# hiroharu-kato/neural_renderer

Measured on AMD Instinct MI355X. Metric: rasterize fwd+bwd Mpixels/sec @256x256 batch=64, higher is better.
Workload: dtype f32

## Files before the change

neural_renderer_amd/_build.py:

```python
import os
import subprocess

HERE = os.path.dirname(os.path.abspath(__file__))
SOURCES = [os.path.join(HERE, 'csrc', n) for n in ('nr_forward.hip', 'nr_backward.hip', 'nr_backward_pixel_map.hip',
                                                      'nr_backward_gather.hip', 'nr_geometry.hip',
                                                      'nr_image.hip', 'nr_frontend.hip', 'nr_texture_io.hip', 'nr_optim.hip',
                                                      'nr_uv_pixel.hip', 'nr_vertex_colors.hip')]
HEADERS = [os.path.join(os.path.dirname(HERE), 'include', 'nr_hip.h'), os.path.join(os.path.dirname(HERE), 'include', 'nr_hip_profile.h'),
           os.path.join(HERE, 'csrc', 'nr_device.h'),
           os.path.join(HERE, 'csrc', 'nr_k6_tune.h'), os.path.join(HERE, 'csrc', 'nr_band_lines.h'),
           os.path.join(HERE, 'csrc', 'nr_shade.h')]
LIB_PATH = os.path.join(HERE, 'libnr_hip.so')
PROFILE_LIB_PATH = os.path.join(HERE, 'libnr_hip_prof.so')

HIPCC_FLAGS = [
    '--offload-arch=gfx950', '-O3', '-std=c++17', '-ffp-contract=off',
    '-fhip-fp32-correctly-rounded-divide-sqrt', '-munsafe-fp-atomics', '-fno-fast-math',
    '-fno-slp-vectorize',
    '-fPIC', '-shared', '-fvisibility=hidden',
]


def hipcc():
    for c in (os.environ.get('HIPCC'), '/opt/rocm/bin/hipcc', 'hipcc'):
        if c and (os.path.isabs(c) and os.path.exists(c) or not os.path.isabs(c)):
            return c
    return 'hipcc'


def needs_build():
    if not os.path.exists(LIB_PATH):
        return True
    t = os.path.getmtime(LIB_PATH)
    return any(os.path.getmtime(p) > t for p in SOURCES + HEADERS + [os.path.abspath(__file__)])


def build(force=False, verbose=False):
    if force or needs_build():
        cmd = [hipcc()] + HIPCC_FLAGS + SOURCES + ['-o', LIB_PATH]
        if verbose:
            print(' '.join(cmd))
        subprocess.check_call(cmd)
    return LIB_PATH


def build_profile(force=False, verbose=False):
    if force or not os.path.exists(PROFILE_LIB_PATH) or \
            any(os.path.getmtime(p) > os.path.getmtime(PROFILE_LIB_PATH) for p in SOURCES + HEADERS + [os.path.abspath(__file__)]):
        cmd = [hipcc()] + HIPCC_FLAGS + ['-DNR_PROFILE_HOOK=1'] + SOURCES + ['-o', PROFILE_LIB_PATH]
        if verbose:
            print(' '.join(cmd))
        subprocess.check_call(cmd)
    return PROFILE_LIB_PATH


def build_variant(tag, defines, verbose=False, sources=None, flags=None):
    out = os.path.join(HERE, 'libnr_hip_%s.so' % tag)
    cmd = [hipcc()] + (flags or HIPCC_FLAGS) + ['-D%s' % d for d in defines] + (sources or SOURCES) + ['-o', out]
    if verbose:
        print(' '.join(cmd))
    subprocess.check_call(cmd)
    return out


if __name__ == '__main__':
    import sys
    if len(sys.argv) > 2:
        print(build_variant(sys.argv[1], sys.argv[2:], verbose=True))
    else:
        print(build(force=True, verbose=True))
        print(build_profile(force=True, verbose=True))
```

neural_renderer_amd/csrc/nr_backward.hip:

```cpp
#include "nr_device.h"
#include "nr_band_lines.h"
#include "nr_k6_tune.h"

using namespace nr;

int nr::plan_backward(const BackwardCall &c, BackwardPlan &p)
{
    p = {};
    const bool fused = c.stages == STAGE_ALL;
    const bool k6 = (c.stages & STAGE_K6) && (c.rgb || c.alpha);
    const bool k7 = (c.stages & STAGE_K7) && (!fused || (c.grad_rgb_map && c.grad_textures));
    const bool k8 = (c.stages & STAGE_K8) && (!fused || c.grad_depth_map);
    const bool sampled = c.sampling_weight_map != nullptr;
    if (!c.faces || !c.face_index_map) return NR_E_NULL;
    if ((c.stages & (STAGE_K6 | STAGE_K8)) && !c.grad_faces) return NR_E_NULL;
    if (c.stages == STAGE_K6 && !k6) return NR_E_MODE;
    if (k6 && c.rgb && (!c.rgb_map || !c.grad_rgb_map)) return NR_E_NULL;
    if (k6 && c.alpha && (!c.alpha_map || !c.grad_alpha_map)) return NR_E_NULL;
    if (k7) {
        if (!c.grad_rgb_map || !c.grad_textures) return NR_E_NULL;
        if ((c.sampling_index_map != nullptr) != sampled) return NR_E_MODE;
        if (!sampled && (!c.weight_map || !c.depth_map)) return NR_E_NULL;
    }
    if (k8 && (!c.depth_map || !c.weight_map || !c.grad_depth_map)) return NR_E_NULL;
    if (int e = check_sizes(c.B, c.F, c.S)) return e;
    if (k6 && (size_t)c.B * c.S * c.S > 0x7fffffffull / 3) return NR_E_SIZE;
    if (k7 && (c.ts < 2 || c.ts > 1024)) return NR_E_SIZE;
    if (k7 && c.lit.light && sampled) return NR_E_MODE;

    const int B = c.B, F = c.F, ts = c.ts;
    p.k6 = k6;
    if (k6) {
        p.k6p = plan_k6(B, F, c.S, c.rgb, c.eps, c.flags);
        p.bands = p.k6p.kernel != K6_KERNEL_GLOBAL;
        if (p.bands && (!c.workspace || c.workspace_bytes < nr_backward_workspace_bytes(B, F, c.S, 1, 0))) return NR_E_WORKSPACE;
    }
    const bool fold = p.bands && k7 && ts <= 13;
    p.gather_first = fold && (size_t)B * F <= k6::SHARED_LAUNCH_MAX_FACES && !(c.flags & NR_FLAG_SERIAL_BACKWARD);
    p.face_zeros = p.gather_first ? FACE_ZEROS_ALL : (fold ? FACE_ZEROS_UNLISTED : FACE_ZEROS_NONE);
    p.finish = !p.bands ? FINISH_NONE : p.gather_first ? (ts <= 8 ? FINISH_BIG : FINISH_ADD) : (fold ? FINISH_GATHER : FINISH_KERNEL);

    if (k7) {
        const size_t n_tex = (size_t)ts * ts * ts * 3;
        const bool ts2_static = ts == 2 && (float)(1.0 - c.eps) < 1.0f;
        p.static_taps = ts2_static && !sampled;
        p.gather = ts <= 13 ? GATHER_FACE : GATHER_ATOMIC;
        p.listed = p.bands && ts <= 13;
        p.lanes = p.static_taps ? 16 : (ts <= 5 ? 16 : (ts <= 8 ? 64 : 256));
        p.gather_lds = p.static_taps ? 0 : (size_t)(256 / p.lanes) * n_tex * sizeof(double);
        p.big = ts <= 8;
        p.depth_in_gather = k8 && ts <= 8 && !sampled && !(ts == 2 && !ts2_static);
        p.tex_bytes = (size_t)B * (c.lit.light ? c.lit.tex_faces : F) * n_tex * sizeof(float);
        if (p.gather_first) {
            p.setup_in_gather = p.k6p.use_records && k6_line_setup_args(c, p.k6p).lds_bytes <= 32768 && p.gather_lds <= 40960;
            if (p.setup_in_gather && !c.lit.light && ((size_t)c.grad_textures & 15) == 0) p.tex_zeros = TEX_ZEROS_SETUP;
        } else if (fold && p.tex_bytes % 16 == 0 && ((size_t)c.grad_textures & 15) == 0 && p.tex_bytes <= p.k6p.fill_max) {
            p.tex_zeros = TEX_ZEROS_BAND;
        }
        if (p.tex_zeros == TEX_ZEROS_NONE && (c.lit.light || p.listed || ts > 13)) p.tex_zeros = TEX_ZEROS_FILL;
        p.light_fill = c.lit.light && c.lit.grad_light;
    }
    p.setup_alone = p.bands && p.k6p.use_records && !p.setup_in_gather;
    p.depth = k8 && !p.depth_in_gather;
    p.fill_faces = fused && !k6;
    p.depth_lists = p.fill_faces && k8 && c.visible_faces && c.workspace && k6_lists_fit(B, F, c.workspace_bytes);
    return 0;
}

static int fill_texture_zeros(const BackwardCall &c, const BackwardPlan &p)
{
    int e = p.tex_zeros == TEX_ZEROS_FILL ? fill_bytes(c.grad_textures, 0, p.tex_bytes, c.st) : 0;
    if (e == 0 && p.light_fill) e = fill_bytes(c.lit.grad_light, 0, (size_t)c.B * c.F * 3 * sizeof(float), c.st);
    return e;
}

int nr::run_backward(const BackwardCall &c)
{
    BackwardPlan p;
    if (int e = plan_backward(c, p)) return e;
    K6Lists l = {};
    if (p.fill_faces)
        if (int e = fill_bytes(c.grad_faces, 0, (size_t)c.B * c.F * 9 * sizeof(float), c.st)) return e;
    if (p.depth_lists) l = k6_list_visible(c);
    if (p.k6) {
        LineSetupArgs ls = {};
        if (p.bands) {
            if (int rc = k6_compact(c, p.k6p, p.face_zeros, l)) return rc;
            ls = k6_line_setup_args(c, p.k6p);
        }
        if (p.gather_first) {
            if (int rc = fill_texture_zeros(c, p)) return rc;
            if (int rc = gather_faces(c, p, l, p.setup_in_gather ? &ls : nullptr)) return rc;
        }
        if (p.setup_alone)
            if (int rc = run_line_setup(ls, c.st)) return rc;
        const bool band_fill = p.tex_zeros == TEX_ZEROS_BAND;
        if (int rc = k6_band(c, p.k6p, l, ls, band_fill ? c.grad_textures : nullptr, band_fill ? p.tex_bytes : 0)) return rc;
        if (p.finish == FINISH_KERNEL) k6_finalize(c, l, false);
    }
    if (p.gather != GATHER_NONE && !p.gather_first) {
        if (int rc = fill_texture_zeros(c, p)) return rc;
        if (p.gather == GATHER_FACE)
            if (int rc = gather_faces(c, p, l, nullptr)) return rc;
    }
    if (p.big) gather_big(c, p, l);
    if (p.gather == GATHER_ATOMIC) gather_atomic(c);
    if (p.depth) gather_depth(c, l);
    if (p.finish == FINISH_ADD) k6_finalize(c, l, true);
    return launch_status();
}

NR_API int nr_backward_pixel_map(const float *faces, const int32_t *face_index_map, const float *rgb_map,
                                 const float *alpha_map, const float *grad_rgb_map, const float *grad_alpha_map,
                                 float *grad_faces, int32_t B, int32_t F, int32_t S, double eps, int32_t return_rgb,
                                 int32_t return_alpha, int32_t flags, const uint8_t *visible_faces, void *workspace,
                                 size_t workspace_bytes, void *stream)
{
    BackwardCall c = {};
    c.stages = STAGE_K6, c.rgb = return_rgb != 0, c.alpha = return_alpha != 0;
    c.faces = faces, c.face_index_map = face_index_map, c.rgb_map = rgb_map, c.alpha_map = alpha_map;
    c.grad_rgb_map = grad_rgb_map, c.grad_alpha_map = grad_alpha_map, c.grad_faces = grad_faces;
    c.B = B, c.F = F, c.S = S, c.eps = eps, c.flags = flags, c.visible_faces = visible_faces;
    c.workspace = workspace, c.workspace_bytes = workspace_bytes, c.st = (hipStream_t)stream;
    return run_backward(c);
}

NR_API int nr_backward_textures(const int32_t *face_index_map, const float *sampling_weight_map,
                                const int32_t *sampling_index_map, const float *faces, const float *faces_z_ref,
                                const float *weight_map, const float *depth_map, const float *grad_rgb_map,
                                float *grad_textures, int32_t B, int32_t F, int32_t S, int32_t ts, double eps, int32_t flags,
                                void *stream)
{
    BackwardCall c = {};
    c.stages = STAGE_K7;
    c.faces = faces, c.faces_z_ref = faces_z_ref, c.face_index_map = face_index_map;
    c.sampling_weight_map = sampling_weight_map, c.sampling_index_map = sampling_index_map;
    c.weight_map = weight_map, c.depth_map = depth_map, c.grad_rgb_map = grad_rgb_map, c.grad_textures = grad_textures;
    c.B = B, c.F = F, c.S = S, c.ts = ts, c.eps = eps, c.flags = flags, c.st = (hipStream_t)stream;
    return run_backward(c);
}

NR_API int nr_backward_depth_map(const float *faces, const float *depth_map, const int32_t *face_index_map,
                                 const float *face_inv_map, const float *weight_map, const float *grad_depth_map,
                                 float *grad_faces, int32_t B, int32_t F, int32_t S, void *stream)
{
    BackwardCall c = {};
    c.stages = STAGE_K8;
    c.faces = faces, c.face_index_map = face_index_map, c.face_inv_map = face_inv_map, c.weight_map = weight_map;
    c.depth_map = depth_map, c.grad_depth_map = grad_depth_map, c.grad_faces = grad_faces;
    c.B = B, c.F = F, c.S = S, c.st = (hipStream_t)stream;
    return run_backward(c);
}

NR_API int nr_backward_rasterize(const float *faces, const float *faces_z_ref, const int32_t *face_index_map,
                                 const float *weight_map, const float *depth_map, const float *rgb_map,
                                 const float *alpha_map, const float *grad_rgb_map, const float *grad_alpha_map,
                                 const float *grad_depth_map, float *grad_faces, float *grad_textures, int32_t B,
                                 int32_t F, int32_t S, int32_t ts, double eps, int32_t flags,
                                 const uint8_t *visible_faces, void *workspace, size_t workspace_bytes, void *stream)
{
    return nr_backward_rasterize_lit(nullptr, faces, faces_z_ref, face_index_map, weight_map, depth_map, rgb_map, alpha_map,
                                     grad_rgb_map, grad_alpha_map, grad_depth_map, grad_faces, grad_textures, B, F, S, ts,
                                     eps, flags, visible_faces, workspace, workspace_bytes, stream);
}

NR_API int nr_backward_rasterize_lit(const nr_face_light *lit, const float *faces, const float *faces_z_ref,
                                     const int32_t *face_index_map, const float *weight_map, const float *depth_map,
                                     const float *rgb_map, const float *alpha_map, const float *grad_rgb_map,
                                     const float *grad_alpha_map, const float *grad_depth_map, float *grad_faces,
                                     float *grad_textures, int32_t B, int32_t F, int32_t S, int32_t ts, double eps,
                                     int32_t flags, const uint8_t *visible_faces, void *workspace, size_t workspace_bytes,
                                     void *stream)
{
    BackwardCall c = {};
    if (int e = face_light_args(grad_rgb_map && grad_textures ? lit : nullptr, F, true, c.lit)) return e;
    c.stages = STAGE_ALL, c.rgb = grad_rgb_map != nullptr, c.alpha = grad_alpha_map != nullptr;
    c.faces = faces, c.faces_z_ref = faces_z_ref, c.face_index_map = face_index_map, c.weight_map = weight_map;
    c.depth_map = depth_map, c.rgb_map = c.rgb ? rgb_map : nullptr, c.alpha_map = c.alpha ? alpha_map : nullptr;
    c.grad_rgb_map = grad_rgb_map, c.grad_alpha_map = grad_alpha_map, c.grad_depth_map = grad_depth_map;
    c.grad_faces = grad_faces, c.grad_textures = grad_textures;
    c.B = B, c.F = F, c.S = S, c.ts = ts, c.eps = eps, c.flags = flags, c.visible_faces = visible_faces;
    c.workspace = workspace, c.workspace_bytes = workspace_bytes, c.st = (hipStream_t)stream;
    return run_backward(c);
}
```

neural_renderer_amd/csrc/nr_backward_gather.hip:

```cpp
#include "nr_device.h"
#include "nr_band_lines.h"
#include <type_traits>

using namespace nr;

namespace {

constexpr int BIG_PX = 2048;

__device__ __forceinline__ float group_sum(float v, int width)
{
    for (int o = width >> 1; o > 0; o >>= 1) v += __shfl_xor(v, o, WAVE);
    return v;
}

__device__ __forceinline__ float row16_sum_last(float v)
{
    v += __int_as_float(__builtin_amdgcn_update_dpp(0, __float_as_int(v), 0x111, 0xf, 0xf, true));
    v += __int_as_float(__builtin_amdgcn_update_dpp(0, __float_as_int(v), 0x112, 0xf, 0xf, true));
    v += __int_as_float(__builtin_amdgcn_update_dpp(0, __float_as_int(v), 0x114, 0xf, 0xf, true));
    v += __int_as_float(__builtin_amdgcn_update_dpp(0, __float_as_int(v), 0x118, 0xf, 0xf, true));
    return v;
}

struct DepthConst {
    float tmp[3], zz[3];
};
__device__ __forceinline__ DepthConst depth_constants(const float f[9], int S)
{
    const float fs = (float)S;
    const float px[3] = {to_pixel(f[0], fs), to_pixel(f[3], fs), to_pixel(f[6], fs)};
    const float py[3] = {to_pixel(f[1], fs), to_pixel(f[4], fs), to_pixel(f[7], fs)};
    float inv[9];
    compute_face_inv(px, py, inv);
    DepthConst d;
#pragma unroll
    for (int k = 0; k < 3; k++) {
        d.tmp[k] = 0.0f;
#pragma unroll
        for (int l = 0; l < 3; l++) d.tmp[k] += -inv[3 * l + k] / f[3 * l + 2];
        d.zz[k] = f[3 * k + 2] * f[3 * k + 2];
    }
    return d;
}

template <int STEPS, class Eval>
__device__ __forceinline__ void walk_owned_pixels(const Cand &cd, int n_mine, int fn, const int32_t *__restrict__ fi_img,
                                                  int S, int sub, int L, int *__restrict__ queue_base, Eval eval)
{
    const int tid = threadIdx.x;
    const int QL = L < 64 ? L : 64;
    int *queue = queue_base + (tid / QL) * (2 * QL);
    const int qsub = tid & (QL - 1);
    const int qshift = (tid & 63) & ~(QL - 1);
    const unsigned long long qmask = QL == 64 ? ~0ull : ((1ull << QL) - 1ull);
    int waiting = 0;
    for (int i = sub;; i += STEPS * L) {
        bool more2[STEPS], owned2[STEPS];
        int off2[STEPS];
#pragma unroll
        for (int h = 0; h < STEPS; ++h) {
            const int ii = i + h * L;
            more2[h] = ii < n_mine;
            int x = 0, y = 0, f = 0;
            off2[h] = 0;
            bool in = false;
            if (more2[h] && cand_pixel(cd, ii, S, x, y)) {
                off2[h] = y * S + x;
                f = fi_img[off2[h]];
                in = true;
            }
            owned2[h] = in && f == fn;
        }
        bool done = false;
#pragma unroll
        for (int h = 0; h < STEPS; ++h) {
            if (done) break;
            const bool more = more2[h], owned = owned2[h];
            const int off = off2[h];
            const bool any_more = __ballot(more) != 0ull;
            const unsigned long long m = (__ballot(owned) >> qshift) & qmask;
            if (owned) queue[waiting + __popcll(m & ((1ull << qsub) - 1ull))] = off;
            waiting += __popcll(m);
            const bool ready = waiting >= QL || (!any_more && waiting > 0);
            if (__ballot(ready) != 0ull) {
                __builtin_amdgcn_fence(__ATOMIC_RELEASE, "wavefront");
                __builtin_amdgcn_wave_barrier();
                __builtin_amdgcn_fence(__ATOMIC_ACQUIRE, "wavefront");
                const int take = ready ? (waiting < QL ? waiting : QL) : 0;
                const int e = qsub < take ? queue[qsub] : 0;
                const int rest = (ready && qsub + QL < waiting) ? queue[qsub + QL] : 0;
                __builtin_amdgcn_fence(__ATOMIC_RELEASE, "wavefront");
                __builtin_amdgcn_wave_barrier();
                __builtin_amdgcn_fence(__ATOMIC_ACQUIRE, "wavefront");
                waiting -= take;
                if (ready && qsub < waiting) queue[qsub] = rest;
                if (qsub < take) eval(e);
            }
            if (!any_more) done = true;
        }
        if (done) break;
    }
}

struct FaceGatherArgs {
    const int32_t *face_index_map;
    const float *sampling_weight_map;
    const int32_t *sampling_index_map;
    const float *faces, *zbase, *weight_map, *depth_map, *g_rgb;
    float *grad_textures;
    int n_faces_total, F, S, ts;
    double eps;
    int fix_batch_z, L;
    const int *vis_list, *vis_count;
    const float *g_depth;
    float *grad_faces;
    const double *k6_scratch;
    const int *slot_of;
    FaceLight lit;
};

template <bool TS2, bool DEPTH, bool LIT>
__device__ __forceinline__ void face_gather_body(const FaceGatherArgs &a, const int bx, const int by)
{
    const int32_t *__restrict__ face_index_map = a.face_index_map;
    const float *__restrict__ sampling_weight_map = a.sampling_weight_map;
    const int32_t *__restrict__ sampling_index_map = a.sampling_index_map;
    const float *__restrict__ faces = a.faces, *__restrict__ zbase = a.zbase, *__restrict__ weight_map = a.weight_map,
                *__restrict__ depth_map = a.depth_map, *__restrict__ g_rgb = a.g_rgb;
    float *__restrict__ grad_textures = a.grad_textures;
    const int n_faces_total = a.n_faces_total, F = a.F, S = a.S, ts = a.ts;
    const double eps = a.eps;
    const int fix_batch_z = a.fix_batch_z, L = a.L;
    const int *__restrict__ vis_list = a.vis_list, *__restrict__ vis_count = a.vis_count;
    const float *__restrict__ g_depth = a.g_depth;
    float *__restrict__ grad_faces = a.grad_faces;
    const double *__restrict__ k6_scratch = a.k6_scratch;
    const FaceLight &lit = a.lit;
    extern __shared__ __attribute__((aligned(16))) double s_acc[];
    __shared__ int s_queue[512];
    __shared__ int s_own;
    __shared__ float s_gl[3];

    const int tid = threadIdx.x;
    const int grp = tid / L, sub = tid - grp * L;
    const int n_tex = ts * ts * ts * 3;
    int gi = bx * (256 / L) + grp;
    bool face_ok = gi < n_faces_total;
    int slot = 0;
    if (vis_list) {
        slot = gi;
        const int n_vis = vis_count[by];
        if (bx * (256 / L) >= n_vis) return;
        face_ok = slot < n_vis;
        gi = face_ok ? by * F + vis_list[(size_t)by * F + slot] : 0;
    }
    double *acc_l = s_acc + (size_t)grp * n_tex;

    float acc[24];
#pragma unroll
    for (int k = 0; k < 24; k++) acc[k] = 0.0f;
    float dacc[9];
#pragma unroll
    for (int k = 0; k < 9; k++) dacc[k] = 0.0f;
    bool any_box = false;
    bool own = false;
    if (!TS2) {
        for (int k = sub; k < n_tex; k += L) acc_l[k] = 0.0;
        if (LIT) {
            if (tid < 3) s_gl[tid] = 0.0f;
            if (tid == 0) s_own = 0;
        }
        __syncthreads();
    }

    Cand cd;
    cd.n = 0;
    int fn = 0;
    size_t img = 0;
    DepthConst dc;
#pragma unroll
    for (int k = 0; k < 3; k++) dc.tmp[k] = dc.zz[k] = 0.0f;
    float face_z[3] = {1.0f, 1.0f, 1.0f};
    bool flip = false;
    size_t cube = 0;
    if (LIT) {
        const int b = vis_list ? by : gi / F, f = gi - b * F;
        flip = f >= lit.tex_faces;
        cube = (size_t)b * lit.tex_faces + (flip ? f - lit.tex_faces : f);
    }
    if (face_ok) {
        const int b = gi / F;
        fn = gi - b * F;
        const float *f = faces + (size_t)gi * 9;
        cd = face_candidates(f[0], f[1], f[3], f[4], f[6], f[7], S);
        if (cd.n > 0 && (L == 256 || (cd.n <= BIG_PX))) {
            any_box = true;
            if (DEPTH) {
                float fv[9];
#pragma unroll
                for (int k = 0; k < 9; k++) fv[k] = f[k];
                dc = depth_constants(fv, S);
            }
            const float *fz = (fix_batch_z ? faces + (size_t)b * F * 9 : zbase) + (size_t)fn * 9;
            face_z[0] = fz[2]; face_z[1] = fz[5]; face_z[2] = fz[8];
            img = (size_t)b * S * S;
        }
    }
    walk_owned_pixels<(TS2 && DEPTH) ? 1 : 2>(cd, any_box ? cd.n : 0, fn, face_index_map + img, S, sub, L, s_queue, [&](int off) {
        const size_t p = img + (size_t)off;
        float wk[3] = {0.0f, 0.0f, 0.0f}, depth = 0.0f, gd = 0.0f;
        if (weight_map) { wk[0] = weight_map[3 * p]; wk[1] = weight_map[3 * p + 1]; wk[2] = weight_map[3 * p + 2]; }
        if (depth_map) depth = depth_map[p];
        if (DEPTH) gd = g_depth[p];
        const float g[3] = {g_rgb[3 * p], g_rgb[3 * p + 1], g_rgb[3 * p + 2]};
        if (LIT) own = true;
        Taps t;
        if (sampling_weight_map) {
#pragma unroll
            for (int pn = 0; pn < 8; pn++) {
                t.w[pn] = sampling_weight_map[8 * p + pn];
                t.isc[pn] = sampling_index_map[8 * p + pn];
            }
        } else {
            compute_taps(face_z, wk, depth, ts, eps, t, LIT && flip);
        }
        if (DEPTH) {
            const float depth2 = depth * depth;
#pragma unroll
            for (int k = 0; k < 3; k++) dacc[3 * k + 2] += gd * wk[k] * depth2 / dc.zz[k];
#pragma unroll
            for (int k = 0; k < 3; k++)
#pragma unroll
                for (int l = 0; l < 2; l++) dacc[3 * k + l] += -gd * dc.tmp[l] * wk[k] * depth2 * (float)S / 2.0f;
        }
#pragma unroll
        for (int pn = 0; pn < 8; pn++) {
            if (TS2) {
                acc[3 * pn + 0] += t.w[pn] * g[0];
                acc[3 * pn + 1] += t.w[pn] * g[1];
                acc[3 * pn + 2] += t.w[pn] * g[2];
            } else {
                if (t.isc[pn] * 3 >= n_tex) continue;
                double *q = acc_l + t.isc[pn] * 3;
                atomicAdd(q + 0, (double)(t.w[pn] * g[0]));
                atomicAdd(q + 1, (double)(t.w[pn] * g[1]));
                atomicAdd(q + 2, (double)(t.w[pn] * g[2]));
            }
        }
    });

    bool owned = false;
    if (LIT) {
        if (L <= 64) {
            const unsigned long long bm = __ballot(own);
            owned = L == 64 ? bm != 0ull : ((bm >> (tid & 48)) & 0xffffull) != 0ull;
        } else {
            if (own) s_own = 1;
            __syncthreads();
            owned = s_own != 0;
        }
    }
    if (TS2) {
#pragma unroll
        for (int k = 0; k < 24; k++) acc[k] = row16_sum_last(acc[k]);
        if (LIT) {
            if (face_ok && sub == 15 && owned) {
                const float *lc = lit.light + (size_t)gi * 3;
                const float l3[3] = {lc[0], lc[1], lc[2]};
                float tx[24];
                if (lit.textures) {
                    const float4 *src = reinterpret_cast<const float4 *>(lit.textures + cube * 24);
#pragma unroll
                    for (int k = 0; k < 6; k++) {
                        const float4 v = src[k];
                        tx[4 * k] = v.x; tx[4 * k + 1] = v.y; tx[4 * k + 2] = v.z; tx[4 * k + 3] = v.w;
                    }
                } else {
#pragma unroll
                    for (int k = 0; k < 24; k++) tx[k] = 0.0f;
                }
                float o[24], gl[3] = {0.0f, 0.0f, 0.0f};
#pragma unroll
                for (int u = 0; u < 8; u++) {
                    const int r = (u & 1) * 4 + (u & 2) + (u >> 2);
#pragma unroll
                    for (int c = 0; c < 3; c++) {
                        const float a = flip ? acc[3 * u + c] : acc[3 * r + c];
                        o[3 * u + c] = a * l3[c];
                        gl[c] += a * tx[3 * u + c];
                    }
                }
                float4 *dst = reinterpret_cast<float4 *>(grad_textures + cube * 24);
#pragma unroll
                for (int k = 0; k < 6; k++) dst[k] = make_float4(o[4 * k], o[4 * k + 1], o[4 * k + 2], o[4 * k + 3]);
                if (lit.grad_light) {
                    float *gd = lit.grad_light + (size_t)gi * 3;
                    gd[0] = gl[0]; gd[1] = gl[1]; gd[2] = gl[2];
                }
            }
        } else if (face_ok && sub == 15) {
            float o[24];
#pragma unroll
            for (int pn = 0; pn < 8; pn++) {
                const int isc = (pn & 1) * 4 + ((pn >> 1) & 1) * 2 + ((pn >> 2) & 1);
                o[3 * isc + 0] = acc[3 * pn + 0];
                o[3 * isc + 1] = acc[3 * pn + 1];
                o[3 * isc + 2] = acc[3 * pn + 2];
            }
            float4 *dst = reinterpret_cast<float4 *>(grad_textures + (size_t)gi * 24);
#pragma unroll
            for (int k = 0; k < 6; k++) dst[k] = make_float4(o[4 * k], o[4 * k + 1], o[4 * k + 2], o[4 * k + 3]);
        }
    } else if (LIT) {
        __syncthreads();
        float gl0 = 0.0f, gl1 = 0.0f, gl2 = 0.0f;
        if (face_ok && owned) {
            const float *lc = lit.light + (size_t)gi * 3;
            const float l3[3] = {lc[0], lc[1], lc[2]};
            const float *tex = lit.textures ? lit.textures + cube * n_tex : nullptr;
            float *dst = grad_textures + cube * n_tex;
            if (tex) {
                for (int k = sub; k < n_tex; k += L) {
                    const int c = k % 3;
                    const float v = (float)acc_l[k] * tex[k];
                    gl0 += c == 0 ? v : 0.0f;
                    gl1 += c == 1 ? v : 0.0f;
                    gl2 += c == 2 ? v : 0.0f;
                }
            }
            for (int k = sub; k < n_tex; k += L) {
                const int c = k % 3;
                dst[k] = (float)acc_l[k] * (c == 0 ? l3[0] : (c == 1 ? l3[1] : l3[2]));
            }
        }
        if (lit.grad_light) {
            if (L <= 64) {
                gl0 = group_sum(gl0, L); gl1 = group_sum(gl1, L); gl2 = group_sum(gl2, L);
            } else {
                if (gl0 != 0.0f) atomicAdd(&s_gl[0], gl0);
                if (gl1 != 0.0f) atomicAdd(&s_gl[1], gl1);
                if (gl2 != 0.0f) atomicAdd(&s_gl[2], gl2);
                __syncthreads();
                gl0 = s_gl[0]; gl1 = s_gl[1]; gl2 = s_gl[2];
            }
            if (face_ok && owned && sub == 0) {
                float *gd = lit.grad_light + (size_t)gi * 3;
                gd[0] = gl0; gd[1] = gl1; gd[2] = gl2;
            }
        }
    } else {
        __syncthreads();
        if (face_ok) {
            float *dst = grad_textures + (size_t)gi * n_tex;
            for (int k = sub; k < n_tex; k += L) dst[k] = (float)acc_l[k];
        }
    }
    if (DEPTH || k6_scratch) {
        if (DEPTH && __ballot(any_box) != 0ull) {
#pragma unroll
            for (int k = 0; k < 9; k++) dacc[k] = (L == 16) ? row16_sum_last(dacc[k]) : group_sum(dacc[k], L);
        }
        if (face_ok && sub == ((L == 16) ? 15 : 0)) {
            float *gf = grad_faces + (size_t)gi * 9;
            if (k6_scratch) {
                const double *sc = k6_scratch + ((size_t)by * F + slot) * 6;
#pragma unroll
                for (int v = 0; v < 3; v++) {
                    gf[3 * v + 0] = (float)sc[2 * v + 0] + dacc[3 * v + 0];
                    gf[3 * v + 1] = (float)sc[2 * v + 1] + dacc[3 * v + 1];
                    gf[3 * v + 2] = 0.0f + dacc[3 * v + 2];
                }
            } else if (any_box) {
#pragma unroll
                for (int k = 0; k < 9; k++) gf[k] += dacc[k];
            }
        }
    }
}

template <bool TS2, bool DEPTH, bool LIT>
__global__ __launch_bounds__(256) void k_backward_textures_face(FaceGatherArgs a)
{
    face_gather_body<TS2, DEPTH, LIT>(a, (int)blockIdx.x, (int)blockIdx.y);
}

struct ZeroArgs {
    float *grad_textures;
    const int *slot_of;
    int F;
    int epf;
    int vec;
    unsigned wgs;
};

__device__ __forceinline__ void zero_unlisted_body(const ZeroArgs &z, const int bx, const int by)
{
    const size_t per_image = (size_t)z.F * z.epf;
    const size_t e0 = (size_t)bx * 2048, e1 = e0 + 2048 < per_image ? e0 + 2048 : per_image;
    const int *__restrict__ slot = z.slot_of + (size_t)by * z.F;
    for (size_t e = e0 + threadIdx.x; e < e1; e += 256) {
        const int face = (int)(e / (unsigned)z.epf);
        if (slot[face] >= 0) continue;
        const size_t at = (size_t)by * per_image + e;
        if (z.vec) reinterpret_cast<float4 *>(z.grad_textures)[at] = make_float4(0.0f, 0.0f, 0.0f, 0.0f);
        else z.grad_textures[at] = 0.0f;
    }
}

template <bool TS2, bool DEPTH, bool LIT>
__global__ __launch_bounds__(256) void k_setup_gather(LineSetupArgs ls, FaceGatherArgs g, ZeroArgs z, unsigned gather_x)
{
    const unsigned bx = blockIdx.x;
    if (bx < ls.grid_x) line_setup_body(ls, (int)bx, (int)blockIdx.y);
    else if (bx < ls.grid_x + gather_x) face_gather_body<TS2, DEPTH, LIT>(g, (int)(bx - ls.grid_x), (int)blockIdx.y);
    else zero_unlisted_body(z, (int)(bx - ls.grid_x - gather_x), (int)blockIdx.y);
}

template <int TEX, bool DEPTH, bool LIT>
__global__ __launch_bounds__(256) void k_backward_big(
    const int32_t *__restrict__ face_index_map, const float *__restrict__ sampling_weight_map,
    const int32_t *__restrict__ sampling_index_map, const float *__restrict__ face_inv_map, const float *__restrict__ faces,
    const float *__restrict__ zbase, const float *__restrict__ weight_map, const float *__restrict__ depth_map, const float *__restrict__ g_rgb,
    float *__restrict__ grad_textures, int n_faces_total, int F, int S, int ts, double eps, int fix_batch_z,
    const int *__restrict__ vis_list, const int *__restrict__ vis_count, const float *__restrict__ g_depth,
    float *__restrict__ grad_faces, const unsigned char *__restrict__ visible, FaceLight lit,
    const double *__restrict__ k6_scratch)
{
    extern __shared__ __attribute__((aligned(16))) double s_tex[];
    __shared__ int s_list[256];
    __shared__ int s_wave_n[4];
    __shared__ float s_red[36];
    __shared__ int s_own;
    const int tid = threadIdx.x;
    if (vis_list && (int)blockIdx.x * 256 >= vis_count[blockIdx.y]) return;
    int n_big;
    {
        int gi = blockIdx.x * 256 + tid;
        bool ok = gi < n_faces_total;
        if (vis_list) {
            ok = gi < vis_count[blockIdx.y];
            gi = ok ? (int)blockIdx.y * F + vis_list[(size_t)blockIdx.y * F + gi] : 0;
        }
        if (k6_scratch && ok && blockIdx.z == 0) {
            const double *sc = k6_scratch + ((size_t)blockIdx.y * F + blockIdx.x * 256 + tid) * 6;
            float *gf = grad_faces + (size_t)gi * 9;
#pragma unroll
            for (int v = 0; v < 3; v++) {
                atomicAdd(gf + 3 * v + 0, (float)sc[2 * v + 0]);
                atomicAdd(gf + 3 * v + 1, (float)sc[2 * v + 1]);
            }
        }
        bool big = false;
        if (ok && !vis_list && visible && !visible[gi]) ok = false;
        if (ok) {
            const float *f = faces + (size_t)gi * 9;
            const Cand cd = face_candidates(f[0], f[1], f[3], f[4], f[6], f[7], S);
            big = cd.n > BIG_PX;
        }
        const unsigned long long m = __ballot(big);
        const int lane = tid & 63, wave = tid >> 6;
        if (lane == 0) s_wave_n[wave] = __popcll(m);
        __syncthreads();
        int before = 0;
        for (int w = 0; w < wave; w++) before += s_wave_n[w];
        if (big) s_list[before + __popcll(m & ((1ull << lane) - 1ull))] = gi;
        n_big = s_wave_n[0] + s_wave_n[1] + s_wave_n[2] + s_wave_n[3];
        __syncthreads();
    }
    const int n_tex = TEX ? ts * ts * ts * 3 : 0;
    const int n_lds = TEX == 1 ? n_tex : 0;
    for (int q = blockIdx.z; q < n_big; q += gridDim.z) {
        const int gi = s_list[q];
        const int b = gi / F, fn = gi - b * F;
        const float *fp = faces + (size_t)gi * 9;
        float f[9];
#pragma unroll
        for (int k = 0; k < 9; k++) f[k] = fp[k];
        const Cand cd = face_candidates(f[0], f[1], f[3], f[4], f[6], f[7], S);
        DepthConst dc;
        if (DEPTH) dc = depth_constants(f, S);
        const float *fz = (fix_batch_z ? faces + (size_t)b * F * 9 : zbase) + (size_t)fn * 9;
        const float face_z[3] = {fz[2], fz[5], fz[8]};
        const bool flip = TEX && LIT && fn >= lit.tex_faces;
        for (int k = tid; k < n_lds; k += 256) s_tex[k] = 0.0;
        if (tid < 36) s_red[tid] = 0.0f;
        if (LIT && tid == 0) s_own = 0;
        __syncthreads();
        bool own = false;
        float dacc[9], tacc[24];
#pragma unroll
        for (int k = 0; k < 9; k++) dacc[k] = 0.0f;
#pragma unroll
        for (int k = 0; k < 24; k++) tacc[k] = 0.0f;
        const size_t img = (size_t)b * S * S;
        for (int i = tid; i < cd.n; i += 256) {
            int x, y;
            if (!cand_pixel(cd, i, S, x, y)) continue;
            const size_t p = img + (size_t)y * S + x;
            if (face_index_map[p] != fn) continue;
            if (LIT) own = true;
            float wk[3] = {0.0f, 0.0f, 0.0f}, depth = 0.0f;
            if (weight_map) { wk[0] = weight_map[3 * p]; wk[1] = weight_map[3 * p + 1]; wk[2] = weight_map[3 * p + 2]; }
            if (depth_map) depth = depth_map[p];
            if (TEX) {
                Taps t;
                if (sampling_weight_map) {
#pragma unroll
                    for (int pn = 0; pn < 8; pn++) {
                        t.w[pn] = sampling_weight_map[8 * p + pn];
                        t.isc[pn] = sampling_index_map[8 * p + pn];
                    }
                } else {
                    compute_taps(face_z, wk, depth, ts, eps, t, flip);
                }
                const float g[3] = {g_rgb[3 * p], g_rgb[3 * p + 1], g_rgb[3 * p + 2]};
#pragma unroll
                for (int pn = 0; pn < 8; pn++) {
                    if (TEX == 2) {
                        tacc[3 * pn + 0] += t.w[pn] * g[0];
                        tacc[3 * pn + 1] += t.w[pn] * g[1];
                        tacc[3 * pn + 2] += t.w[pn] * g[2];
                    } else {
                        if (t.isc[pn] * 3 >= n_tex) continue;
                        double *a = s_tex + t.isc[pn] * 3;
                        atomicAdd(a + 0, (double)(t.w[pn] * g[0]));
                        atomicAdd(a + 1, (double)(t.w[pn] * g[1]));
                        atomicAdd(a + 2, (double)(t.w[pn] * g[2]));
                    }
                }
            }
            if (DEPTH) {
                const float gd = g_depth[p];
                const float depth2 = depth * depth;
                float tmp[3] = {dc.tmp[0], dc.tmp[1], dc.tmp[2]};
                if (face_inv_map) {
                    tmp[0] = tmp[1] = tmp[2] = 0.0f;
#pragma unroll
                    for (int k = 0; k < 3; k++)
#pragma unroll
                        for (int l = 0; l < 3; l++) tmp[k] += -face_inv_map[9 * p + 3 * l + k] / f[3 * l + 2];
                }
#pragma unroll
                for (int k = 0; k < 3; k++) dacc[3 * k + 2] += gd * wk[k] * depth2 / dc.zz[k];
#pragma unroll
                for (int k = 0; k < 3; k++)
#pragma unroll
                    for (int l = 0; l < 2; l++) dacc[3 * k + l] += -gd * tmp[l] * wk[k] * depth2 * (float)S / 2.0f;
            }
        }
        if (DEPTH) {
#pragma unroll
            for (int k = 0; k < 9; k++) {
                const float v = group_sum(dacc[k], 64);
                if ((tid & 63) == 0 && v != 0.0f) atomicAdd(&s_red[k], v);
            }
        }
        if (TEX == 2) {
#pragma unroll
            for (int k = 0; k < 24; k++) {
                const float v = group_sum(tacc[k], 64);
                if ((tid & 63) == 0 && v != 0.0f) atomicAdd(&s_red[9 + k], v);
            }
        }
        if (TEX && LIT && own) s_own = 1;
        __syncthreads();
        if (TEX && LIT) {
            if (s_own) {
                const size_t cube = (size_t)b * lit.tex_faces + (flip ? fn - lit.tex_faces : fn);
                const float *lc = lit.light + (size_t)gi * 3;
                const float *tex = lit.textures ? lit.textures + cube * n_tex : nullptr;
                float *dst = grad_textures + cube * n_tex;
                for (int k = tid; k < n_tex; k += 256) {
                    const int q = k / 3, c = k - 3 * q;
                    int u = k;
                    float a;
                    if (TEX == 2) {
                        u = 3 * (flip ? q : (q & 1) * 4 + (q & 2) + (q >> 2)) + c;
                        a = s_red[9 + k];
                    } else {
                        a = (float)s_tex[k];
                    }
                    dst[u] = a * lc[c];
                    if (tex && a != 0.0f) atomicAdd(&s_red[33 + c], a * tex[u]);
                }
                if (lit.grad_light) {
                    __syncthreads();
                    if (tid < 3) lit.grad_light[(size_t)gi * 3 + tid] = s_red[33 + tid];
                }
            }
        } else {
        if (TEX == 1) {
            float *dst = grad_textures + (size_t)gi * n_tex;
            for (int k = tid; k < n_tex; k += 256) dst[k] = (float)s_tex[k];
        }
        if (TEX == 2 && tid < 24) {
            const int pn = tid / 3, c = tid - 3 * pn;
            const int isc = (pn & 1) * 4 + ((pn >> 1) & 1) * 2 + ((pn >> 2) & 1);
            grad_textures[(size_t)gi * 24 + 3 * isc + c] = s_red[9 + tid];
        }
        }
        if (DEPTH && tid < 9) {
            if (k6_scratch) atomicAdd(grad_faces + (size_t)gi * 9 + tid, s_red[tid]);
            else grad_faces[(size_t)gi * 9 + tid] += s_red[tid];
        }
        __syncthreads();
    }
}

__global__ __launch_bounds__(256) void k_backward_textures_atomic(
    const int32_t *__restrict__ face_index_map, const float *__restrict__ sampling_weight_map,
    const int32_t *__restrict__ sampling_index_map, const float *__restrict__ faces,
    const float *__restrict__ zbase, const float *__restrict__ weight_map, const float *__restrict__ depth_map,
    const float *__restrict__ g_rgb, float *__restrict__ grad_textures, int F, int S, int ts, double eps,
    int fix_batch_z, size_t n_pixels)
{
    const size_t i = (size_t)blockIdx.x * blockDim.x + threadIdx.x;
    if (i >= n_pixels) return;
    const int fi = face_index_map[i];
    if (fi < 0) return;
    const int b = (int)(i / ((size_t)S * S));
    Taps t;
    if (sampling_weight_map) {
#pragma unroll
        for (int pn = 0; pn < 8; pn++) {
            t.w[pn] = sampling_weight_map[8 * i + pn];
            t.isc[pn] = sampling_index_map[8 * i + pn];
        }
    } else {
        const float *face = (fix_batch_z ? faces + (size_t)b * F * 9 : zbase) + (size_t)fi * 9;
        const float w[3] = {weight_map[3 * i], weight_map[3 * i + 1], weight_map[3 * i + 2]};
        const float fz[3] = {face[2], face[5], face[8]};
        compute_taps(fz, w, depth_map[i], ts, eps, t);
    }
    const float g[3] = {g_rgb[3 * i], g_rgb[3 * i + 1], g_rgb[3 * i + 2]};
    float *gt = grad_textures + ((size_t)b * F + fi) * ts * ts * ts * 3;
#pragma unroll
    for (int pn = 0; pn < 8; pn++) {
        if (t.isc[pn] >= ts * ts * ts) continue;
        float *p = gt + t.isc[pn] * 3;
        atomicAdd(p + 0, t.w[pn] * g[0]);
        atomicAdd(p + 1, t.w[pn] * g[1]);
        atomicAdd(p + 2, t.w[pn] * g[2]);
    }
}


__global__ __launch_bounds__(256) void k_backward_textures_atomic_lit(
    const int32_t *__restrict__ face_index_map, const float *__restrict__ faces, const float *__restrict__ zbase,
    const float *__restrict__ weight_map, const float *__restrict__ depth_map, const float *__restrict__ g_rgb,
    float *__restrict__ grad_textures, int F, int S, int ts, double eps, int fix_batch_z, size_t n_pixels, FaceLight lit)
{
    const size_t i = (size_t)blockIdx.x * blockDim.x + threadIdx.x;
    if (i >= n_pixels) return;
    const int fi = face_index_map[i];
    if (fi < 0) return;
    const int b = (int)(i / ((size_t)S * S));
    const bool flip = fi >= lit.tex_faces;
    const size_t cube = ((size_t)b * lit.tex_faces + (flip ? fi - lit.tex_faces : fi)) * ts * ts * ts * 3;
    Taps t;
    const float *face = (fix_batch_z ? faces + (size_t)b * F * 9 : zbase) + (size_t)fi * 9;
    const float w[3] = {weight_map[3 * i], weight_map[3 * i + 1], weight_map[3 * i + 2]};
    const float fz[3] = {face[2], face[5], face[8]};
    compute_taps(fz, w, depth_map[i], ts, eps, t, flip);
    const float g[3] = {g_rgb[3 * i], g_rgb[3 * i + 1], g_rgb[3 * i + 2]};
    const float *lc = lit.light + ((size_t)b * F + fi) * 3;
    const float l3[3] = {lc[0], lc[1], lc[2]};
    float *gt = grad_textures + cube;
    const float *tex = lit.textures ? lit.textures + cube : nullptr;
    float sample[3] = {0.0f, 0.0f, 0.0f};
#pragma unroll
    for (int pn = 0; pn < 8; pn++) {
        if (t.isc[pn] >= ts * ts * ts) continue;
        float *p = gt + t.isc[pn] * 3;
#pragma unroll
        for (int c = 0; c < 3; c++) {
            atomicAdd(p + c, (t.w[pn] * g[c]) * l3[c]);
            if (tex) sample[c] += t.w[pn] * tex[t.isc[pn] * 3 + c];
        }
    }
    if (lit.grad_light) {
        float *gl = lit.grad_light + ((size_t)b * F + fi) * 3;
#pragma unroll
        for (int c = 0; c < 3; c++) atomicAdd(gl + c, g[c] * sample[c]);
    }
}

__global__ __launch_bounds__(256) void k_backward_depth_face(
    const float *__restrict__ faces, const float *__restrict__ depth_map, const int32_t *__restrict__ face_index_map,
    const float *__restrict__ face_inv_map, const float *__restrict__ weight_map, const float *__restrict__ g_depth,
    float *__restrict__ grad_faces, int n_faces_total, int F, int S, const int *__restrict__ vis_list,
    const int *__restrict__ vis_count, const unsigned char *__restrict__ visible)
{
    constexpr int L = 16;
    const int tid = threadIdx.x;
    const int grp = tid / L, sub = tid - grp * L;
    if (vis_list && (int)blockIdx.x * (256 / L) >= vis_count[blockIdx.y]) return;
    int gi = blockIdx.x * (256 / L) + grp;
    bool face_ok = gi < n_faces_total;
    if (vis_list) {
        const int slot = gi;
        face_ok = slot < vis_count[blockIdx.y];
        gi = face_ok ? (int)blockIdx.y * F + vis_list[(size_t)blockIdx.y * F + slot] : 0;
    } else if (visible && face_ok && !visible[gi]) {
        face_ok = false;
    }
    float acc[9];
#pragma unroll
    for (int k = 0; k < 9; k++) acc[k] = 0.0f;
    bool any_box = false;
    __shared__ int s_queue[512];
    Cand cd;
    cd.n = 0;
    int fn = 0;
    size_t img = 0;
    float f[9];
#pragma unroll
    for (int k = 0; k < 9; k++) f[k] = 1.0f;
    DepthConst dc;
#pragma unroll
    for (int k = 0; k < 3; k++) dc.tmp[k] = dc.zz[k] = 0.0f;
    if (face_ok) {
        const int b = gi / F;
        fn = gi - b * F;
        const float *fp = faces + (size_t)gi * 9;
#pragma unroll
        for (int k = 0; k < 9; k++) f[k] = fp[k];
        cd = face_candidates(f[0], f[1], f[3], f[4], f[6], f[7], S);
        if (cd.n > 0 && cd.n <= BIG_PX) {
            any_box = true;
            dc = depth_constants(f, S);
            img = (size_t)b * S * S;
        }
    }
    walk_owned_pixels<2>(cd, any_box ? cd.n : 0, fn, face_index_map + img, S, sub, L, s_queue, [&](int off) {
        const size_t p = img + (size_t)off;
        const float depth = depth_map[p];
        const float w[3] = {weight_map[3 * p], weight_map[3 * p + 1], weight_map[3 * p + 2]};
        const float gd = g_depth[p];
        const float depth2 = depth * depth;
#pragma unroll
        for (int k = 0; k < 3; k++) acc[3 * k + 2] += gd * w[k] * depth2 / dc.zz[k];
        float tmp[3] = {dc.tmp[0], dc.tmp[1], dc.tmp[2]};
        if (face_inv_map) {
            tmp[0] = tmp[1] = tmp[2] = 0.0f;
#pragma unroll
            for (int k = 0; k < 3; k++)
#pragma unroll
                for (int l = 0; l < 3; l++) tmp[k] += -face_inv_map[9 * p + 3 * l + k] / f[3 * l + 2];
        }
#pragma unroll
        for (int k = 0; k < 3; k++)
#pragma unroll
            for (int l = 0; l < 2; l++) acc[3 * k + l] += -gd * tmp[l] * w[k] * depth2 * (float)S / 2.0f;
    });
    if (__ballot(any_box) == 0ull) return;
#pragma unroll
    for (int k = 0; k < 9; k++) acc[k] = row16_sum_last(acc[k]);
    if (face_ok && any_box && sub == 15) {
        float *gf = grad_faces + (size_t)gi * 9;
#pragma unroll
        for (int k = 0; k < 9; k++) gf[k] += acc[k];
    }
}

inline dim3 big_grid(bool listed, int B, int F)
{
    const size_t n = (size_t)B * F;
    const dim3 g = listed ? dim3((unsigned)((F + 255) / 256), (unsigned)B) : dim3((unsigned)((n + 255) / 256));
    const size_t ranges = (size_t)g.x * g.y;
    const size_t target = n / 64 < 1024 ? 1024 : (n / 64 > 4096 ? 4096 : n / 64);
    const size_t z = target / ranges;
    return dim3(g.x, g.y, (unsigned)(z < 1 ? 1 : (z > 64 ? 64 : z)));
}

}


int nr::gather_faces(const BackwardCall &c, const BackwardPlan &p, const K6Lists &l, const LineSetupArgs *ls)
{
    const int B = c.B, F = c.F, n = B * F, ts = c.ts;
    const size_t n_tex = (size_t)ts * ts * ts * 3;
    const int per = 256 / p.lanes;
    const int *vis_list = p.listed ? l.vis_list : nullptr;
    const dim3 grid = vis_list ? dim3((unsigned)((F + per - 1) / per), (unsigned)B) : dim3((unsigned)((n + per - 1) / per));
    const bool fold = p.finish == FINISH_GATHER;
    const FaceGatherArgs ga = {c.face_index_map, c.sampling_weight_map, c.sampling_index_map, c.faces,
                               c.faces_z_ref ? c.faces_z_ref : c.faces,
                               c.weight_map, c.depth_map, c.grad_rgb_map, c.grad_textures, n, F, c.S, ts, c.eps,
                               (c.flags & NR_FLAG_FIX_TEXTURE_BATCH_Z) ? 1 : 0, p.lanes, vis_list, l.vis_count,
                               p.depth_in_gather ? c.grad_depth_map : nullptr,
                               (p.depth_in_gather || fold) ? c.grad_faces : nullptr, fold ? l.scratch : nullptr,
                               fold ? l.slot_of : nullptr, c.lit};
    auto go = [&](auto ts2, auto dep, auto lit) {
        constexpr bool T = decltype(ts2)::value, D = decltype(dep)::value, LIT = decltype(lit)::value;
        if (ls) {
            ZeroArgs z = {c.grad_textures, l.slot_of, F, (int)n_tex, 0, 0u};
            if (p.tex_zeros == TEX_ZEROS_SETUP) {
                z.vec = n_tex % 4 == 0;
                z.epf = z.vec ? (int)(n_tex / 4) : (int)n_tex;
                z.wgs = (unsigned)(((size_t)F * z.epf + 2047) / 2048);
            }
            const size_t both = p.gather_lds > ls->lds_bytes ? p.gather_lds : ls->lds_bytes;
            hipLaunchKernelGGL((k_setup_gather<T, D, LIT>), dim3(ls->grid_x + grid.x + z.wgs, (unsigned)B), dim3(256), both, c.st,
                               *ls, ga, z, grid.x);
        } else {
            hipLaunchKernelGGL((k_backward_textures_face<T, D, LIT>), grid, dim3(256), p.gather_lds, c.st, ga);
        }
    };
    auto with_lit = [&](auto ts2, auto dep) {
        if (c.lit.light) go(ts2, dep, std::true_type()); else go(ts2, dep, std::false_type());
    };
    using T = std::true_type;
    using N = std::false_type;
    if (p.static_taps) { if (p.depth_in_gather) with_lit(T(), T()); else with_lit(T(), N()); }
    else { if (p.depth_in_gather) with_lit(N(), T()); else with_lit(N(), N()); }
    return launch_status();
}

void nr::gather_big(const BackwardCall &c, const BackwardPlan &p, const K6Lists &l)
{
    const int n = c.B * c.F, ts = c.ts;
    const int *vis_list = p.listed ? l.vis_list : nullptr;
    const dim3 grid = big_grid(vis_list != nullptr, c.B, c.F);
    const size_t lds = p.static_taps ? 0 : (size_t)ts * ts * ts * 3 * sizeof(double);
    const float *zbase = c.faces_z_ref ? c.faces_z_ref : c.faces;
    const int fix = (c.flags & NR_FLAG_FIX_TEXTURE_BATCH_Z) ? 1 : 0;
    const double *finish_k6 = p.finish == FINISH_BIG ? l.scratch : nullptr;
    const float *g_depth = p.depth_in_gather ? c.grad_depth_map : nullptr;
    float *grad_faces = (p.depth_in_gather || finish_k6) ? c.grad_faces : nullptr;
    auto go = [&](auto lit) {
        constexpr bool LIT = decltype(lit)::value;
#define NR_BIG(T, D)                                                                                                            \
    hipLaunchKernelGGL((k_backward_big<T, D, LIT>), grid, dim3(256), lds, c.st, c.face_index_map, c.sampling_weight_map,        \
                       c.sampling_index_map, (const float *)nullptr, c.faces, zbase, c.weight_map, c.depth_map, c.grad_rgb_map, \
                       c.grad_textures, n, c.F, c.S, ts, c.eps, fix, vis_list, l.vis_count, g_depth, grad_faces,               \
                       (const unsigned char *)nullptr, c.lit, finish_k6)
        if (p.static_taps) { if (g_depth) NR_BIG(2, true); else NR_BIG(2, false); }
        else { if (g_depth) NR_BIG(1, true); else NR_BIG(1, false); }
#undef NR_BIG
    };
    if (c.lit.light) go(std::true_type()); else go(std::false_type());
}

void nr::gather_atomic(const BackwardCall &c)
{
    const size_t np = (size_t)c.B * c.S * c.S;
    const float *zbase = c.faces_z_ref ? c.faces_z_ref : c.faces;
    const int fix = (c.flags & NR_FLAG_FIX_TEXTURE_BATCH_Z) ? 1 : 0;
    if (c.lit.light)
        hipLaunchKernelGGL(k_backward_textures_atomic_lit, dim3((unsigned)((np + 255) / 256)), dim3(256), 0, c.st,
                           c.face_index_map, c.faces, zbase, c.weight_map, c.depth_map, c.grad_rgb_map, c.grad_textures, c.F,
                           c.S, c.ts, c.eps, fix, np, c.lit);
    else
        hipLaunchKernelGGL(k_backward_textures_atomic, dim3((unsigned)((np + 255) / 256)), dim3(256), 0, c.st, c.face_index_map,
                           c.sampling_weight_map, c.sampling_index_map, c.faces, zbase, c.weight_map, c.depth_map,
                           c.grad_rgb_map, c.grad_textures, c.F, c.S, c.ts, c.eps, fix, np);
}

void nr::gather_depth(const BackwardCall &c, const K6Lists &l)
{
    const int B = c.B, F = c.F, n = B * F;
    const dim3 grid = l.vis_list ? dim3((unsigned)((F + 15) / 16), (unsigned)B) : dim3((unsigned)((n + 15) / 16));
    hipLaunchKernelGGL(k_backward_depth_face, grid, dim3(256), 0, c.st, c.faces, c.depth_map, c.face_index_map, c.face_inv_map,
                       c.weight_map, c.grad_depth_map, c.grad_faces, n, F, c.S, l.vis_list, l.vis_count, c.visible_faces);
    const dim3 grid_big = big_grid(l.vis_list != nullptr, B, F);
    hipLaunchKernelGGL((k_backward_big<0, true, false>), grid_big, dim3(256), 0, c.st, c.face_index_map, (const float *)nullptr,
                       (const int32_t *)nullptr, c.face_inv_map, c.faces, c.faces, c.weight_map, c.depth_map, (const float *)nullptr,
                       (float *)nullptr, n, F, c.S, 2, 0.0, 0, l.vis_list, l.vis_count, c.grad_depth_map, c.grad_faces,
                       c.visible_faces, FaceLight(), (const double *)nullptr);
}
```

neural_renderer_amd/csrc/nr_backward_pixel_map.hip:

```cpp
#include "nr_device.h"
#include "nr_band_lines.h"
#include "nr_k6_tune.h"

#include <atomic>
#include <mutex>
#include <type_traits>

using namespace nr;

namespace {

constexpr int GRP = 10;
constexpr int NGRP = 6;

struct __attribute__((aligned(16))) LineRec {
    int in_rng;
    int out_rng;
    int base;
    int flags;
    float cross, c0, c1, pad;
    float in_c[4];
    float out_c[4];
};

template <bool RGB, bool ALPHA>
__global__ __launch_bounds__(WAVE) void k_bpm_global(
    const float *__restrict__ faces, const int32_t *__restrict__ fi_map, const float *__restrict__ rgb_map,
    const float *__restrict__ alpha_map, const float *__restrict__ g_rgb, const float *__restrict__ g_alpha,
    float *__restrict__ grad_faces, int F, int S, double eps)
{
    __shared__ LineRec recs[NGRP][GRP];

    const int lane = threadIdx.x;
    const int gi = blockIdx.x;
    const int b = gi / F, fn = gi - b * F;
    const float *f = faces + (size_t)gi * 9;
    const float fx[3] = {f[0], f[3], f[6]}, fy[3] = {f[1], f[4], f[7]};
    float *out = grad_faces + (size_t)gi * 9;
    if (is_backside(fx[0], fy[0], fx[1], fy[1], fx[2], fy[2])) {
        if (lane < 9) out[lane] = 0.0f;
        return;
    }
    const int g = lane / GRP, sub = lane - g * GRP;
    const bool lane_on = g < NGRP;
    const int edge = (g >> 1) % 3, axis = g & 1;
    const double s_d = (double)S, two_over_s = 2.0 / (double)S;
    const bool s_pow2 = (S & (S - 1)) == 0;

    const float fs = (float)S;
    const int i0 = edge, i1 = (edge + 1) % 3, i2 = (edge + 2) % 3;
    const float ppx[3] = {to_pixel(fx[i0], fs), to_pixel(fx[i1], fs), to_pixel(fx[i2], fs)};
    const float ppy[3] = {to_pixel(fy[i0], fs), to_pixel(fy[i1], fs), to_pixel(fy[i2], fs)};
    const float p0x = axis ? ppy[0] : ppx[0], p0y = axis ? ppx[0] : ppy[0];
    const float p1x = axis ? ppy[1] : ppx[1], p1y = axis ? ppx[1] : ppy[1];
    const float p2x = axis ? ppy[2] : ppx[2], p2y = axis ? ppx[2] : ppy[2];
    int direction;
    if (axis == 0) direction = (p0x < p1x) ? -1 : 1; else direction = (p0x < p1x) ? 1 : -1;
    const int d0_from = (int)fmax((double)ceilf(fminf(p0x, p1x)), 0.0);
    const int d0_to = (int)fmin((double)fmaxf(p0x, p1x), S - 1.0);
    int n_lines = 0;
    if (lane_on && p0x != p1x && d0_to >= d0_from) n_lines = d0_to - d0_from + 1;
    const float slope = (p1y - p0y) / (p1x - p0x);
    const int sd0 = axis ? S : 1, sd1 = axis ? 1 : S;
    const int img_base = b * S * S;

    int max_lines = n_lines;
#pragma unroll
    for (int o = 32; o > 0; o >>= 1) max_lines = max(max_lines, __shfl_xor(max_lines, o, WAVE));

    double G0 = 0.0, G1 = 0.0;

    for (int batch0 = 0; batch0 < max_lines; batch0 += GRP) {
        if (lane_on) {
            LineRec r;
            r.in_rng = 1; r.out_rng = 1; r.base = 0; r.flags = 0;
            r.cross = r.c0 = r.c1 = r.pad = 0.0f;
#pragma unroll
            for (int k = 0; k < 4; k++) { r.in_c[k] = 0.0f; r.out_c[k] = 0.0f; }
            const int it = batch0 + sub;
            if (it < n_lines) {
                const int d0 = d0_from + it;
                const float d0f = (float)d0;
                const float d1_cross = slope * (d0f - p0x) + p0y;
                const int d1_in = (0 < direction) ? (int)floorf(d1_cross) : (int)ceilf(d1_cross);
                const int d1_out = d1_in + direction;
                if (!(d1_in < 0 || S <= d1_in) && !(d1_out < 0 || S <= d1_out)) {
                    const int line_base = img_base + d0 * sd0;
                    const int idx_in = line_base + d1_in * sd1, idx_out = line_base + d1_out * sd1;
                    if (ALPHA) { r.in_c[0] = alpha_map[idx_in]; r.out_c[0] = alpha_map[idx_out]; }
                    if (RGB) {
#pragma unroll
                        for (int k = 0; k < 3; k++) {
                            r.in_c[1 + k] = rgb_map[3 * (size_t)idx_in + k];
                            r.out_c[1 + k] = rgb_map[3 * (size_t)idx_out + k];
                        }
                    }
                    const bool is_in_fn = (fi_map[idx_in] == fn);
                    int flags = 0;
                    if (p1x != d0f) flags |= 4;
                    if (p0x != d0f) flags |= 8;
                    r.c0 = (p1x - p0x) / (p1x - d0f);
                    r.c1 = (p1x - p0x) / (d0f - p0x);
                    if (is_in_fn) {
                        const int lim = (0 < direction) ? S - 1 : 0;
                        const int o_from = max(min(d1_out, lim), 0), o_to = min(max(d1_out, lim), S - 1);
                        r.out_rng = o_from | (o_to << 16);
                        flags |= 2;
                    }
                    float d0_cross2;
                    if ((d0f - p0x) * (d0f - p2x) < 0)
                        d0_cross2 = (p2y - p0y) / (p2x - p0x) * (d0f - p0x) + p0y;
                    else
                        d0_cross2 = (p1y - p2y) / (p1x - p2x) * (d0f - p2x) + p2y;
                    const int lim2 = (0 < direction) ? (int)ceilf(d0_cross2) : (int)floorf(d0_cross2);
                    const int i_from = max(min(d1_in, lim2), 0), i_to = min(max(d1_in, lim2), S - 1);
                    r.in_rng = i_from | (i_to << 16);
                    r.base = line_base;
                    r.flags = flags;
                    r.cross = d1_cross;
                }
            }
            recs[g][sub] = r;
        }
        __syncthreads();

        const int nl = lane_on ? min(max(n_lines - batch0, 0), GRP) : 0;
        int l = -1, ph = 0, d1 = 0, d1_end = -1, base = 0, cur_flags = 0;
        float cross = 0, c0 = 0, c1 = 0, ref_a = 0, ref_r = 0, ref_g = 0, ref_b = 0;
        while (__ballot(l < nl) != 0ull) {
            if (d1 > d1_end && l < nl) {
                if (ph == 0 && (cur_flags & 2)) ph = 1; else { ph = 0; ++l; }
                if (l < nl) {
                    const LineRec *r = &recs[g][l];
                    const int4 h = *reinterpret_cast<const int4 *>(r);
                    const float4 q = *reinterpret_cast<const float4 *>(&r->cross);
                    const float4 col = *reinterpret_cast<const float4 *>(ph == 0 ? r->out_c : r->in_c);
                    const int rng = ph == 0 ? h.x : h.y;
                    d1 = (rng & 0xffff) + sub;
                    d1_end = rng >> 16;
                    base = h.z;
                    cur_flags = h.w;
                    cross = q.x; c0 = q.y; c1 = q.z;
                    ref_a = col.x; ref_r = col.y; ref_g = col.z; ref_b = col.w;
                }
            }
            if (l < nl && d1 <= d1_end) {
                const int idx = base + d1 * sd1;
                bool skip = (ph == 0) && (fi_map[idx] != fn);
                float diff = 0.0f;
                if (!skip) {
                    if (ALPHA) diff += (alpha_map[idx] - ref_a) * g_alpha[idx];
                    if (RGB) {
                        const float *pp = rgb_map + 3 * (size_t)idx;
                        const float *gg = g_rgb + 3 * (size_t)idx;
                        diff += (pp[0] - ref_r) * gg[0];
                        diff += (pp[1] - ref_g) * gg[1];
                        diff += (pp[2] - ref_b) * gg[2];
                    }
                }
                if (!skip && !(diff <= 0.0f)) {
                    const float t = (float)d1 - cross;
                    if (cur_flags & 4) {
                        const float ct = c0 * t;
                        float dist = (float)(s_pow2 ? (double)ct * two_over_s : (double)ct * 2.0 / s_d);
                        dist = (0.0f < dist) ? (float)((double)dist + eps) : (float)((double)dist - eps);
                        G0 -= (double)(diff / dist);
                    }
                    if (cur_flags & 8) {
                        const float ct = c1 * t;
                        float dist = (float)(s_pow2 ? (double)ct * two_over_s : (double)ct * 2.0 / s_d);
                        dist = (0.0f < dist) ? (float)((double)dist + eps) : (float)((double)dist - eps);
                        G1 -= (double)(diff / dist);
                    }
                }
                d1 += GRP;
            }
        }
        __syncthreads();
    }

#pragma unroll
    for (int o = 8; o > 0; o >>= 1) {
        const double t0 = __shfl_down(G0, o, WAVE), t1 = __shfl_down(G1, o, WAVE);
        if (sub + o < GRP) { G0 += t0; G1 += t1; }
    }
    const int partner = (2 * ((edge + 2) % 3) + axis) * GRP;
    const double G1p = __shfl(G1, partner, WAVE);
    if (lane_on && sub == 0) {
        out[3 * edge + (1 - axis)] = (float)(G0 + G1p);
        if (axis == 0) out[3 * edge + 2] = 0.0f;
    }
}


constexpr int BAND_WIN = 256;
constexpr int FSEG = 15;
enum { K6_FAST = 0, K6_EXACT_POW2 = 1, K6_EXACT = 2 };

__global__ __launch_bounds__(256) void k_mark_visible(const int32_t *__restrict__ fi_map,
                                                      unsigned char *__restrict__ flags, int F, int SS, size_t P)
{
    const size_t i = (size_t)blockIdx.x * blockDim.x + threadIdx.x;
    if (i >= P) return;
    const int fi = fi_map[i];
    if (fi >= 0) flags[(i / SS) * F + fi] = 1;
}

__device__ __forceinline__ void emit_visible(int b, int fn, int pos, int F, int S, const float *__restrict__ faces,
                                             int *__restrict__ vis_list, unsigned *__restrict__ rng,
                                             double *__restrict__ scratch, int *band_count, int n_bands, int W,
                                             int *line_diff = nullptr)
{
    vis_list[(size_t)b * F + pos] = fn;
    const float *f = faces + ((size_t)b * F + fn) * 9;
    const float fs = (float)S;
    float px[3], py[3];
#pragma unroll
    for (int k = 0; k < 3; k++) { px[k] = to_pixel(f[3 * k], fs); py[k] = to_pixel(f[3 * k + 1], fs); }
    unsigned *r0 = rng + (((size_t)b * 2 + 0) * F + pos) * 3, *r1 = rng + (((size_t)b * 2 + 1) * F + pos) * 3;
#pragma unroll
    for (int e = 0; e < 3; e++) {
        const unsigned ra = edge_range(px[e], px[(e + 1) % 3], S), rb = edge_range(py[e], py[(e + 1) % 3], S);
        r0[e] = ra;
        r1[e] = rb;
#pragma unroll
        for (int axis = 0; axis < 2; axis++) {
            const unsigned r = axis ? rb : ra;
            const int lo = (int)(r & 0xffffu), hi = (int)(r >> 16);
            if (line_diff) {
                if (lo <= hi) {
                    atomicAdd(line_diff + axis * (S + 1) + lo, 1);
                    atomicAdd(line_diff + axis * (S + 1) + hi + 1, -1);
                }
                continue;
            }
            for (int band = lo / W; band * W <= hi; ++band)
                atomicAdd(band_count + axis * n_bands + band, min(hi, band * W + W - 1) - max(lo, band * W) + 1);
        }
    }
    double2 *z = reinterpret_cast<double2 *>(scratch + ((size_t)b * F + pos) * 6);
    z[0] = z[1] = z[2] = make_double2(0.0, 0.0);
}

__device__ __forceinline__ void zero_face(float *__restrict__ o)
{
#pragma unroll
    for (int k = 0; k < 9; k++) o[k] = 0.0f;
}

constexpr int VIS_CHUNK = 1024;
constexpr int SMALL_CHUNKS = 16;

__global__ __launch_bounds__(VIS_CHUNK) void k_compact_par(const unsigned char *__restrict__ flags,
                                                           int *__restrict__ vis_list, int *__restrict__ vis_count,
                                                           int *__restrict__ slot_of, int F, int n_chunks,
                                                           const float *__restrict__ faces, unsigned *__restrict__ rng,
                                                           double *__restrict__ scratch, int S,
                                                           int *__restrict__ chunk_band, int n_bands, int W,
                                                           int *__restrict__ band_cursor, float *__restrict__ zero_faces,
                                                           int zero_listed, int use_diff)
{
    extern __shared__ int s_band[];
    __shared__ int s_wcnt[VIS_CHUNK / 64];
    __shared__ int s_part[VIS_CHUNK / 64];
    const int b = blockIdx.y, chunk = blockIdx.x, tid = threadIdx.x, lane = tid & 63, wave = tid >> 6;
    for (int i = tid; i < 2 * n_bands; i += VIS_CHUNK) s_band[i] = 0;
    int *s_diff = use_diff ? s_band + 2 * n_bands : nullptr;
    if (use_diff)
        for (int i = tid; i < 2 * (S + 1); i += VIS_CHUNK) s_diff[i] = 0;
    int part = 0;
    for (int c = 0; c < chunk; ++c) part += __popcll(__ballot(flags[(size_t)b * F + c * VIS_CHUNK + tid] != 0));
    const int fn = chunk * VIS_CHUNK + tid;
    const bool v = fn < F && flags[(size_t)b * F + fn] != 0;
    const unsigned long long m = __ballot(v);
    if (lane == 0) { s_part[wave] = part; s_wcnt[wave] = __popcll(m); }
    __syncthreads();
    int off = 0, own = 0;
    for (int w = 0; w < VIS_CHUNK / 64; ++w) {
        off += s_part[w];
        if (w < wave) off += s_wcnt[w];
        own += s_wcnt[w];
    }
    if (fn < F) {
        const int before = off + __popcll(m & ((1ull << lane) - 1ull));
        slot_of[(size_t)b * F + fn] = v ? before : -1;
        if (v) emit_visible(b, fn, before, F, S, faces, vis_list, rng, scratch, s_band, n_bands, W, s_diff);
        if (zero_faces && (!v || zero_listed)) zero_face(zero_faces + ((size_t)b * F + fn) * 9);
    }
    __syncthreads();
    if (use_diff) {
        const int n2 = 2 * (S + 1), per = (n2 + VIS_CHUNK - 1) / VIS_CHUNK, i0 = tid * per, i1 = min(n2, i0 + per);
        int local = 0;
        for (int i = i0; i < i1; ++i) local += s_diff[i];
        int inc = local;
#pragma unroll
        for (int o = 1; o < 64; o <<= 1) {
            const int t = __shfl_up(inc, o, WAVE);
            if (lane >= o) inc += t;
        }
        __syncthreads();
        if (lane == 63) s_wcnt[wave] = inc;
        __syncthreads();
        int run = inc - local;
        for (int w = 0; w < wave; ++w) run += s_wcnt[w];
// ... 553 lines not shown
                        f0 = __builtin_fmaf(-dm, __builtin_amdgcn_rcpf(y0), f0);
                        f1 = __builtin_fmaf(-dm, __builtin_amdgcn_rcpf(y1), f1);
                    }
                };
                if (cls == 0) {
                    for (int u = 0; u < u_cnt; ++u) {
                    const auto p0 = f0, p1 = f1;
                    f0 = 0;
                    f1 = 0;
                    float4 gc[FB], gn[FB];
                    float ac[FB], an[FB];
#pragma unroll
                    for (int j = 0; j < FB; ++j) {
                        gc[j] = gn[j] = make_float4(0.0f, 0.0f, 0.0f, 0.0f);
                        ac[j] = an[j] = 0.0f;
                        if (RGB) gc[j] = lds_px4(gp + 4 * j);
                        else ac[j] = gp[j];
                    }
#pragma unroll
                    for (int kb = 0; kb < FSEG; kb += FB) {
                        asm volatile("" : "+v"(d1fb));
                        if (kb + FB < FSEG) {
#pragma unroll
                            for (int j = 0; j < FB; ++j) {
                                if (RGB) gn[j] = lds_px4(gp + 4 * (kb + FB + j));
                                else an[j] = gp[kb + FB + j];
                            }
                        }
#pragma unroll
                        for (int j = 0; j < FB; ++j) visit(bg_diff(gc[j], ac[j]), kb + j);
#pragma unroll
                        for (int j = 0; j < FB; ++j) { gc[j] = gn[j]; ac[j] = an[j]; }
                        __builtin_amdgcn_sched_barrier(0);
                    }
                    f0 += p0;
                    f1 += p1;
                    gp += (RGB ? 4 : 1) * FSEG;
                    d1fb += (float)FSEG;
                    }
                } else {
#pragma unroll
                    for (int kb = 0; kb < FSEG; kb += FB) {
                        asm volatile("" : "+v"(d1fb));
                        float4 g4[FB], c4[FB];
                        float ga[FB], ca[FB];
#pragma unroll
                        for (int j = 0; j < FB; ++j) {
                            g4[j] = c4[j] = make_float4(0.0f, 0.0f, 0.0f, 0.0f);
                            ga[j] = ca[j] = 0.0f;
                            if (RGB) {
                                g4[j] = lds_px4(gp + 4 * (kb + j));
                                c4[j] = lds_px4(cp + 4 * (kb + j));
                            } else {
                                ga[j] = gp[kb + j];
                                ca[j] = cp[kb + j];
                            }
                        }
#pragma unroll
                        for (int j = 0; j < FB; ++j) visit(own_diff(c4[j], ca[j], g4[j], ga[j]), kb + j);
                        __builtin_amdgcn_sched_barrier(0);
                    }
                }
            } else {
                const int own_mask = mode_in ? -1 : 0;
                float d1f = (float)s_from;
                float b0 = 0.0f, b1 = 0.0f;
                for (int l = base + s_from; l <= base + s_to; ++l, d1f += 1.0f) {
                    const int fi = px.fi[l];
                    float4 g4 = make_float4(0.0f, 0.0f, 0.0f, 0.0f), c4 = g4;
                    float ga = 0.0f, ca = 0.0f;
                    if (RGB) { g4 = lds_px4(px.g + 4 * (size_t)l); c4 = lds_px4(px.c + 4 * (size_t)l); }
                    else { ga = px.g[l]; ca = px.c[l]; }
                    const float diff = own_diff(c4, ca, g4, ga);
                    if ((((fi ^ fnr) & own_mask) != 0) | (diff <= 0.0f)) continue;
                    const float t = d1f - cross;
                    if constexpr (EXACT) {
                        f0 -= (double)exact_term(diff, c0k, t);
                        f1 -= (double)exact_term(diff, c1k, t);
                    } else {
                        const float x0 = c0k * t, x1 = c1k * t;
                        const float y0 = x0 + ((0.0f < x0) ? eps_f : -eps_f);
                        const float y1 = x1 + ((0.0f < x1) ? eps_f : -eps_f);
                        b0 = __builtin_fmaf(-diff, __builtin_amdgcn_rcpf(y0), b0);
                        b1 = __builtin_fmaf(-diff, __builtin_amdgcn_rcpf(y1), b1);
                    }
                }
                if constexpr (!EXACT) { f0 += b0; f1 += b1; }
            }
            using RunT = typename std::conditional<EXACT, double, float>::type;
            RunT p0 = (valid && (flags & 2)) ? (RunT)f0 : RunT(0), p1 = (valid && (flags & 4)) ? (RunT)f1 : RunT(0);
            const int key = valid ? line : -1 - (tid & 63);
            run_sums(key, p0, p1);
            const double a0 = (double)p0, a1 = (double)p1;
            if (a0 != 0.0) atomicAdd(&acc[2 * line], a0);
            if (a1 != 0.0) atomicAdd(&acc[2 * line + 1], a1);
        }
    }
}

template <bool RGB, bool ALPHA, int MODE, int NT, bool OVF = false>
__global__ __launch_bounds__(NT, MODE == K6_EXACT ? 4 : (NT == 256 ? k6::MINWAVES_256 : 6)) void k_bpm_fast(
    const float *__restrict__ faces, const int32_t *__restrict__ fi_map, const float *__restrict__ rgb_map,
    const float *__restrict__ alpha_map, const float *__restrict__ g_rgb, const float *__restrict__ g_alpha,
    const int *__restrict__ vis_list, const int *__restrict__ vis_count, const unsigned *__restrict__ rng,
    double *__restrict__ scratch, const int *__restrict__ band_lines, const int *__restrict__ band_start,
    const int *__restrict__ lines_ok, const BandLine *__restrict__ line_buf, size_t cap, int F, int S, int W, int SP,
    double eps, float k2s, int B, int win_lines, int qcap, uint4 *__restrict__ zero16, size_t n_zero16)
{
    extern __shared__ __attribute__((aligned(16))) unsigned char smem[];
    const int tid = threadIdx.x;
    const unsigned n_bands = (unsigned)(S + W - 1) / (unsigned)W;
    const unsigned total_wg = n_bands * 2u * (unsigned)B;
    constexpr bool overflow_only = OVF;
    auto band_body = [&](const unsigned logical) {
    if (n_zero16) {
        const size_t per = (n_zero16 + total_wg - 1) / total_wg, z_lo = (size_t)logical * per, z_hi = min(n_zero16, z_lo + per);
        for (size_t k = z_lo + tid; k < z_hi; k += NT) zero16[k] = make_uint4(0u, 0u, 0u, 0u);
    }
    const int band = (int)(logical % n_bands), axis = (int)((logical / n_bands) & 1u), b = (int)(logical / (2u * n_bands));
    const int band_lo = band * W, band_hi = min(band_lo + W, S) - 1;
    const int nld = band_hi - band_lo + 1;
    const size_t bidx = ((size_t)b * 2 + axis) * n_bands + band;
    if (overflow_only && lines_ok[b] != 0) return;
    const int n_band_lines = overflow_only ? 1 : band_lines[bidx];
    if (n_band_lines == 0) return;

    size_t off = 0;
    auto carve = [&](size_t bytes) { unsigned char *p = smem + off; off += (bytes + 15) & ~(size_t)15; return p; };
    constexpr int NC = RGB ? 4 : 1;
    FastPx px;
    px.fi = (int *)carve((size_t)W * SP * 4);
    px.g = (float *)carve((size_t)W * SP * NC * 4);
    px.c = (float *)carve((size_t)W * SP * NC * 4);
    px.bg = (float *)carve(16);
    px.CW = (((SP + 31) >> 5) + 3) & ~3;
    px.cov = (unsigned *)carve((size_t)W * px.CW * 4);
    px.span = (int *)carve(4 * 2 * 4);
    const bool wide = S > 63 * FSEG;
    BandLine *s_line = (BandLine *)carve(sizeof(BandLine) * win_lines);
    double *s_lacc = (double *)carve(16 * (size_t)win_lines);
    void *s_queue = carve((size_t)qcap * (wide ? 4 : 2));
    int *s_tmp = (int *)carve(4 * 16);

    const size_t img = (size_t)b * S * S;
    for (int i = tid; i < W * px.CW; i += NT) px.cov[i] = 0u;
    __syncthreads();
    fast_stage<RGB, ALPHA, NT>(px, fi_map, rgb_map, alpha_map, g_rgb, g_alpha, img, axis, band_lo, nld, S, SP);
    __syncthreads();
    if (tid < nld) {
        int first = 0x7fffffff, last = -1;
        for (int w = 0; w < px.CW; ++w) {
            const unsigned m = px.cov[tid * px.CW + w];
            if (m) { first = min(first, 32 * w + __ffs((int)m) - 1); last = 32 * w + 31 - __clz((int)m); }
        }
        px.span[2 * tid] = first;
        px.span[2 * tid + 1] = last;
    }

    const bool use_rec = !overflow_only && lines_ok[b] != 0;
    const BandLine *recs = line_buf + (size_t)b * cap + (use_rec ? band_start[bidx] : 0);
    const int n_vis = use_rec ? 0 : vis_count[b];
    const unsigned *rng_ba = rng + ((size_t)b * 2 + axis) * F * 3;
    int chunk = 0, win = 0;
    auto each_sum = [&](int n2, auto fn) {
        if (tid < n2) fn(tid);
        if (NT < 2 * BAND_WIN && tid + NT < n2) fn(tid + NT);
    };
    for (;;) {
        int n_win;
        if (use_rec) {
            if (win >= n_band_lines) break;
            n_win = min(n_band_lines - win, win_lines);
            if (tid < n_win) s_line[tid] = recs[win + tid];
            each_sum(2 * n_win, [&](int i) { s_lacc[i] = 0.0; });
            win += win_lines;
        } else {
            if (chunk >= n_vis) break;
            int nl = 0;
            int e_lo[3] = {0, 0, 0}, e_n[3] = {0, 0, 0};
            if (chunk + tid < n_vis) {
                const unsigned *r = rng_ba + (size_t)(chunk + tid) * 3;
#pragma unroll
                for (int e = 0; e < 3; e++) {
                    const unsigned pr = r[e];
                    const int lo = max((int)(pr & 0xffffu), band_lo), hi = min((int)(pr >> 16), band_hi);
                    if (hi >= lo) { e_lo[e] = lo; e_n[e] = hi - lo + 1; nl += e_n[e]; }
                }
            }
            int total_lines = 0;
            const int line_off = block_excl_scan<NT>(nl, s_tmp, &total_lines);
            if (win >= total_lines) {
                chunk += NT;
                win = 0;
                continue;
            }
            n_win = min(total_lines - win, win_lines);
            int2 *s_rec = reinterpret_cast<int2 *>(s_lacc);
            if (nl > 0 && line_off < win + win_lines && line_off + nl > win) {
                int k = line_off;
#pragma unroll
                for (int e = 0; e < 3; e++)
                    for (int j = 0; j < e_n[e]; j++, k++)
                        if (k >= win && k < win + win_lines) s_rec[k - win] = make_int2((chunk + tid) | (e << 28), e_lo[e] + j - band_lo);
            }
            __syncthreads();
            int2 rec = make_int2(0, 0);
            if (tid < n_win) rec = s_rec[tid];
            __syncthreads();
            if (tid < n_win) {
                const int pos = rec.x & 0x0fffffff, e = (rec.x >> 28) & 3, ld = rec.y;
                const int rfn = vis_list[(size_t)b * F + pos];
                s_line[tid] = make_fast_line(faces + ((size_t)b * F + rfn) * 9, e, axis, band_lo + ld, ld, S, rfn,
                                             pos | (e << 28) | (((e + 1) % 3) << 30),
                                             [&](int d1) { return px.fi[ld * SP + d1]; }, k2s);
            }
            each_sum(2 * n_win, [&](int i) { s_lacc[i] = 0.0; });
            win += win_lines;
        }
        __syncthreads();
        fast_sweeps<RGB, ALPHA, MODE, NT>(px, s_line, n_win, SP, eps, S, s_lacc, s_queue, qcap, wide,
                                      reinterpret_cast<unsigned long long *>(s_tmp));
        __syncthreads();
        each_sum(2 * n_win, [&](int i) {
            const double a = s_lacc[i];
            if (a != 0.0) {
                const int tgt = s_line[i >> 1].tgt;
                const int pos = tgt & 0x0fffffff, v = (i & 1) ? (tgt >> 30) & 3 : (tgt >> 28) & 3;
                atomicAdd(scratch + ((size_t)b * F + pos) * 6 + 2 * v + (1 - axis), a);
            }
        });
        __syncthreads();
    }
    };
    if constexpr (!OVF) {
        const unsigned logical = xcd_block(total_wg);
        if (logical < total_wg) band_body(logical);
    } else {
        int any = 0;
        for (int i = tid; i < B; i += NT) any |= lines_ok[i] == 0;
        if (!__syncthreads_or(any)) return;
        for (unsigned logical = blockIdx.x; logical < total_wg; logical += gridDim.x) {
            band_body(logical);
            __syncthreads();
        }
    }
}

__device__ __forceinline__ int window_team(int n_rec, int n_parts, int nsl)
{
    const int n_win = (n_rec + 63) >> 6;
    if (nsl < 32) return 1;
    int team = n_parts;
    while (team > 1 && n_parts / team < n_win) team >>= 1;
    return team;
}

__device__ __forceinline__ void wave_lds_handover()
{
    __builtin_amdgcn_fence(__ATOMIC_RELEASE, "wavefront");
    __builtin_amdgcn_wave_barrier();
    __builtin_amdgcn_fence(__ATOMIC_ACQUIRE, "wavefront");
}

namespace rowk {
constexpr int NT = 256, NW = NT / 64;
constexpr int WIN = 64;
constexpr int SEG = 16;
constexpr int MAX_SEGS = 64;
constexpr int IN_SEG = 16;
constexpr int IN_BATCH = 4;
constexpr int MAX_PX = 1024;
constexpr int K_BYTES = 4 * 16, WAVE_BYTES = WIN * 16;
template <bool RGB> __host__ __device__ constexpr size_t g_bytes(size_t npx) { return npx * (RGB ? 16 : 4); }
template <bool RGB, bool EXACT> __host__ __device__ constexpr size_t c_bytes(size_t npx) { return EXACT ? g_bytes<RGB>(npx) : npx * 4; }
template <bool RGB, bool EXACT> __host__ __device__ constexpr size_t lds_bytes(size_t npx)
{
    return g_bytes<RGB>(npx) + c_bytes<RGB, EXACT>(npx) + npx * 4 + (EXACT ? 0 : K_BYTES) + NW * WAVE_BYTES;
}
}

#ifdef NR_ROW_STATS
__device__ unsigned long long g_row_stats[8];
NR_API int nr_dev_row_stats(unsigned long long *out8)
{
    if (hipMemcpyFromSymbol(out8, HIP_SYMBOL(g_row_stats), sizeof(unsigned long long) * 8) != hipSuccess) return 1;
    unsigned long long z[8] = {0, 0, 0, 0, 0, 0, 0, 0};
    return hipMemcpyToSymbol(HIP_SYMBOL(g_row_stats), z, sizeof(z)) == hipSuccess ? 0 : 1;
}
#define NR_ROW_STAT(i, v) do { if (lane == 0) atomicAdd(&g_row_stats[i], (unsigned long long)(v)); } while (0)
constexpr unsigned NR_ROW_DUMP_WINDOWS = 1u << 16;
__device__ unsigned g_row_dump_n;
__device__ unsigned g_row_dump[NR_ROW_DUMP_WINDOWS * 64];
NR_API int nr_dev_row_dump(unsigned *out, unsigned *n_windows)
{
    if (hipMemcpyFromSymbol(n_windows, HIP_SYMBOL(g_row_dump_n), sizeof(unsigned)) != hipSuccess) return 1;
    const unsigned n = *n_windows < NR_ROW_DUMP_WINDOWS ? *n_windows : NR_ROW_DUMP_WINDOWS, zero = 0;
    if (n && hipMemcpyFromSymbol(out, HIP_SYMBOL(g_row_dump), (size_t)n * 64 * sizeof(unsigned)) != hipSuccess) return 1;
    return hipMemcpyToSymbol(HIP_SYMBOL(g_row_dump_n), &zero, sizeof(unsigned)) == hipSuccess ? 0 : 1;
}
#else
#define NR_ROW_STAT(i, v) ((void)0)
#endif

template <bool RGB, bool ALPHA, int MODE, bool CHUNKED>
__global__ __launch_bounds__(rowk::NT, MODE == K6_FAST ? 5 : 4) void k_bpm_row(
    const int32_t *__restrict__ fi_map, const float *__restrict__ rgb_map, const float *__restrict__ alpha_map,
    const float *__restrict__ g_rgb, const float *__restrict__ g_alpha, double *__restrict__ scratch,
    const int *__restrict__ band_lines, const int *__restrict__ band_start, const int *__restrict__ lines_ok,
    const BandLine *__restrict__ line_buf, size_t cap, int F, int S, int W, int CH, float eps_f, double eps_d, int B,
    uint4 *__restrict__ zero16, size_t n_zero16)
{
    using namespace rowk;
    constexpr bool EXACT = MODE != K6_FAST;
    extern __shared__ __attribute__((aligned(16))) unsigned char smem[];
    const int tid = threadIdx.x, lane = tid & 63, wave = rfl(tid >> 6);
    const unsigned n_bands = (unsigned)(S + W - 1) / (unsigned)W, n_ch = CHUNKED ? (unsigned)(S + CH - 1) / (unsigned)CH : 1u;
    const unsigned total_wg = n_bands * 2u * (unsigned)B * n_ch;
    const unsigned logical = xcd_block(total_wg);
    if (logical >= total_wg) return;
    if (n_zero16) {
        const size_t per = (n_zero16 + total_wg - 1) / total_wg, z_lo = (size_t)logical * per, z_hi = min(n_zero16, z_lo + per);
        for (size_t k = z_lo + tid; k < z_hi; k += NT) zero16[k] = make_uint4(0u, 0u, 0u, 0u);
    }
    const unsigned bandidx = logical / n_ch;
    const int c0 = CHUNKED ? (int)(logical - bandidx * n_ch) * CH : 0, SL = CHUNKED ? min(CH, S - c0) : S;
    const int band = (int)(bandidx % n_bands), axis = (int)((bandidx / n_bands) & 1u), b = (int)(bandidx / (2u * n_bands));
    if (lines_ok[b] == 0) return;
    const int band_lo = band * W, nld = min(W, S - band_lo);
    const size_t lt = ((size_t)b * 2 + axis) * S + band_lo;
    int n_tot = 0;
    for (int l = 0; l < nld; ++l) n_tot += band_lines[lt + l];
    if (n_tot == 0) return;

    constexpr int NC = RGB ? 4 : 1;
    const int SP = (SL + 31) & ~31, nsl = SP / SEG;
    const unsigned npx = (unsigned)(W * SP), G_BYTES = (unsigned)g_bytes<RGB>(npx), C_BYTES = (unsigned)c_bytes<RGB, EXACT>(npx), FI_BYTES = npx * 4u;
    float *const s_g = (float *)smem;
    float *const s_p = (float *)(smem + G_BYTES);
    int *const s_fi = (int *)(smem + G_BYTES + C_BYTES);
    float4 *const s_k = (float4 *)(smem + G_BYTES + C_BYTES + FI_BYTES);
    unsigned char *wave_mem = smem + G_BYTES + C_BYTES + FI_BYTES + (EXACT ? 0u : (unsigned)K_BYTES) + (unsigned)wave * WAVE_BYTES;
    double2 *acc = (double2 *)wave_mem;
    int *hist = (int *)wave_mem;
    const int n_parts = max(1, NW / W);
    const BandLine *recs_b = line_buf + (size_t)b * cap;
    const size_t img = (size_t)b * S * S;
    auto map_index = [&](int ld, int d1) { return axis ? img + (size_t)(band_lo + ld) * S + (c0 + d1) : img + (size_t)(c0 + d1) * S + band_lo + ld; };
    auto map_colour = [&](size_t gi) {
        float4 c = make_float4(0.0f, 0.0f, 0.0f, 0.0f);
        if constexpr (!RGB || ALPHA) c.x = alpha_map[gi];
        if constexpr (RGB) { c.y = rgb_map[3 * gi]; c.z = rgb_map[3 * gi + 1]; c.w = rgb_map[3 * gi + 2]; }
        return c;
    };
    auto line_k = [&](int ld) {
        if constexpr (EXACT) return make_float4(0.0f, 0.0f, 0.0f, 0.0f);
        float4 k = map_colour(map_index(ld, 0));
        const bool fin = fabsf(k.x) <= 3.0e38f && fabsf(k.y) <= 3.0e38f && fabsf(k.z) <= 3.0e38f && fabsf(k.w) <= 3.0e38f;
        if (!fin) k = make_float4(0.0f, 0.0f, 0.0f, 0.0f);
        return k;
    };
    int4 hh_first = make_int4(1, 1, 0, 0);
    float4 qq_first = make_float4(0.0f, 0.0f, 0.0f, 0.0f);
    if (wave < nld * n_parts) {
        const int ld = wave / n_parts, part = wave - ld * n_parts;
        const int n_rec = band_lines[lt + ld], r = (part / window_team(n_rec, n_parts, nsl)) * WIN + lane;
        if (r < n_rec) {
            const BandLine *R = recs_b + band_start[lt + ld] + r;
            hh_first = *reinterpret_cast<const int4 *>(R);
            qq_first = *reinterpret_cast<const float4 *>(&R->cross);
        }
    }
    {
        auto put = [&](int ld, int d1, int fi, const float4 &k, float al, float ga, float r, float g, float bl, float gr, float gg, float gb) {
            const int l = ld * SP + d1;
            s_fi[l] = fi;
            if constexpr (RGB) {
                *reinterpret_cast<float4 *>(s_g + 4 * (size_t)l) = make_float4(ga, gr, gg, gb);
                if constexpr (EXACT)
                    *reinterpret_cast<float4 *>(s_p + 4 * (size_t)l) = make_float4(al, r, g, bl);
                else
                    s_p[l] = (float)((ALPHA ? (double)(al - k.x) * (double)ga : 0.0) + (double)(r - k.y) * (double)gr +
                                     (double)(g - k.z) * (double)gg + (double)(bl - k.w) * (double)gb);
            } else {
                s_g[l] = ga;
                s_p[l] = EXACT ? al : (al - k.x) * ga;
            }
            if constexpr (!EXACT) { if (d1 == 0) s_k[ld] = k; }
        };
        auto put_quad = [&](size_t g, int ld0, int d10, int ld_step, int d1_step) {
            const int4 vf = *reinterpret_cast<const int4 *>(fi_map + g);
            float4 va = make_float4(0, 0, 0, 0), vg = va;
            if (ALPHA) {
                va = *reinterpret_cast<const float4 *>(alpha_map + g);
                vg = *reinterpret_cast<const float4 *>(g_alpha + g);
            }
            float rr[12], qq[12];
#pragma unroll
            for (int k = 0; k < 12; k++) rr[k] = qq[k] = 0.0f;
            if (RGB) {
                const float4 *pr = reinterpret_cast<const float4 *>(rgb_map + 3 * g);
                const float4 *pg = reinterpret_cast<const float4 *>(g_rgb + 3 * g);
                const float4 r0 = pr[0], r1 = pr[1], r2 = pr[2], q0 = pg[0], q1 = pg[1], q2 = pg[2];
                rr[0] = r0.x; rr[1] = r0.y; rr[2] = r0.z; rr[3] = r0.w; rr[4] = r1.x; rr[5] = r1.y; rr[6] = r1.z; rr[7] = r1.w;
                rr[8] = r2.x; rr[9] = r2.y; rr[10] = r2.z; rr[11] = r2.w;
                qq[0] = q0.x; qq[1] = q0.y; qq[2] = q0.z; qq[3] = q0.w; qq[4] = q1.x; qq[5] = q1.y; qq[6] = q1.z; qq[7] = q1.w;
                qq[8] = q2.x; qq[9] = q2.y; qq[10] = q2.z; qq[11] = q2.w;
            }
            const int fis[4] = {vf.x, vf.y, vf.z, vf.w};
            const float als[4] = {va.x, va.y, va.z, va.w}, gas[4] = {vg.x, vg.y, vg.z, vg.w};
            float4 k = line_k(ld0);
#pragma unroll
            for (int j = 0; j < 4; ++j) {
                if (j > 0 && ld_step) k = line_k(ld0 + j * ld_step);
                put(ld0 + j * ld_step, d10 + j * d1_step, fis[j], k, als[j], gas[j], rr[3 * j], rr[3 * j + 1], rr[3 * j + 2], qq[3 * j],
                    qq[3 * j + 1], qq[3 * j + 2]);
            }
        };
        auto put_one = [&](int ld, int d1) {
            const size_t g = map_index(ld, d1);
            float al = 0, ga = 0, r = 0, gn = 0, bl = 0, gr = 0, gg = 0, gb = 0;
            if (ALPHA) { al = alpha_map[g]; ga = g_alpha[g]; }
            if (RGB) {
                r = rgb_map[3 * g]; gn = rgb_map[3 * g + 1]; bl = rgb_map[3 * g + 2];
                gr = g_rgb[3 * g]; gg = g_rgb[3 * g + 1]; gb = g_rgb[3 * g + 2];
            }
            put(ld, d1, fi_map[g], line_k(ld), al, ga, r, gn, bl, gr, gg, gb);
        };
        if (SP != SL) {
            const int pad = SP - SL;
            for (int i = tid; i < nld * pad; i += NT) {
                const int ld = i / pad, l = ld * SP + SL + (i - ld * pad);
                s_fi[l] = -1;
                if constexpr (EXACT && RGB) *reinterpret_cast<float4 *>(s_p + 4 * (size_t)l) = make_float4(0.0f, 0.0f, 0.0f, 0.0f);
                else s_p[l] = 0.0f;
                if constexpr (RGB) *reinterpret_cast<float4 *>(s_g + 4 * (size_t)l) = make_float4(0.0f, 0.0f, 0.0f, 0.0f);
                else s_g[l] = 0.0f;
            }
        }
        if (axis && (S & 3) == 0) {
            const int quads = SL >> 2;
            for (int i = tid; i < nld * quads; i += NT) {
                const int ld = i / quads, x = (i - ld * quads) << 2;
                put_quad(img + (size_t)(band_lo + ld) * S + c0 + x, ld, x, 0, 1);
            }
        } else if (axis) {
            for (int i = tid; i < nld * SL; i += NT) put_one(i / SL, i % SL);
        } else if (nld == 4 && (S & 3) == 0 && (band_lo & 3) == 0) {
            for (int y = tid; y < SL; y += NT) put_quad(img + (size_t)(c0 + y) * S + band_lo, 0, y, 1, 0);
        } else {
            for (int i = tid; i < nld * SL; i += NT) put_one(i % nld, i / nld);
        }
    }
    __syncthreads();

    float eps_v = eps_f;
    asm volatile("" : "+v"(eps_v));
    const unsigned eps_hi = (unsigned)__double2hiint(eps_d), eps_lo = (unsigned)__double2loint(eps_d);
    const double s_d = (double)S, two_over_s_d = 2.0 / (double)S;
    const float two_over_s_f = (float)(2.0 / (double)S);
    auto exact_scale = [&](float ct) {
        if constexpr (MODE == K6_EXACT_POW2) return ct * two_over_s_f;
        float q = (float)((double)ct * two_over_s_d);
        if (__builtin_expect(!(fabsf(q) >= 1.17549435e-38f) && ct != 0.0f, 0)) q = (float)((double)ct * 2.0 / s_d);
        return q;
    };
    auto exact_dist = [&](float ct) {
        const float dist = exact_scale(ct);
        return (float)((double)dist + signed_eps(dist, eps_hi, eps_lo));
    };
    auto recip_n = [](float y) {
        const float r = __builtin_amdgcn_rcpf(y);
        return __builtin_fmaf(__builtin_fmaf(-y, r, 1.0f), r, r);
    };
    auto exact_diff = [&](const float4 &c4, const float4 &cr, const float4 &g4) {
        if constexpr (!RGB) return (c4.x - cr.x) * g4.x;
        float d = ALPHA ? (c4.x - cr.x) * g4.x + (c4.y - cr.y) * g4.y : (c4.y - cr.y) * g4.y;
        d += (c4.z - cr.z) * g4.z;
        d += (c4.w - cr.w) * g4.w;
        return d;
    };
    const int row = (lane >> 2) & 3, l16 = ((((lane >> 4) + ((lane >> 2) & 2)) & 3) << 2) | (lane & 3);
    for (int vt = wave; vt < nld * n_parts; vt += NW) {
        const int ld = vt / n_parts, part = vt - ld * n_parts;
        const int n_rec = band_lines[lt + ld];
        if (n_rec == 0) continue;
        const BandLine *recs = recs_b + band_start[lt + ld];
        const int base = ld * SP;
        float4 kc = make_float4(0.0f, 0.0f, 0.0f, 0.0f);
        if constexpr (!EXACT) kc = s_k[ld];
        const int team = window_team(n_rec, n_parts, nsl), member = part & (team - 1), n_teams = n_parts / team;
        const bool sweeps_mine = member == 0;
        const int w_first = (part / team) * WIN;
        for (int w0 = w_first; w0 < n_rec; w0 += WIN * n_teams) {
            const int nw = min(WIN, n_rec - w0);
            int4 hh = hh_first;
            float4 qq = qq_first;
            if (!(vt == wave && w0 == w_first)) {
                hh = make_int4(1, 1, 0, 0);
                qq = make_float4(0.0f, 0.0f, 0.0f, 0.0f);
                if (lane < nw) {
                    const BandLine *R = recs + w0 + lane;
                    hh = *reinterpret_cast<const int4 *>(R);
                    qq = *reinterpret_cast<const float4 *>(&R->cross);
                }
            }
            const int flags = (hh.z >> 24) & 0xff, d1_in = (hh.z & 0xffff) - c0;
            const int og_from = hh.y & 0xffff, og_to = hh.y >> 16;
            const int ig_from = hh.x & 0xffff, ig_to = hh.x >> 16;
            const bool has_out = og_from <= og_to;
            const bool has_in = ig_from <= ig_to;
            const bool dpos = (flags & 8) != 0;
            const int d1_out = d1_in + (dpos ? 1 : -1);
            const int in_from = max(ig_from, c0) - c0, in_to = min(ig_to, c0 + SL - 1) - c0;
            const bool out_px_here = has_out && d1_out >= 0 && d1_out < SL;
            const int bg_from = og_from + ((dpos && !EXACT) ? 1 : 0), bg_to = og_to - ((!dpos && !EXACT) ? 1 : 0);
            const int b_from = max(bg_from, c0) - c0, b_to = min(bg_to, c0 + SL - 1) - c0;
            const bool has_b = has_out && b_from <= b_to;
            const bool in_here = has_in && in_from <= in_to;
            float4 c_in = make_float4(0.0f, 0.0f, 0.0f, 0.0f), c_out = c_in;
            if (has_in && (has_b || in_here || out_px_here)) {
                c_in = map_colour(map_index(ld, d1_in));
                c_out = map_colour(map_index(ld, d1_out));
            }
            const float4 oref = make_float4(c_in.x - kc.x, c_in.y - kc.y, c_in.z - kc.z, c_in.w - kc.w);
            const float4 iref = make_float4(c_out.x - kc.x, c_out.y - kc.y, c_out.z - kc.z, c_out.w - kc.w);
            auto direct_diff = [&](const float4 &ci, const float4 &cr, int l) {
                float4 g4;
                if constexpr (RGB) g4 = lds_px4(s_g + 4 * (size_t)l);
                else g4 = make_float4(s_g[l], 0.0f, 0.0f, 0.0f);
                float d;
                if constexpr (EXACT) {
                    d = exact_diff(ci, cr, g4);
                } else if constexpr (RGB) {
                    d = ALPHA ? __builtin_fmaf(ci.y - cr.y, g4.y, (ci.x - cr.x) * g4.x) : (ci.y - cr.y) * g4.y;
                    d = __builtin_fmaf(ci.z - cr.z, g4.z, d);
                    d = __builtin_fmaf(ci.w - cr.w, g4.w, d);
                } else {
                    d = (ci.x - cr.x) * g4.x;
                }
                return d;
            };
            float f0 = 0.0f, f1 = 0.0f;
            if (out_px_here && !EXACT && sweeps_mine) {
                const float d = direct_diff(c_out, c_in, base + d1_out);
                const float dm = !(d <= 0.0f) ? d : 0.0f;
                const float t = fabsf((float)(c0 + d1_out) - qq.x);
                f0 = dm * recip_n(__builtin_fmaf(fabsf(qq.y), t, eps_v));
                f1 = dm * recip_n(__builtin_fmaf(fabsf(qq.z), t, eps_v));
            }
            if constexpr (!EXACT) {
                const int d1_2 = d1_out + (dpos ? 1 : -1);
                const float t2 = fabsf((float)(c0 + d1_2) - qq.x);
                if (has_out && og_from < og_to && d1_2 >= 0 && d1_2 < SL && t2 <= 1.0f && sweeps_mine) {
                    const int l = base + d1_2;
                    float4 g4;
                    if constexpr (RGB) g4 = lds_px4(s_g + 4 * (size_t)l);
                    else g4 = make_float4(s_g[l], 0.0f, 0.0f, 0.0f);
                    float d = s_p[l];
                    if constexpr (!RGB || ALPHA) d = __builtin_fmaf(-oref.x, g4.x, d);
                    if constexpr (RGB) {
                        d = __builtin_fmaf(-oref.y, g4.y, d);
                        d = __builtin_fmaf(-oref.z, g4.z, d);
                        d = __builtin_fmaf(-oref.w, g4.w, d);
                    }
                    const float dm = !(d <= 0.0f) ? d : 0.0f;
                    f0 = __builtin_fmaf(dm, recip_n(__builtin_fmaf(fabsf(qq.y), t2, eps_v)), f0);
                    f1 = __builtin_fmaf(dm, recip_n(__builtin_fmaf(fabsf(qq.z), t2, eps_v)), f1);
                }
            }
            const int nseg = has_b ? (dpos ? nsl - (b_from >> 4) : (b_to >> 4) + 1) : 0;
            hist[lane] = 0;
            double in0 = 0.0, in1 = 0.0;
            if (in_here && sweeps_mine) {
                const float cross = qq.x, c0k = qq.y, c1k = qq.z;
                const int fnr = __float_as_int(qq.w);
                const float d_first = (EXACT || d1_in < 0 || d1_in >= SL) ? 0.0f : direct_diff(c_in, c_out, base + d1_in);
                for (int s0 = in_from; s0 <= in_to; s0 += IN_SEG) {
                    const int s1 = min(s0 + IN_SEG - 1, in_to);
                    float b0 = 0.0f, b1 = 0.0f;
                    for (int q0 = s0; q0 <= s1; q0 += IN_BATCH) {
                        int fi[IN_BATCH];
                        float4 g4[IN_BATCH], c4[IN_BATCH];
                        float p4[IN_BATCH];
#pragma unroll
                        for (int k = 0; k < IN_BATCH; ++k) {
                            const int l = base + min(q0 + k, s1);
                            fi[k] = s_fi[l];
                            c4[k] = make_float4(0.0f, 0.0f, 0.0f, 0.0f);
                            p4[k] = 0.0f;
                            if constexpr (EXACT) {
                                if constexpr (RGB) c4[k] = lds_px4(s_p + 4 * (size_t)l);
                                else c4[k].x = s_p[l];
                            } else {
                                p4[k] = s_p[l];
                            }
                            if constexpr (RGB) g4[k] = lds_px4(s_g + 4 * (size_t)l);
                            else g4[k] = make_float4(s_g[l], 0.0f, 0.0f, 0.0f);
                        }
#pragma unroll
                        for (int k = 0; k < IN_BATCH; ++k) {
                            float diff;
                            if constexpr (EXACT) {
                                diff = exact_diff(c4[k], c_out, g4[k]);
                            } else {
                                diff = p4[k];
                                if constexpr (!RGB || ALPHA) diff = __builtin_fmaf(-iref.x, g4[k].x, diff);
                                if constexpr (RGB) {
                                    diff = __builtin_fmaf(-iref.y, g4[k].y, diff);
                                    diff = __builtin_fmaf(-iref.z, g4[k].z, diff);
                                    diff = __builtin_fmaf(-iref.w, g4[k].w, diff);
                                }
                                if (q0 + k == d1_in) diff = d_first;
                            }
                            const bool take = (q0 + k <= s1) & (fi[k] == fnr) & !(diff <= 0.0f);
                            const float t = (float)(c0 + q0 + k) - cross;
                            if constexpr (EXACT) {
                                const float dm = take ? diff : 0.0f;
                                const float y0 = take ? exact_dist(c0k * t) : 1.0f, y1 = take ? exact_dist(c1k * t) : 1.0f;
                                in0 -= (double)(dm / y0);
                                in1 -= (double)(dm / y1);
                            } else {
                                const float x0 = c0k * t, x1 = c1k * t;
                                const float y0 = x0 + ((0.0f < x0) ? eps_v : -eps_v);
                                const float y1 = x1 + ((0.0f < x1) ? eps_v : -eps_v);
                                const float dm = take ? diff : 0.0f;
                                b0 = __builtin_fmaf(-dm, recip_n(y0), b0);
                                b1 = __builtin_fmaf(-dm, recip_n(y1), b1);
                            }
                        }
                    }
                    in0 += (double)b0;
                    in1 += (double)b1;
                }
            }
            wave_lds_handover();
            const int key = MAX_SEGS - nseg;
            int rank = 0;
            if (has_b) rank = atomicAdd(&hist[key], 1);
            wave_lds_handover();
            const int cnt = hist[lane], incl = wave_incl_sum_dpp(cnt);
            const int n_out = __builtin_amdgcn_readlane(incl, 63);
            wave_lds_handover();
            hist[lane] = incl - cnt;
            wave_lds_handover();
            const unsigned long long no_out = __ballot(!has_b);
            int pos = n_out + (int)__builtin_amdgcn_mbcnt_hi((unsigned)(no_out >> 32), __builtin_amdgcn_mbcnt_lo((unsigned)no_out, 0u));
            if (has_b) pos = hist[key] + rank;
            const int inv = __builtin_amdgcn_ds_permute(pos << 2, lane);
            wave_lds_handover();
            NR_ROW_STAT(0, 1);
            NR_ROW_STAT(1, nw);
            NR_ROW_STAT(2, n_out);
#ifdef NR_ROW_STATS
            {
                unsigned wid = 0;
                if (lane == 0) wid = atomicAdd(&g_row_dump_n, 1u);
                wid = (unsigned)__builtin_amdgcn_readfirstlane((int)wid);
                if (wid < NR_ROW_DUMP_WINDOWS)
                    g_row_dump[(size_t)wid * 64 + lane] = lane < nw ? ((unsigned)nseg | (dpos ? 256u : 0u) | (has_b ? 512u : 0u) | 1024u) : 0u;
            }
            {
                int sn = nseg, si = has_b ? (b_to - b_from + 1) : 0;
                for (int o = 32; o > 0; o >>= 1) { sn += __shfl_xor(sn, o, WAVE); si += __shfl_xor(si, o, WAVE); }
                NR_ROW_STAT(3, sn);
                NR_ROW_STAT(4, si);
            }
#endif
            const float v_ncd = dpos ? -qq.x : qq.x;
            const float v_ac0 = EXACT ? (dpos ? qq.y : -qq.y)
                                      : __uint_as_float((__float_as_uint(qq.y) & 0x7fffffffu) | (dpos ? 0u : 0x80000000u));
            const float v_ac1 = EXACT ? (dpos ? qq.z : -qq.z) : fabsf(qq.z);
            const int v_nseg = EXACT ? (dpos ? nseg : -nseg) : nseg;
            float4 oref_b = oref;
            if constexpr (EXACT) oref_b = c_in;
            const int g_first = 4 * member, g_step = 4 * team;
            int src_next = __builtin_amdgcn_ds_bpermute(((g_first + row) & 63) << 2, inv);
            for (int g0 = g_first; g0 < n_out; g0 += g_step) {
                const bool act = g0 + row < n_out;
                const int src = src_next;
                src_next = __builtin_amdgcn_ds_bpermute(((g0 + g_step + row) & 63) << 2, inv);
                const int sa = src << 2;
                const int r_nseg_s = __builtin_amdgcn_ds_bpermute(sa, v_nseg);
                const int r_nseg = EXACT ? abs(r_nseg_s) : r_nseg_s;
                float ncd = __int_as_float(__builtin_amdgcn_ds_bpermute(sa, __float_as_int(v_ncd)));
                const float ac0s = __int_as_float(__builtin_amdgcn_ds_bpermute(sa, __float_as_int(v_ac0)));
                const float ac1 = __int_as_float(__builtin_amdgcn_ds_bpermute(sa, __float_as_int(v_ac1)));
                float ra = 0.0f, rr = 0.0f, rg = 0.0f, rb = 0.0f;
                if constexpr (!RGB || ALPHA) ra = __int_as_float(__builtin_amdgcn_ds_bpermute(sa, __float_as_int(oref_b.x)));
                if constexpr (RGB) {
                    rr = __int_as_float(__builtin_amdgcn_ds_bpermute(sa, __float_as_int(oref_b.y)));
                    rg = __int_as_float(__builtin_amdgcn_ds_bpermute(sa, __float_as_int(oref_b.z)));
                    rb = __int_as_float(__builtin_amdgcn_ds_bpermute(sa, __float_as_int(oref_b.w)));
                }
                if (!act) ncd = -__builtin_inff();
                const float sdir = EXACT ? (r_nseg_s < 0 ? -1.0f : 1.0f)
                                         : __uint_as_float(0x3f800000u | (__float_as_uint(ac0s) & 0x80000000u));
                const int steps = __builtin_amdgcn_readfirstlane(r_nseg), steps2 = EXACT ? (steps + 1) & ~1 : steps;
                NR_ROW_STAT(5, 1);
                NR_ROW_STAT(6, steps2);
                const bool rpos = EXACT ? r_nseg_s >= 0 : !(__float_as_uint(ac0s) >> 31);
                const int seg0 = rpos ? nsl - steps2 : 0;
                const int p0 = seg0 * SEG + l16;
                float pf = (float)(c0 + p0);
                double A0 = 0.0, A1 = 0.0;
                if constexpr (EXACT) {
                    const unsigned char *gp = (const unsigned char *)s_g + (size_t)(base + p0) * (NC * 4);
                    const unsigned char *cp = (const unsigned char *)s_p + (size_t)(base + p0) * (NC * 4);
                    const float4 cref = make_float4(ra, rr, rg, rb);
                    auto load_x = [&](int k, float4 &g4, float4 &c4) {
                        if constexpr (RGB) {
                            g4 = *reinterpret_cast<const float4 *>(gp + k * (SEG * NC * 4));
                            c4 = *reinterpret_cast<const float4 *>(cp + k * (SEG * NC * 4));
                        } else {
                            g4 = make_float4(*reinterpret_cast<const float *>(gp + k * (SEG * NC * 4)), 0.0f, 0.0f, 0.0f);
                            c4 = make_float4(*reinterpret_cast<const float *>(cp + k * (SEG * NC * 4)), 0.0f, 0.0f, 0.0f);
                        }
                    };
                    auto visit_x = [&](const float4 &g4, const float4 &c4, const float pfv) {
                        if constexpr (RGB && !ALPHA) asm volatile("" : : "v"(g4.x), "v"(c4.x));
                        const float d = exact_diff(c4, cref, g4);
                        const float td = __builtin_fmaf(sdir, pfv, ncd);
                        const bool keep = !(td <= 0.0f) && !(d <= 0.0f);
                        const float e0 = exact_dist(ac0s * td), e1 = exact_dist(ac1 * td);
                        const float dm = keep ? d : 0.0f, y0 = keep ? e0 : 1.0f, y1 = keep ? e1 : 1.0f;
                        A0 -= (double)(dm / y0);
                        A1 -= (double)(dm / y1);
                    };
                    for (int s = 0; s < steps2; s += 2) {
                        float4 gA, cA, gB, cB;
                        load_x(0, gA, cA);
                        load_x(1, gB, cB);
                        visit_x(gA, cA, pf);
                        visit_x(gB, cB, pf + (float)SEG);
                        gp += 2 * SEG * NC * 4;
                        cp += 2 * SEG * NC * 4;
                        pf += (float)(2 * SEG);
                    }
                    A0 = __builtin_amdgcn_mfma_f64_4x4x4f64(A0, 1.0, 0.0, 0, 0, 0);
                    A1 = __builtin_amdgcn_mfma_f64_4x4x4f64(A1, 1.0, 0.0, 0, 0, 0);
                    A0 = __builtin_amdgcn_mfma_f64_4x4x4f64(A0, 1.0, 0.0, 0, 0, 0);
                    A1 = __builtin_amdgcn_mfma_f64_4x4x4f64(A1, 1.0, 0.0, 0, 0, 0);
                } else {
                    const unsigned char *gp = (const unsigned char *)s_g + (size_t)(base + p0) * (NC * 4);
                    const float *pp = s_p + base + p0;
                    auto visit = [&](const float4 &g4, const float pv, const float pfv, float &a0, float &a1) {
                        float d = pv;
                        if constexpr (!RGB || ALPHA) d = __builtin_fmaf(-ra, g4.x, d);
                        if constexpr (RGB) {
                            d = __builtin_fmaf(-rr, g4.y, d);
                            d = __builtin_fmaf(-rg, g4.z, d);
                            d = __builtin_fmaf(-rb, g4.w, d);
                        }
                        const float td = __builtin_fmaf(sdir, pfv, ncd);
                        const bool keep = !(td <= 1.0f) && !(d <= 0.0f);
                        const float dm = keep ? d : 0.0f;
                        const float y0 = __builtin_fmaf(fabsf(ac0s), fabsf(td), eps_v), y1 = __builtin_fmaf(ac1, fabsf(td), eps_v);
                        a0 = __builtin_fmaf(dm, __builtin_amdgcn_rcpf(y0), a0);
                        a1 = __builtin_fmaf(dm, __builtin_amdgcn_rcpf(y1), a1);
                    };
                    auto load = [&](int k, float4 &g4, float &pv) {
                        if constexpr (RGB) g4 = *reinterpret_cast<const float4 *>(gp + k * (SEG * NC * 4));
                        else g4 = make_float4(*reinterpret_cast<const float *>(gp + k * (SEG * NC * 4)), 0.0f, 0.0f, 0.0f);
                        pv = pp[k * SEG];
                    };
                    auto used = [&](const float4 &g4) {
                        if constexpr (RGB && !ALPHA) asm volatile("" : : "v"(g4.x));
                    };
                    float a0 = 0.0f, a1 = 0.0f, b0 = 0.0f, b1 = 0.0f;
                    {
                        float4 gA, gB, gC, gD;
                        float pA, pB, pC, pD;
                        load(0, gA, pA);
                        load(1, gB, pB);
                        int s = 0;
                        for (; s + 4 <= steps2; s += 4) {
                            load(2, gC, pC);
                            load(3, gD, pD);
                            __builtin_amdgcn_sched_barrier(0);
                            visit(gA, pA, pf, a0, a1);
                            used(gA);
                            visit(gB, pB, pf + (float)SEG, b0, b1);
                            used(gB);
                            __builtin_amdgcn_sched_barrier(0);
                            load(4, gA, pA);
                            load(5, gB, pB);
                            __builtin_amdgcn_sched_barrier(0);
                            visit(gC, pC, pf + (float)(2 * SEG), a0, a1);
                            used(gC);
                            visit(gD, pD, pf + (float)(3 * SEG), b0, b1);
                            used(gD);
                            __builtin_amdgcn_sched_barrier(0);
                            gp += 4 * (SEG * NC * 4);
                            pp += 4 * SEG;
                            pf += (float)(4 * SEG);
                        }
                        if (const int rem = steps2 - s) {
                            if (rem == 3) load(2, gC, pC);
                            visit(gA, pA, pf, a0, a1);
                            used(gA);
                            if (rem >= 2) {
                                visit(gB, pB, pf + (float)SEG, b0, b1);
                                used(gB);
                            }
                            if (rem == 3) {
                                visit(gC, pC, pf + (float)(2 * SEG), a0, a1);
                                used(gC);
                            }
                        }
                    }
                    A0 = __builtin_amdgcn_mfma_f64_4x4x4f64((double)a0, 1.0, 0.0, 0, 0, 0);
                    A1 = __builtin_amdgcn_mfma_f64_4x4x4f64((double)a1, 1.0, 0.0, 0, 0, 0);
                    A0 = __builtin_amdgcn_mfma_f64_4x4x4f64((double)b0, 1.0, A0, 0, 0, 0);
                    A1 = __builtin_amdgcn_mfma_f64_4x4x4f64((double)b1, 1.0, A1, 0, 0, 0);
                    A0 = __builtin_amdgcn_mfma_f64_4x4x4f64(A0, 1.0, 0.0, 0, 0, 0);
                    A1 = __builtin_amdgcn_mfma_f64_4x4x4f64(A1, 1.0, 0.0, 0, 0, 0);
                }
                if (act && lane == (row << 2)) acc[src] = make_double2(A0, A1);
            }
            wave_lds_handover();
            if (lane < nw) {
                double2 a = make_double2(0.0, 0.0);
                if (has_b && ((pos >> 2) & (team - 1)) == member) a = acc[lane];
                a.x += (double)f0;
                a.y += (double)f1;
                const bool tneg = !dpos;
                const bool neg0 = EXACT || (((__float_as_uint(qq.y) >> 31) != 0) != tneg);
                const bool neg1 = EXACT || (((__float_as_uint(qq.z) >> 31) != 0) != tneg);
                const double t0 = (flags & 2) ? in0 + (neg0 ? a.x : -a.x) : 0.0;
                const double t1 = (flags & 4) ? in1 + (neg1 ? a.y : -a.y) : 0.0;
                const int tgt = hh.w, lpos = tgt & 0x0fffffff;
                double *dst = scratch + ((size_t)b * F + lpos) * 6 + (1 - axis);
                if (t0 != 0.0) atomicAdd(dst + 2 * ((tgt >> 28) & 3), t0);
                if (t1 != 0.0) atomicAdd(dst + 2 * ((tgt >> 30) & 3), t1);
            }
            wave_lds_handover();
        }
    }
}

__global__ __launch_bounds__(256) void k_bpm_finalize(const double *__restrict__ scratch, const int *__restrict__ slot_of,
                                                      float *__restrict__ grad_faces, int F, int n_faces_total, int add)
{
    const int i = blockIdx.x * blockDim.x + threadIdx.x;
    if (i >= n_faces_total) return;
    const int pos = slot_of[i];
    float *o = grad_faces + (size_t)i * 9;
    if (add) {
        if (pos < 0) return;
        const double *src = scratch + ((size_t)(i / F) * F + pos) * 6;
#pragma unroll
        for (int v = 0; v < 3; v++) {
            o[3 * v + 0] = (float)src[2 * v + 0] + o[3 * v + 0];
            o[3 * v + 1] = (float)src[2 * v + 1] + o[3 * v + 1];
        }
        return;
    }
    double a[6] = {0.0, 0.0, 0.0, 0.0, 0.0, 0.0};
    if (pos >= 0) {
        const double *src = scratch + ((size_t)(i / F) * F + pos) * 6;
#pragma unroll
        for (int k = 0; k < 6; k++) a[k] = src[k];
    }
#pragma unroll
    for (int v = 0; v < 3; v++) {
        o[3 * v + 0] = (float)a[2 * v + 0];
        o[3 * v + 1] = (float)a[2 * v + 1];
        o[3 * v + 2] = 0.0f;
    }
}


struct BpmLayout {
    size_t flags_off, scratch_off, count_off, chunk_off, cband_off, list_off, rng_off, slot_off, band_off, start_off, cursor_off, ok_off,
        lines_off, total, cap;
    int n_chunks;
};

size_t line_capacity(int F, int S)
{
    const size_t want = (size_t)8 * F + (size_t)32 * S + (size_t)(1.2 * (double)S * sqrt((double)F));
    return (want + 2047 - 1088) / 2048 * 2048 + 1088;
}

BpmLayout bpm_layout(int B, int F, int S)
{
    BpmLayout L;
    const size_t n = (size_t)B * F;
    L.flags_off = 0;
    L.scratch_off = align_up(n, 256);
    L.count_off = align_up(L.scratch_off + n * 6 * sizeof(double), 256);
    L.n_chunks = (F + VIS_CHUNK - 1) / VIS_CHUNK;
    L.chunk_off = L.count_off + align_up((size_t)B * sizeof(int), 256);
    L.cband_off = L.chunk_off + align_up((size_t)B * L.n_chunks * sizeof(int), 256);
    L.list_off = L.cband_off + (L.n_chunks <= SMALL_CHUNKS ? align_up((size_t)B * L.n_chunks * 2 * S * sizeof(int), 256) : 0);
    L.rng_off = L.list_off + align_up(n * sizeof(int), 256);
    L.slot_off = L.rng_off + align_up(n * 6 * sizeof(unsigned), 256);
    const size_t per_band = align_up((size_t)B * 2 * S * sizeof(int), 256);
    L.band_off = L.slot_off + align_up(n * sizeof(int), 256);
    L.start_off = L.band_off + per_band;
    L.cursor_off = L.start_off + per_band;
    L.ok_off = L.cursor_off + per_band;
    L.lines_off = L.ok_off + align_up((size_t)B * sizeof(int), 256);
    L.cap = line_capacity(F, S);
    L.total = L.lines_off + (size_t)B * L.cap * sizeof(BandLine);
    return L;
}

struct ListsLayout {
    size_t count_off, list_off, total;
};
ListsLayout lists_layout(int B, int F)
{
    ListsLayout L;
    L.count_off = 0;
    L.list_off = align_up((size_t)B * sizeof(int), 256);
    L.total = L.list_off + (size_t)B * F * sizeof(int);
    return L;
}

BandShape band_shape(int S)
{
    if (S <= k6::SMALL_RASTER_MAX) return {256, 2, (size_t)40 * 1024};
    if (S > k6::WIDE_BUDGET_FROM && S <= k6::WIDE_BUDGET_TO) return {512, k6::WMAX, (size_t)80 * 1024};
    return {512, k6::WMAX, k6::LDS_BUDGET};
}

int fast_band_config(int S, bool rgb, const BandShape &shape, int w_max, size_t *lds_bytes, int *win, int *qcap)
{
    const size_t per_px = rgb ? 36 : 12, SP = (size_t)S + 4, dsz = S > 63 * FSEG ? 4 : 2;
    const size_t segs_per_line = (size_t)S / (S <= 320 ? 32 : 48) + 3;
    const size_t NT = (size_t)shape.threads, LDS_BUDGET = shape.budget;
    const int win_max = BAND_WIN < shape.threads ? BAND_WIN : shape.threads;
    auto lines_bytes = [&](int ww) { return (sizeof(BandLine) + 16) * (size_t)ww; };
    for (int W = w_max; W >= 1; W >>= 1) {
        const size_t px = (size_t)W * SP * per_px + (size_t)W * (((SP + 31) / 32 + 3) / 4 * 4) * 4 + 16  + 32  + 64  +
                          8 * 16 ;
        const size_t lim = (W == 1 && px + lines_bytes(32) + NT * dsz > LDS_BUDGET) ? 160 * 1024 : LDS_BUDGET;
        if (px + lines_bytes(32) + NT * dsz > lim) continue;
        const size_t rest = lim - px;
        int w = (int)(rest / (48 + segs_per_line * dsz));
        w = max(32, min(win_max, w / 32 * 32));
        while (w > 32 && lines_bytes(w) + NT * dsz > rest) w -= 32;
        if (W > 1 && w < 96) continue;
        size_t q = (rest - lines_bytes(w)) / dsz / NT * NT;
        q = q > 16384 ? 16384 : q;
        *win = w;
        *qcap = (int)q;
        *lds_bytes = px + lines_bytes(w) + q * dsz;
        return W;
    }
    return 0;
}

struct LdsLimit {
    std::atomic<size_t> granted[32];
    std::mutex mtx;
    LdsLimit() { for (auto &g : granted) g.store(48 * 1024); }
    int ensure(const void *kern, size_t lds)
    {
        int dev = 0;
        if (hipGetDevice(&dev) != hipSuccess || dev < 0 || dev >= 32) dev = 31;
        if (lds <= granted[dev].load(std::memory_order_acquire) && dev != 31) return 0;
        std::lock_guard<std::mutex> lock(mtx);
        const size_t have = granted[dev].load(std::memory_order_relaxed);
        if (lds <= have && dev != 31) return 0;
        const size_t want = lds > have ? lds : have;
        const hipError_t e = hipFuncSetAttribute(kern, hipFuncAttributeMaxDynamicSharedMemorySize, (int)want);
        if (e != 0) return e;
        granted[dev].store(want, std::memory_order_release);
        return 0;
    }
};

template <class Fn> int with_k6_types(bool rgb, bool alpha, int mode, const Fn &f)
{
    using T = std::true_type;
    using N = std::false_type;
    auto by_mode = [&](auto r, auto a) {
        if (mode == K6_FAST) return f(r, a, std::integral_constant<int, K6_FAST>());
        if (mode == K6_EXACT_POW2) return f(r, a, std::integral_constant<int, K6_EXACT_POW2>());
        return f(r, a, std::integral_constant<int, K6_EXACT>());
    };
    return (rgb && alpha) ? by_mode(T(), T()) : (rgb ? by_mode(T(), N()) : by_mode(N(), T()));
}

template <bool RGB, bool ALPHA, int MODE, bool OVF>
int launch_fast(const K6Plan &p, const BackwardCall &c, const K6Lists &l, const LineSetupArgs &ls, void *zero_ptr, size_t zero_bytes)
{
    const int B = c.B, S = c.S;
    const unsigned total_wg = (unsigned)((S + p.W_fast - 1) / p.W_fast) * 2u * (unsigned)B;
    const unsigned grid = OVF ? (total_wg < k6::OVF_GRID ? total_wg : k6::OVF_GRID) : xcd_grid(total_wg);
    auto go = [&](auto nt) {
        constexpr int NT = decltype(nt)::value;
        static LdsLimit limit;
        auto kern = k_bpm_fast<RGB, ALPHA, MODE, NT, OVF>;
        if (int rc = limit.ensure((const void *)kern, p.fast_lds)) return rc;
        hipLaunchKernelGGL(kern, dim3(grid), dim3(NT), p.fast_lds, c.st, c.faces, c.face_index_map, c.rgb_map, c.alpha_map,
                           c.grad_rgb_map, c.grad_alpha_map, l.vis_list, l.vis_count, ls.rng, l.scratch, ls.band_lines, ls.band_start,
                           ls.lines_ok, ls.line_buf, ls.cap, c.F, S, p.W_fast, S + 4, c.eps, ls.k2s, B, p.win_lines, p.qcap,
                           (uint4 *)zero_ptr, zero_bytes / 16);
        return 0;
    };
    return p.shape.threads == 256 ? go(std::integral_constant<int, 256>()) : go(std::integral_constant<int, 512>());
}

constexpr int ROW_CHUNK_PX = 512;
int row_chunk(int S, int F)
{
    if (F >= (1 << 15)) return (S + 31) & ~31;
    const int n_ch = (S + ROW_CHUNK_PX - 1) / ROW_CHUNK_PX, len = (S + n_ch - 1) / n_ch;
    return (len + 31) & ~31;
}

int row_band_config(int S, int F, bool rgb, bool exact, int B, size_t *lds_bytes)
{
    if ((((size_t)S + 31) & ~(size_t)31) / rowk::SEG > (size_t)rowk::MAX_SEGS) return 0;
    const size_t SP = (size_t)row_chunk(S, F), n_ch = ((size_t)S + SP - 1) / SP;
    for (int W = rowk::NW; W >= 1; W >>= 1) {
        const size_t wgs = (size_t)B * 2 * ((S + W - 1) / W) * n_ch;
        if ((W > 2 && wgs < k6::ROW_MIN_WGS) || (W == 2 && wgs < k6::ROW_MIN_WGS_1)) continue;
        if ((size_t)W * SP > (size_t)rowk::MAX_PX) continue;
        const size_t npx = (size_t)W * SP;
        *lds_bytes = rgb ? (exact ? rowk::lds_bytes<true, true>(npx) : rowk::lds_bytes<true, false>(npx))
                         : (exact ? rowk::lds_bytes<false, true>(npx) : rowk::lds_bytes<false, false>(npx));
        return W;
    }
    return 0;
}

template <bool RGB, bool ALPHA, int MODE>
int launch_row(const K6Plan &p, const BackwardCall &c, const K6Lists &l, const LineSetupArgs &ls, void *zero_ptr, size_t zero_bytes)
{
    const int B = c.B, F = c.F, S = c.S;
    const double eps = c.eps;
    const int CH = row_chunk(S, F), W = p.W_row;
    const unsigned n_ch = (unsigned)((S + CH - 1) / CH), total_wg = (unsigned)((S + W - 1) / W) * 2u * (unsigned)B * n_ch;
    auto go = [&](auto chunked) {
        constexpr bool C = decltype(chunked)::value;
        static LdsLimit limit;
        if (int rc = limit.ensure((const void *)k_bpm_row<RGB, ALPHA, MODE, C>, p.row_lds)) return rc;
        hipLaunchKernelGGL((k_bpm_row<RGB, ALPHA, MODE, C>), dim3(xcd_grid(total_wg)), dim3(rowk::NT), p.row_lds, c.st,
                           c.face_index_map, c.rgb_map, c.alpha_map, c.grad_rgb_map, c.grad_alpha_map, l.scratch, ls.band_lines,
                           ls.band_start, ls.lines_ok, ls.line_buf, ls.cap, F, S, W, CH, (float)eps, eps, B, (uint4 *)zero_ptr,
                           zero_bytes / 16);
        return 0;
    };
    return n_ch > 1 ? go(std::true_type()) : go(std::false_type());
}

int k6_row_band(int B, int F, int S, bool rgb, double eps, int flags, size_t *row_lds)
{
    const bool exact = (flags & NR_FLAG_EXACT_GRADIENT) != 0;
    const bool possible = !(flags & (NR_FLAG_K6_SCAN | NR_FLAG_K6_LEGACY)) && B <= 65535 && (exact || (float)eps >= 1e-30f);
    return possible ? row_band_config(S, F, rgb, exact, B, row_lds) : 0;
}

}

K6Plan nr::plan_k6(int B, int F, int S, bool rgb, double eps, int flags)
{
    K6Plan p = {};
    const bool exact = (flags & NR_FLAG_EXACT_GRADIENT) != 0;
    p.mode = !exact ? K6_FAST : ((S & (S - 1)) == 0 ? K6_EXACT_POW2 : K6_EXACT);
    p.shape = band_shape(S);
    int w_max = p.shape.w_max, win = BAND_WIN;
    while (w_max > 1 && (size_t)B * 2 * ((S + w_max - 1) / w_max) < 3072) w_max >>= 1;
    p.W_fast = fast_band_config(S, rgb, p.shape, w_max, &p.fast_lds, &win, &p.qcap);
    if (p.W_fast == 0 || (flags & NR_FLAG_K6_GLOBAL)) {
        p.kernel = K6_KERNEL_GLOBAL;
        return p;
    }
    p.win_lines = min(win, max(4, min(BAND_WIN, (int)(65535ll * FSEG / (2ll * S))) & ~3));
    p.W_row = k6_row_band(B, F, S, rgb, eps, flags, &p.row_lds);
    const bool row = p.W_row > 0;
    p.kernel = row ? K6_KERNEL_ROW : K6_KERNEL_FAST;
    p.overflow_pass = row;
    p.W = row ? 1 : p.W_fast;
    p.n_bands = (S + p.W - 1) / p.W;
    p.use_records = !(flags & NR_FLAG_K6_SCAN) && B <= 65535 && p.n_bands <= 3072;
    const int W_band = row ? p.W_row : p.W_fast;
    const size_t band_wgs = (size_t)((S + W_band - 1) / W_band) * 2 * (size_t)B;
    p.fill_max = band_wgs * ((size_t)k6::FOLD_KB << 10) * (size_t)(row ? rowk::NT : p.shape.threads) / 512;
    return p;
}

NR_API size_t nr_backward_workspace_bytes(int32_t B, int32_t F, int32_t S, int32_t return_rgb, int32_t return_alpha)
{
    if (check_sizes(B, F, S)) return 0;
    if (!return_rgb && !return_alpha) return lists_layout(B, F).total;
    return bpm_layout(B, F, S).total;
}

#ifdef NR_PROFILE_HOOK
#include "../../include/nr_hip_profile.h"
namespace {
struct BandKernelTimer {
    bool on = false, recorded = false;
    int which = -1;
    hipEvent_t start = nullptr, stop = nullptr;
} g_band_timer;
}

NR_API int nr_profile_band_kernel(int32_t enable)
{
    BandKernelTimer &t = g_band_timer;
    if (enable && !t.start) {
        if (hipEventCreate(&t.start) != hipSuccess || hipEventCreate(&t.stop) != hipSuccess) {
            t.start = t.stop = nullptr;
            return launch_status();
        }
    }
    t.on = enable != 0 && t.start != nullptr;
    t.recorded = false;
    return 0;
}

NR_API float nr_profile_band_kernel_ms(void)
{
    BandKernelTimer &t = g_band_timer;
    float ms = -1.0f;
    if (!t.recorded || hipEventSynchronize(t.stop) != hipSuccess || hipEventElapsedTime(&ms, t.start, t.stop) != hipSuccess) {
        (void)hipGetLastError();
        return -1.0f;
    }
    return ms;
}
NR_API int nr_profile_band_kernel_which(void) { return g_band_timer.recorded ? g_band_timer.which : -1; }
NR_API int nr_profile_k6_choice(int32_t B, int32_t F, int32_t S, int32_t return_rgb, int32_t return_alpha, double eps, int32_t flags)
{
    (void)return_alpha;
    return plan_k6(B, F, S, return_rgb != 0, eps, flags).kernel == K6_KERNEL_ROW ? 1 : 0;
}
#define NR_BAND_TIMER_START(st, kernel) if (g_band_timer.on) { g_band_timer.which = (kernel); g_band_timer.recorded = hipEventRecord(g_band_timer.start, st) == hipSuccess; }
#define NR_BAND_TIMER_STOP(st) if (g_band_timer.on && g_band_timer.recorded) g_band_timer.recorded = hipEventRecord(g_band_timer.stop, st) == hipSuccess
#else
#define NR_BAND_TIMER_START(st, kernel) ((void)0)
#define NR_BAND_TIMER_STOP(st) ((void)0)
#endif


static bool compact_in_one_launch(const BpmLayout &L, int n_bands) { return L.n_chunks <= SMALL_CHUNKS && n_bands <= 4096; }

int nr::k6_compact(const BackwardCall &c, const K6Plan &plan, int face_zeros, K6Lists &out)
{
    const int B = c.B, F = c.F, S = c.S, n = B * F;
    const BpmLayout L = bpm_layout(B, F, S);
    const hipStream_t st = c.st;
    unsigned char *ws = (unsigned char *)c.workspace;
    int *band_lines = (int *)(ws + L.band_off);
    const int W = plan.W, n_bands = plan.n_bands;
    double *scratch = (double *)(ws + L.scratch_off);
    int *vis_count = (int *)(ws + L.count_off);
    int *vis_list = (int *)(ws + L.list_off);
    int *slot_of = (int *)(ws + L.slot_off);
    unsigned *rng = (unsigned *)(ws + L.rng_off);
    out = {vis_list, vis_count, slot_of, scratch};
    const unsigned char *vflags = c.visible_faces;
    if (!vflags) {
        unsigned char *f = ws + L.flags_off;
        const int he = fill_bytes(f, 0, (size_t)n, st);
        if (he != 0) return he;
        const size_t P = (size_t)B * S * S;
        hipLaunchKernelGGL(k_mark_visible, dim3((unsigned)((P + 255) / 256)), dim3(256), 0, st, c.face_index_map, f, F,
                           S * S, P);
        vflags = f;
    }
    int *band_start = (int *)(ws + L.start_off), *band_cursor = (int *)(ws + L.cursor_off), *lines_ok = (int *)(ws + L.ok_off);
    float *zero_faces = face_zeros != FACE_ZEROS_NONE ? c.grad_faces : nullptr;
    const int zero_listed = face_zeros == FACE_ZEROS_ALL ? 1 : 0;
    if (compact_in_one_launch(L, n_bands)) {
        int *chunk_band = (int *)(ws + L.cband_off);
        const int use_diff = (size_t)(2 * n_bands + 2 * (S + 1)) * sizeof(int) <= 40960 ? 1 : 0;
        hipLaunchKernelGGL(k_compact_par, dim3((unsigned)L.n_chunks, (unsigned)B), dim3(VIS_CHUNK),
                           (size_t)(2 * n_bands + (use_diff ? 2 * (S + 1) : 0)) * sizeof(int), st, vflags, vis_list, vis_count,
                           slot_of, F, L.n_chunks, c.faces, rng, scratch, S, chunk_band, n_bands, W, band_cursor, zero_faces,
                           zero_listed, use_diff);
        if (!plan.use_records)
            hipLaunchKernelGGL(k_band_total, dim3((unsigned)B), dim3(256), 0, st, chunk_band, L.n_chunks, band_lines, band_start,
                               lines_ok, n_bands);
    } else {
        int *chunk_count = (int *)(ws + L.chunk_off);
        hipLaunchKernelGGL(k_count_visible, dim3((unsigned)L.n_chunks, (unsigned)B), dim3(VIS_CHUNK), 0, st, vflags,
                           chunk_count, F, L.n_chunks, band_lines, n_bands);
        const int lds_counters = n_bands <= 4096;
        hipLaunchKernelGGL(k_compact_visible, dim3((unsigned)L.n_chunks, (unsigned)B), dim3(VIS_CHUNK),
                           lds_counters ? (size_t)2 * n_bands * sizeof(int) : 0, st, vflags, chunk_count, vis_list, vis_count,
                           slot_of, F, L.n_chunks, c.faces, rng, scratch, S, band_lines, n_bands, W, lds_counters, zero_faces,
                           zero_listed);
        hipLaunchKernelGGL(k_band_scan, dim3((unsigned)B), dim3(256), 0, st, band_lines, band_start, band_cursor, lines_ok,
                           n_bands, plan.use_records ? L.cap : 0, 0);
    }
    return launch_status();
}

LineSetupArgs nr::k6_line_setup_args(const BackwardCall &c, const K6Plan &plan)
{
    const BpmLayout L = bpm_layout(c.B, c.F, c.S);
    unsigned char *ws = (unsigned char *)c.workspace;
    const int n_bands = plan.n_bands;
    const float k2s = (c.flags & NR_FLAG_EXACT_GRADIENT) ? 1.0f : 2.0f / (float)c.S;
    return {c.faces, c.face_index_map, (const int *)(ws + L.list_off), (const int *)(ws + L.count_off),
            (const unsigned *)(ws + L.rng_off), (const int *)(ws + L.cband_off), compact_in_one_launch(L, n_bands) ? L.n_chunks : 0,
            (int *)(ws + L.band_off), (int *)(ws + L.start_off), (int *)(ws + L.cursor_off), (int *)(ws + L.ok_off),
            (BandLine *)(ws + L.lines_off), L.cap, c.F, c.S, plan.W, n_bands, k2s, (unsigned)((c.F + LS_FACES - 1) / LS_FACES),
            (unsigned)c.B, (size_t)6 * n_bands * sizeof(int)};
}

int nr::run_line_setup(const LineSetupArgs &a, hipStream_t st)
{
    static LdsLimit ls_limit;
    if (int rc = ls_limit.ensure((const void *)k_line_setup, a.lds_bytes)) return rc;
    hipLaunchKernelGGL(k_line_setup, dim3(a.grid_x, a.grid_y), dim3(256), a.lds_bytes, st, a);
    return launch_status();
}

int nr::k6_band(const BackwardCall &c, const K6Plan &plan, const K6Lists &l, const LineSetupArgs &ls, void *fill, size_t fill_bytes)
{
    if (plan.kernel == K6_KERNEL_GLOBAL) {
        auto global = [&](auto r, auto a) {
            hipLaunchKernelGGL((k_bpm_global<decltype(r)::value, decltype(a)::value>), dim3((unsigned)(c.B * c.F)), dim3(WAVE), 0,
                               c.st, c.faces, c.face_index_map, c.rgb_map, c.alpha_map, c.grad_rgb_map, c.grad_alpha_map,
                               c.grad_faces, c.F, c.S, c.eps);
            return launch_status();
        };
        using T = std::true_type;
        using N = std::false_type;
        return (c.rgb && c.alpha) ? global(T(), T()) : (c.rgb ? global(T(), N()) : global(N(), T()));
    }
    auto band_fast = [&](auto overflow_only, void *zp, size_t zb) {
        return with_k6_types(c.rgb, c.alpha, plan.mode, [&](auto r, auto a, auto m) {
            return launch_fast<decltype(r)::value, decltype(a)::value, decltype(m)::value, decltype(overflow_only)::value>(
                plan, c, l, ls, zp, zb);
        });
    };
    auto band_row = [&]() {
        return with_k6_types(c.rgb, c.alpha, plan.mode, [&](auto r, auto a, auto m) {
            return launch_row<decltype(r)::value, decltype(a)::value, decltype(m)::value>(plan, c, l, ls, fill, fill_bytes);
        });
    };
    NR_BAND_TIMER_START(c.st, plan.kernel);
    int rc = plan.kernel == K6_KERNEL_ROW ? band_row() : band_fast(std::false_type(), fill, fill_bytes);
    NR_BAND_TIMER_STOP(c.st);
    if (rc == 0 && plan.overflow_pass) rc = band_fast(std::true_type(), nullptr, 0);
    return rc ? rc : launch_status();
}

void nr::k6_finalize(const BackwardCall &c, const K6Lists &l, bool add)
{
    const int n = c.B * c.F;
    hipLaunchKernelGGL(k_bpm_finalize, dim3((unsigned)((n + 255) / 256)), dim3(256), 0, c.st, l.scratch, l.slot_of, c.grad_faces,
                       c.F, n, add ? 1 : 0);
}

bool nr::k6_lists_fit(int B, int F, size_t workspace_bytes)
{
    return workspace_bytes >= lists_layout(B, F).total && (F + VIS_CHUNK - 1) / VIS_CHUNK <= SMALL_CHUNKS;
}

K6Lists nr::k6_list_visible(const BackwardCall &c)
{
    const ListsLayout L = lists_layout(c.B, c.F);
    const int n_chunks = (c.F + VIS_CHUNK - 1) / VIS_CHUNK;
    unsigned char *ws = (unsigned char *)c.workspace;
    int *list = (int *)(ws + L.list_off), *count = (int *)(ws + L.count_off);
    hipLaunchKernelGGL(k_list_visible, dim3((unsigned)n_chunks, (unsigned)c.B), dim3(VIS_CHUNK), 0, c.st, c.visible_faces, list,
                       count, c.F, n_chunks);
    return {list, count, nullptr, nullptr};
}
```

neural_renderer_amd/csrc/nr_device.h:

```cpp
#pragma once
#include <hip/hip_runtime.h>
#include <stdint.h>
#include <stdlib.h>

#include "../../include/nr_hip.h"

#define NR_API extern "C" __attribute__((visibility("default")))

namespace nr {

constexpr int WAVE = 64;


__device__ __forceinline__ bool is_backside(float x0, float y0, float x1, float y1, float x2, float y2)
{
    return (y2 - y0) * (x1 - x0) < (y1 - y0) * (x2 - x0);
}

__device__ __forceinline__ float to_pixel(float v, float fs) { return 0.5f * (v * fs + fs - 1.0f); }

__device__ __forceinline__ void compute_face_inv(const float px[3], const float py[3], float inv[9])
{
    inv[0] = py[1] - py[2];
    inv[1] = px[2] - px[1];
// ... 39 lines not shown
{
    Cand c;
    c.x_lo = c.y_lo = 0; c.bw = 1; c.n = 0; c.strip = 0; c.a = c.b = 0.0f;
    if (is_backside(x0, y0, x1, y1, x2, y2)) return c;
    if ((x0 == x1) && (x1 == x2) && (y0 == y1) && (y1 == y2)) return c;
    const float fs = (float)S;
    const float px[3] = {to_pixel(x0, fs), to_pixel(x1, fs), to_pixel(x2, fs)};
    const float py[3] = {to_pixel(y0, fs), to_pixel(y1, fs), to_pixel(y2, fs)};
    const float den = px[2] * (py[0] - py[1]) + px[0] * (py[1] - py[2]) + px[1] * (py[2] - py[0]);
    const float e0x = x1 - x0, e0y = y1 - y0, e1x = x2 - x1, e1y = y2 - y1, e2x = x0 - x2, e2y = y0 - y2;
    const float area2 = fabsf(e0x * e1y - e0y * e1x);
    const float l0 = e0x * e0x + e0y * e0y, l1 = e1x * e1x + e1y * e1y, l2 = e2x * e2x + e2y * e2y;
    const float len2 = fmaxf(fmaxf(l0, l1), l2);
    const bool thin = !(area2 > 0x1p-18f * len2) || !(fabsf(den) > 0.0f);
    const float big = 1.0e6f;
    const bool wild = !(len2 < __builtin_inff()) || !(fabsf(den) < __builtin_inff()) ||
                      !(fmaxf(fmaxf(fabsf(px[0]), fabsf(px[1])), fabsf(px[2])) < big) ||
                      !(fmaxf(fmaxf(fabsf(py[0]), fabsf(py[1])), fabsf(py[2])) < big);
    const bool strip_ok = len2 * fs * fs * 0.25f * 0x1p-36f <= 0.25f;
    if (thin && !wild && strip_ok) {
        const int k = (l0 >= l1 && l0 >= l2) ? 0 : (l1 >= l2 ? 1 : 2);
        const float ax = px[k], ay = py[k];
        const float dx = k == 0 ? e0x : (k == 1 ? e1x : e2x), dy = k == 0 ? e0y : (k == 1 ? e1y : e2y);
        if (fabsf(dy) >= fabsf(dx) && dy != 0.0f) {
            c.strip = 1; c.a = dx / dy; c.b = ax - c.a * ay;
        } else if (dx != 0.0f) {
            c.strip = 2; c.a = dy / dx; c.b = ay - c.a * ax;
        }
        if (c.strip) { c.n = S * STRIP_W; return c; }
    }
    if (thin || wild) {
        c.bw = S; c.n = S * S;
        return c;
    }
    const float xmin = fminf(fminf(px[0], px[1]), px[2]), xmax = fmaxf(fmaxf(px[0], px[1]), px[2]);
    const float ymin = fminf(fminf(py[0], py[1]), py[2]), ymax = fmaxf(fmaxf(py[0], py[1]), py[2]);
    const float lo_c = -2.0f, hi_c = (float)S + 1.0f;
    const int xl = max((int)ceilf(fminf(fmaxf(xmin - BBOX_GUARD, lo_c), hi_c)), 0);
    const int xh = min((int)floorf(fminf(fmaxf(xmax + BBOX_GUARD, lo_c), hi_c)), S - 1);
    const int yl = max((int)ceilf(fminf(fmaxf(ymin - BBOX_GUARD, lo_c), hi_c)), 0);
    const int yh = min((int)floorf(fminf(fmaxf(ymax + BBOX_GUARD, lo_c), hi_c)), S - 1);
    if (xl <= xh && yl <= yh) {
        c.x_lo = xl; c.y_lo = yl; c.bw = xh - xl + 1; c.n = c.bw * (yh - yl + 1);
    }
    return c;
}

__device__ __forceinline__ bool cand_pixel(const Cand &c, int i, int S, int &x, int &y)
{
    if (c.strip == 0) {
        const int yy = i / c.bw;
        x = c.x_lo + (i - yy * c.bw);
        y = c.y_lo + yy;
        return true;
    }
    const int m = i / STRIP_W, j = i - m * STRIP_W;
    const int o = (int)floorf(c.a * (float)m + c.b) - 1 + j;
    if (c.strip == 1) { y = m; x = o; } else { x = m; y = o; }
    return o >= 0 && o < S;
}

struct FaceLight {
    const float *light = nullptr;
    int tex_faces = 0;
    const float *textures = nullptr;
    float *grad_light = nullptr;
};

__device__ __forceinline__ int transpose_texel(int t, int ts)
{
    const int k = t % ts, j = (t / ts) % ts, i = t / (ts * ts);
    return (k * ts + j) * ts + i;
}

struct Taps {
    int isc[8];
    float w[8];
};

__device__ __forceinline__ void compute_taps(const float *__restrict__ z, const float *__restrict__ weight,
                                             float depth, int ts, double eps, Taps &t, bool flip = false)
{
    float tif[3];
    int ti[3];
    float fr[3];
#pragma unroll
    for (int k = 0; k < 3; k++) {
        float v = weight[k] * (float)(ts - 1) * (depth / z[k]);
        v = fmaxf(v, 0.0f);
        v = (float)fmin((double)v, (double)(ts - 1) - eps);
        tif[k] = v;
        ti[k] = (int)v;
        fr[k] = v - (float)ti[k];
    }
#pragma unroll
    for (int pn = 0; pn < 8; pn++) {
        float w = 1.0f;
        int idx[3];
#pragma unroll
        for (int k = 0; k < 3; k++) {
            if (((pn >> k) & 1) == 0) {
                w *= 1.0f - fr[k];
                idx[k] = ti[k];
            } else {
                w *= fr[k];
                idx[k] = ti[k] + 1;
            }
        }
        t.isc[pn] = (flip ? idx[2] : idx[0]) * ts * ts + idx[1] * ts + (flip ? idx[0] : idx[2]);
        t.w[pn] = w;
    }
}


__device__ __forceinline__ int f2i(float x) { return (int)x; }

__device__ __forceinline__ void texel_reads(const float *face, const float d[3], int H, int W, long long p[4], float w[4])
{
    const float pos_x = (face[0] * d[0] + face[2] * d[1] + face[4] * d[2]) * (float)(W - 1);
    const float pos_y = (face[1] * d[0] + face[3] * d[1] + face[5] * d[2]) * (float)(H - 1);
    const int xi = f2i(pos_x), yi = f2i(pos_y), yi1 = f2i(pos_y + 1.0f);
    const float wx1 = pos_x - (float)xi, wx0 = 1.0f - wx1;
    const float wy1 = pos_y - (float)yi, wy0 = 1.0f - wy1;
    const long long last = (long long)H * W - 1;
    auto clampi = [&](int row, int col) -> long long {
        const long long q = (long long)row * W + col;
        return q < 0 ? 0 : (q > last ? last : q);
    };
    p[0] = clampi(yi, xi);
    p[1] = clampi(yi1, xi);
    p[2] = clampi(yi, xi + 1);
    p[3] = clampi(yi1, xi + 1);
    w[0] = wx0 * wy0;
    w[1] = wx0 * wy1;
    w[2] = wx1 * wy0;
    w[3] = wx1 * wy1;
}

__device__ __forceinline__ int mirror_row(long long p, int H, int W)
{
    const int row = (int)(p / W), col = (int)(p - (long long)row * W);
    return (H - 1 - row) * W + col;
}

struct UVShade {
    const float *images = nullptr;
    const int32_t *table = nullptr;
    const float *faces_uv = nullptr;
    const int32_t *face_image = nullptr;
    const float *base = nullptr;
    int ts = 0, M = 0, P = 0;
    int shared = 0;
};

struct UVSample {
    int m, f0;
    int q[4];
    float w[4];
    Taps t;
};

__device__ __forceinline__ void uv_locate(const UVShade &uv, int fi, int tex_faces, const float *face, float w0, float w1,
                                          float w2, float zp, double eps, UVSample &s)
{
    const bool flip = fi >= tex_faces;
    s.f0 = flip ? fi - tex_faces : fi;
    const int m = uv.face_image[s.f0];
    s.m = (m >= 0 && m < uv.M) ? m : -1;
    const float fz[3] = {face[2], face[5], face[8]};
    const float w[3] = {w0, w1, w2};
    if (s.m < 0) {
        compute_taps(fz, w, zp, uv.ts, eps, s.t, flip);
        return;
    }
    float d[3];
#pragma unroll
    for (int k = 0; k < 3; k++) d[k] = fminf(fmaxf(w[k] * (zp / fz[k]), 0.0f), 1.0f);
    if (flip) {
        const float d0 = d[0];
        d[0] = d[2];
        d[2] = d0;
    }
    const int off = uv.table[3 * s.m], H = uv.table[3 * s.m + 1], W = uv.table[3 * s.m + 2];
    long long p[4];
    texel_reads(uv.faces_uv + (size_t)s.f0 * 6, d, H, W, p, s.w);
#pragma unroll
    for (int r = 0; r < 4; r++) s.q[r] = off + mirror_row(p[r], H, W);
}

__device__ __forceinline__ void uv_color(const UVShade &uv, const UVSample &s, int b, float c[3])
{
    c[0] = c[1] = c[2] = 0.0f;
    if (s.m >= 0) {
        const float *img = uv.images + (uv.shared ? 0 : (size_t)b * uv.P * 3);
#pragma unroll
        for (int r = 0; r < 4; r++) {
            const float *px = img + (size_t)s.q[r] * 3;
            c[0] += px[0] * s.w[r];
            c[1] += px[1] * s.w[r];
            c[2] += px[2] * s.w[r];
        }
        return;
    }
    const int T = uv.ts * uv.ts * uv.ts;
    const float *texture = uv.base + (size_t)s.f0 * T * 3;
#pragma unroll
    for (int pn = 0; pn < 8; pn++) {
        if (s.t.isc[pn] >= T) continue;
        const float *tx = texture + s.t.isc[pn] * 3;
        c[0] += s.t.w[pn] * tx[0];
        c[1] += s.t.w[pn] * tx[1];
        c[2] += s.t.w[pn] * tx[2];
    }
}


constexpr unsigned NUM_XCD = 8;
inline unsigned xcd_grid(size_t n_blocks) { return (unsigned)((n_blocks + NUM_XCD - 1) / NUM_XCD * NUM_XCD); }
#ifdef __HIPCC__
__device__ __forceinline__ unsigned xcd_block(unsigned n_blocks)
{
    const unsigned chunk = (n_blocks + NUM_XCD - 1) / NUM_XCD;
    const unsigned logical = (blockIdx.x % NUM_XCD) * chunk + blockIdx.x / NUM_XCD;
    return logical < n_blocks ? logical : n_blocks;
}
#endif

inline size_t align_up(size_t v, size_t a) { return (v + a - 1) / a * a; }

#ifdef __HIPCC__
static __global__ __launch_bounds__(256) void k_fill_bytes(unsigned char *__restrict__ dst, size_t bytes, unsigned value32)
{
    const size_t i0 = ((size_t)blockIdx.x * blockDim.x + threadIdx.x) * 16;
    if (i0 >= bytes) return;
    if (i0 + 16 <= bytes && ((size_t)(dst + i0) & 15) == 0) {
        *reinterpret_cast<uint4 *>(dst + i0) = make_uint4(value32, value32, value32, value32);
    } else {
        for (size_t i = i0; i < bytes && i < i0 + 16; ++i) dst[i] = (unsigned char)value32;
    }
}
inline int fill_bytes(void *dst, int byte, size_t bytes, hipStream_t st)
{
    if (bytes == 0) return 0;
    const unsigned b = (unsigned)(byte & 0xff), v = b | (b << 8) | (b << 16) | (b << 24);
    hipLaunchKernelGGL(k_fill_bytes, dim3((unsigned)((bytes + 4095) / 4096)), dim3(256), 0, st, (unsigned char *)dst, bytes, v);
    return (int)hipGetLastError();
}
#endif

inline int check_sizes(int B, int F, int S)
{
    if (B < 1 || B > 65535 || F < 1 || S < 1 || S > 16384) return NR_E_SIZE;
    if ((size_t)B * (size_t)F > 0x7fffffffull / 9) return NR_E_SIZE;
    return 0;
}

inline int launch_status()
{
    const hipError_t e = hipGetLastError();
    return e == hipSuccess ? 0 : (int)e;
}


enum { STAGE_K6 = 1, STAGE_K7 = 2, STAGE_K8 = 4, STAGE_ALL = 7 };

struct BackwardCall {
    int stages;
    bool rgb, alpha;
    const float *faces, *faces_z_ref;
    const int32_t *face_index_map;
    const float *weight_map, *depth_map, *rgb_map, *alpha_map, *grad_rgb_map, *grad_alpha_map, *grad_depth_map;
    const float *sampling_weight_map;
    const int32_t *sampling_index_map;
    const float *face_inv_map;
    float *grad_faces, *grad_textures;
    int B, F, S, ts;
    double eps;
    int flags;
    const unsigned char *visible_faces;
    void *workspace;
    size_t workspace_bytes;
    FaceLight lit;
    hipStream_t st;
};

struct BandShape {
    int threads;
    int w_max;
    size_t budget;
};
enum K6Kernel { K6_KERNEL_FAST = 0, K6_KERNEL_ROW = 1, K6_KERNEL_GLOBAL = 2 };
struct K6Plan {
    int kernel;
    int mode;
    BandShape shape;
    int W_fast;
    size_t fast_lds;
    int win_lines, qcap;
    int W_row;
    size_t row_lds;
    int W, n_bands;
    bool use_records;
    bool overflow_pass;
    size_t fill_max;
};
K6Plan plan_k6(int B, int F, int S, bool rgb, double eps, int flags);

enum FaceZeros { FACE_ZEROS_NONE, FACE_ZEROS_UNLISTED, FACE_ZEROS_ALL };
enum TexZeros { TEX_ZEROS_NONE, TEX_ZEROS_BAND, TEX_ZEROS_SETUP, TEX_ZEROS_FILL };
enum K6Finish { FINISH_NONE, FINISH_KERNEL, FINISH_GATHER, FINISH_BIG, FINISH_ADD };
enum Gather { GATHER_NONE, GATHER_FACE, GATHER_ATOMIC };

struct BackwardPlan {
    bool k6;
    K6Plan k6p;
    bool bands;
    int face_zeros;
    bool gather_first;
    bool setup_alone;
    bool setup_in_gather;
    int tex_zeros;
    size_t tex_bytes;
    bool light_fill;
    int gather;
    bool listed;
    bool static_taps;
    int lanes;
    size_t gather_lds;
    bool depth_in_gather;
    bool big;
    int finish;
    bool depth;
    bool fill_faces;
    bool depth_lists;
};
int plan_backward(const BackwardCall &c, BackwardPlan &p);
int run_backward(const BackwardCall &c);

struct K6Lists {
    const int *vis_list, *vis_count, *slot_of;
    double *scratch;
};
struct LineSetupArgs;

int k6_compact(const BackwardCall &c, const K6Plan &p, int face_zeros, K6Lists &out);
LineSetupArgs k6_line_setup_args(const BackwardCall &c, const K6Plan &p);
int run_line_setup(const LineSetupArgs &a, hipStream_t st);
int k6_band(const BackwardCall &c, const K6Plan &p, const K6Lists &l, const LineSetupArgs &ls, void *fill,
            size_t fill_bytes);
void k6_finalize(const BackwardCall &c, const K6Lists &l, bool add);
bool k6_lists_fit(int B, int F, size_t workspace_bytes);
K6Lists k6_list_visible(const BackwardCall &c);
int gather_faces(const BackwardCall &c, const BackwardPlan &p, const K6Lists &l, const LineSetupArgs *ls);
void gather_big(const BackwardCall &c, const BackwardPlan &p, const K6Lists &l);
void gather_atomic(const BackwardCall &c);
void gather_depth(const BackwardCall &c, const K6Lists &l);

int face_light_args(const nr_face_light *lit, int F, bool backward, FaceLight &out);
int uv_images_args(const nr_face_light *lit, const nr_uv_images *uv, int B, int F, FaceLight &fl, UVShade &out);

}
```

neural_renderer_amd/csrc/nr_k6_tune.h:

```cpp
#pragma once

#ifndef NR_K6_FB
#define NR_K6_FB 3
#endif
#ifndef NR_K6_U_GROUP
#define NR_K6_U_GROUP 3
#endif
#ifndef NR_K6_SMALL_RASTER_MAX
#define NR_K6_SMALL_RASTER_MAX 400
#endif
#ifndef NR_K6_MINWAVES_256
#define NR_K6_MINWAVES_256 4
#endif
#ifndef NR_K6_WMAX
#define NR_K6_WMAX 4
#endif
#ifndef NR_K6_FOLD_KB
#define NR_K6_FOLD_KB 128
#endif
#ifndef NR_K6_LDS_BUDGET
#define NR_K6_LDS_BUDGET (53 * 1024)
#endif

#ifndef NR_K6_WIDE_BUDGET_FROM
#define NR_K6_WIDE_BUDGET_FROM 576
#endif
#ifndef NR_K6_WIDE_BUDGET_TO
#define NR_K6_WIDE_BUDGET_TO 832
#endif
#ifndef NR_K6_OVF_GRID
#define NR_K6_OVF_GRID 256
#endif
#ifndef NR_ROW_MIN_WGS
#define NR_ROW_MIN_WGS 4096
#endif
#ifndef NR_ROW_MIN_WGS_1
#define NR_ROW_MIN_WGS_1 1024
#endif

#ifndef NR_SHARED_LAUNCH_MAX_FACES
#define NR_SHARED_LAUNCH_MAX_FACES 98304
#endif

namespace nr {
namespace k6 {
constexpr int FB = NR_K6_FB;
constexpr int U_GROUP = NR_K6_U_GROUP;
static_assert(U_GROUP >= 1 && U_GROUP <= 4, "a super-piece's count travels in two bits");
constexpr int SMALL_RASTER_MAX = NR_K6_SMALL_RASTER_MAX;
constexpr int MINWAVES_256 = NR_K6_MINWAVES_256;
constexpr int WMAX = NR_K6_WMAX;
constexpr int FOLD_KB = NR_K6_FOLD_KB;
constexpr unsigned long LDS_BUDGET = NR_K6_LDS_BUDGET;
constexpr unsigned long ROW_MIN_WGS = NR_ROW_MIN_WGS, ROW_MIN_WGS_1 = NR_ROW_MIN_WGS_1;
constexpr unsigned OVF_GRID = NR_K6_OVF_GRID;
constexpr int WIDE_BUDGET_FROM = NR_K6_WIDE_BUDGET_FROM, WIDE_BUDGET_TO = NR_K6_WIDE_BUDGET_TO;
constexpr unsigned long SHARED_LAUNCH_MAX_FACES = NR_SHARED_LAUNCH_MAX_FACES;
}
}
```

Measured before the change: 14140.

## Fold texture face-gather into the tail of the row band backward kernel

Adds a gather-in-tail path. For ts=2 static-tap, unlit, unsampled row-kernel configurations too large for the shared-launch gather-first path, the per-face texture gather runs inside the band kernel's tail rather than as a separate launch. The gather body moves into a shared header so both kernels can use it, and textures are zeroed only for unlisted faces. This removes a kernel launch and a re-read of the pixel maps, but adds register and LDS pressure to the band kernel and makes its control flow more complex.

```diff
diff --git a/neural_renderer_amd/_build.py b/neural_renderer_amd/_build.py
--- a/neural_renderer_amd/_build.py
+++ b/neural_renderer_amd/_build.py
@@ -8,7 +8,7 @@
                                                       'nr_uv_pixel.hip', 'nr_vertex_colors.hip')]
 HEADERS = [os.path.join(os.path.dirname(HERE), 'include', 'nr_hip.h'), os.path.join(os.path.dirname(HERE), 'include', 'nr_hip_profile.h'),
            os.path.join(HERE, 'csrc', 'nr_device.h'),
-           os.path.join(HERE, 'csrc', 'nr_k6_tune.h'), os.path.join(HERE, 'csrc', 'nr_band_lines.h'),
+           os.path.join(HERE, 'csrc', 'nr_k6_tune.h'), os.path.join(HERE, 'csrc', 'nr_band_lines.h'), os.path.join(HERE, 'csrc', 'nr_face_gather.h'),
            os.path.join(HERE, 'csrc', 'nr_shade.h')]
 LIB_PATH = os.path.join(HERE, 'libnr_hip.so')
 PROFILE_LIB_PATH = os.path.join(HERE, 'libnr_hip_prof.so')
diff --git a/neural_renderer_amd/csrc/nr_backward.hip b/neural_renderer_amd/csrc/nr_backward.hip
--- a/neural_renderer_amd/csrc/nr_backward.hip
+++ b/neural_renderer_amd/csrc/nr_backward.hip
@@ -37,12 +37,16 @@
     }
     const bool fold = p.bands && k7 && ts <= 13;
     p.gather_first = fold && (size_t)B * F <= k6::SHARED_LAUNCH_MAX_FACES && !(c.flags & NR_FLAG_SERIAL_BACKWARD);
-    p.face_zeros = p.gather_first ? FACE_ZEROS_ALL : (fold ? FACE_ZEROS_UNLISTED : FACE_ZEROS_NONE);
-    p.finish = !p.bands ? FINISH_NONE : p.gather_first ? (ts <= 8 ? FINISH_BIG : FINISH_ADD) : (fold ? FINISH_GATHER : FINISH_KERNEL);
+    const bool ts2_static = ts == 2 && (float)(1.0 - c.eps) < 1.0f;
+    p.gather_in_tail = k6::TAIL_GATHER_MAX_FACES > 0 && fold && !p.gather_first && !(c.flags & NR_FLAG_SERIAL_BACKWARD) &&
+                       ts2_static && !sampled && !c.lit.light && p.k6p.kernel == K6_KERNEL_ROW && !(c.flags & NR_FLAG_EXACT_GRADIENT) &&
+                       !p.k6p.row_chunked && c.S <= 512 && (size_t)B * F <= k6::TAIL_GATHER_MAX_FACES;
+    const bool gather_early = p.gather_first || p.gather_in_tail;
+    p.face_zeros = gather_early ? FACE_ZEROS_ALL : (fold ? FACE_ZEROS_UNLISTED : FACE_ZEROS_NONE);
+    p.finish = !p.bands ? FINISH_NONE : gather_early ? (ts <= 8 ? FINISH_BIG : FINISH_ADD) : (fold ? FINISH_GATHER : FINISH_KERNEL);
 
     if (k7) {
         const size_t n_tex = (size_t)ts * ts * ts * 3;
-        const bool ts2_static = ts == 2 && (float)(1.0 - c.eps) < 1.0f;
         p.static_taps = ts2_static && !sampled;
         p.gather = ts <= 13 ? GATHER_FACE : GATHER_ATOMIC;
         p.listed = p.bands && ts <= 13;
@@ -55,7 +59,7 @@
             p.setup_in_gather = p.k6p.use_records && k6_line_setup_args(c, p.k6p).lds_bytes <= 32768 && p.gather_lds <= 40960;
             if (p.setup_in_gather && !c.lit.light && ((size_t)c.grad_textures & 15) == 0) p.tex_zeros = TEX_ZEROS_SETUP;
         } else if (fold && p.tex_bytes % 16 == 0 && ((size_t)c.grad_textures & 15) == 0 && p.tex_bytes <= p.k6p.fill_max) {
-            p.tex_zeros = TEX_ZEROS_BAND;
+            p.tex_zeros = p.gather_in_tail ? TEX_ZEROS_BAND_UNLISTED : TEX_ZEROS_BAND;
         }
         if (p.tex_zeros == TEX_ZEROS_NONE && (c.lit.light || p.listed || ts > 13)) p.tex_zeros = TEX_ZEROS_FILL;
         p.light_fill = c.lit.light && c.lit.grad_light;
@@ -94,11 +98,15 @@
         }
         if (p.setup_alone)
             if (int rc = run_line_setup(ls, c.st)) return rc;
-        const bool band_fill = p.tex_zeros == TEX_ZEROS_BAND;
-        if (int rc = k6_band(c, p.k6p, l, ls, band_fill ? c.grad_textures : nullptr, band_fill ? p.tex_bytes : 0)) return rc;
+        if (p.gather_in_tail)
+            if (int rc = fill_texture_zeros(c, p)) return rc;
+        const bool band_fill = p.tex_zeros == TEX_ZEROS_BAND || p.tex_zeros == TEX_ZEROS_BAND_UNLISTED;
+        if (int rc = k6_band(c, p.k6p, l, ls, band_fill ? c.grad_textures : nullptr, band_fill ? p.tex_bytes : 0,
+                             p.gather_in_tail ? &p : nullptr))
+            return rc;
         if (p.finish == FINISH_KERNEL) k6_finalize(c, l, false);
     }
-    if (p.gather != GATHER_NONE && !p.gather_first) {
+    if (p.gather != GATHER_NONE && !p.gather_first && !p.gather_in_tail) {
         if (int rc = fill_texture_zeros(c, p)) return rc;
         if (p.gather == GATHER_FACE)
             if (int rc = gather_faces(c, p, l, nullptr)) return rc;
diff --git a/neural_renderer_amd/csrc/nr_backward_gather.hip b/neural_renderer_amd/csrc/nr_backward_gather.hip
--- a/neural_renderer_amd/csrc/nr_backward_gather.hip
+++ b/neural_renderer_amd/csrc/nr_backward_gather.hip
@@ -1,411 +1,16 @@
 #include "nr_device.h"
 #include "nr_band_lines.h"
+#include "nr_face_gather.h"
 #include <type_traits>
 
 using namespace nr;
 
 namespace {
-
-constexpr int BIG_PX = 2048;
-
-__device__ __forceinline__ float group_sum(float v, int width)
-{
-    for (int o = width >> 1; o > 0; o >>= 1) v += __shfl_xor(v, o, WAVE);
-    return v;
-}
-
-__device__ __forceinline__ float row16_sum_last(float v)
-{
-    v += __int_as_float(__builtin_amdgcn_update_dpp(0, __float_as_int(v), 0x111, 0xf, 0xf, true));
-    v += __int_as_float(__builtin_amdgcn_update_dpp(0, __float_as_int(v), 0x112, 0xf, 0xf, true));
-    v += __int_as_float(__builtin_amdgcn_update_dpp(0, __float_as_int(v), 0x114, 0xf, 0xf, true));
-    v += __int_as_float(__builtin_amdgcn_update_dpp(0, __float_as_int(v), 0x118, 0xf, 0xf, true));
-    return v;
-}
-
-struct DepthConst {
-    float tmp[3], zz[3];
-};
-__device__ __forceinline__ DepthConst depth_constants(const float f[9], int S)
-{
-    const float fs = (float)S;
-    const float px[3] = {to_pixel(f[0], fs), to_pixel(f[3], fs), to_pixel(f[6], fs)};
-    const float py[3] = {to_pixel(f[1], fs), to_pixel(f[4], fs), to_pixel(f[7], fs)};
-    float inv[9];
-    compute_face_inv(px, py, inv);
-    DepthConst d;
-#pragma unroll
-    for (int k = 0; k < 3; k++) {
-        d.tmp[k] = 0.0f;
-#pragma unroll
-        for (int l = 0; l < 3; l++) d.tmp[k] += -inv[3 * l + k] / f[3 * l + 2];
-        d.zz[k] = f[3 * k + 2] * f[3 * k + 2];
-    }
-    return d;
-}
-
-template <int STEPS, class Eval>
-__device__ __forceinline__ void walk_owned_pixels(const Cand &cd, int n_mine, int fn, const int32_t *__restrict__ fi_img,
-                                                  int S, int sub, int L, int *__restrict__ queue_base, Eval eval)
-{
-    const int tid = threadIdx.x;
-    const int QL = L < 64 ? L : 64;
-    int *queue = queue_base + (tid / QL) * (2 * QL);
-    const int qsub = tid & (QL - 1);
-    const int qshift = (tid & 63) & ~(QL - 1);
-    const unsigned long long qmask = QL == 64 ? ~0ull : ((1ull << QL) - 1ull);
-    int waiting = 0;
-    for (int i = sub;; i += STEPS * L) {
-        bool more2[STEPS], owned2[STEPS];
-        int off2[STEPS];
-#pragma unroll
-        for (int h = 0; h < STEPS; ++h) {
-            const int ii = i + h * L;
-            more2[h] = ii < n_mine;
-            int x = 0, y = 0, f = 0;
-            off2[h] = 0;
-            bool in = false;
-            if (more2[h] && cand_pixel(cd, ii, S, x, y)) {
-                off2[h] = y * S + x;
-                f = fi_img[off2[h]];
-                in = true;
-            }
-            owned2[h] = in && f == fn;
-        }
-        bool done = false;
-#pragma unroll
-        for (int h = 0; h < STEPS; ++h) {
-            if (done) break;
-            const bool more = more2[h], owned = owned2[h];
-            const int off = off2[h];
-            const bool any_more = __ballot(more) != 0ull;
-            const unsigned long long m = (__ballot(owned) >> qshift) & qmask;
-            if (owned) queue[waiting + __popcll(m & ((1ull << qsub) - 1ull))] = off;
-            waiting += __popcll(m);
-            const bool ready = waiting >= QL || (!any_more && waiting > 0);
-            if (__ballot(ready) != 0ull) {
-                __builtin_amdgcn_fence(__ATOMIC_RELEASE, "wavefront");
-                __builtin_amdgcn_wave_barrier();
-                __builtin_amdgcn_fence(__ATOMIC_ACQUIRE, "wavefront");
-                const int take = ready ? (waiting < QL ? waiting : QL) : 0;
-                const int e = qsub < take ? queue[qsub] : 0;
-                const int rest = (ready && qsub + QL < waiting) ? queue[qsub + QL] : 0;
-                __builtin_amdgcn_fence(__ATOMIC_RELEASE, "wavefront");
-                __builtin_amdgcn_wave_barrier();
-                __builtin_amdgcn_fence(__ATOMIC_ACQUIRE, "wavefront");
-                waiting -= take;
-                if (ready && qsub < waiting) queue[qsub] = rest;
-                if (qsub < take) eval(e);
-            }
-            if (!any_more) done = true;
-        }
-        if (done) break;
-    }
-}
-
-struct FaceGatherArgs {
-    const int32_t *face_index_map;
-    const float *sampling_weight_map;
-    const int32_t *sampling_index_map;
-    const float *faces, *zbase, *weight_map, *depth_map, *g_rgb;
-    float *grad_textures;
-    int n_faces_total, F, S, ts;
-    double eps;
-    int fix_batch_z, L;
-    const int *vis_list, *vis_count;
-    const float *g_depth;
-    float *grad_faces;
-    const double *k6_scratch;
-    const int *slot_of;
-    FaceLight lit;
-};
-
-template <bool TS2, bool DEPTH, bool LIT>
-__device__ __forceinline__ void face_gather_body(const FaceGatherArgs &a, const int bx, const int by)
-{
-    const int32_t *__restrict__ face_index_map = a.face_index_map;
-    const float *__restrict__ sampling_weight_map = a.sampling_weight_map;
-    const int32_t *__restrict__ sampling_index_map = a.sampling_index_map;
-    const float *__restrict__ faces = a.faces, *__restrict__ zbase = a.zbase, *__restrict__ weight_map = a.weight_map,
-                *__restrict__ depth_map = a.depth_map, *__restrict__ g_rgb = a.g_rgb;
-    float *__restrict__ grad_textures = a.grad_textures;
-    const int n_faces_total = a.n_faces_total, F = a.F, S = a.S, ts = a.ts;
-    const double eps = a.eps;
-    const int fix_batch_z = a.fix_batch_z, L = a.L;
-    const int *__restrict__ vis_list = a.vis_list, *__restrict__ vis_count = a.vis_count;
-    const float *__restrict__ g_depth = a.g_depth;
-    float *__restrict__ grad_faces = a.grad_faces;
-    const double *__restrict__ k6_scratch = a.k6_scratch;
-    const FaceLight &lit = a.lit;
-    extern __shared__ __attribute__((aligned(16))) double s_acc[];
-    __shared__ int s_queue[512];
-    __shared__ int s_own;
-    __shared__ float s_gl[3];
-
-    const int tid = threadIdx.x;
-    const int grp = tid / L, sub = tid - grp * L;
-    const int n_tex = ts * ts * ts * 3;
-    int gi = bx * (256 / L) + grp;
-    bool face_ok = gi < n_faces_total;
-    int slot = 0;
-    if (vis_list) {
-        slot = gi;
-        const int n_vis = vis_count[by];
-        if (bx * (256 / L) >= n_vis) return;
-        face_ok = slot < n_vis;
-        gi = face_ok ? by * F + vis_list[(size_t)by * F + slot] : 0;
-    }
-    double *acc_l = s_acc + (size_t)grp * n_tex;
-
-    float acc[24];
-#pragma unroll
-    for (int k = 0; k < 24; k++) acc[k] = 0.0f;
-    float dacc[9];
-#pragma unroll
-    for (int k = 0; k < 9; k++) dacc[k] = 0.0f;
-    bool any_box = false;
-    bool own = false;
-    if (!TS2) {
-        for (int k = sub; k < n_tex; k += L) acc_l[k] = 0.0;
-        if (LIT) {
-            if (tid < 3) s_gl[tid] = 0.0f;
-            if (tid == 0) s_own = 0;
-        }
-        __syncthreads();
-    }
-
-    Cand cd;
-    cd.n = 0;
-    int fn = 0;
-    size_t img = 0;
-    DepthConst dc;
-#pragma unroll
-    for (int k = 0; k < 3; k++) dc.tmp[k] = dc.zz[k] = 0.0f;
-    float face_z[3] = {1.0f, 1.0f, 1.0f};
-    bool flip = false;
-    size_t cube = 0;
-    if (LIT) {
-        const int b = vis_list ? by : gi / F, f = gi - b * F;
-        flip = f >= lit.tex_faces;
-        cube = (size_t)b * lit.tex_faces + (flip ? f - lit.tex_faces : f);
-    }
-    if (face_ok) {
-        const int b = gi / F;
-        fn = gi - b * F;
-        const float *f = faces + (size_t)gi * 9;
-        cd = face_candidates(f[0], f[1], f[3], f[4], f[6], f[7], S);
-        if (cd.n > 0 && (L == 256 || (cd.n <= BIG_PX))) {
-            any_box = true;
-            if (DEPTH) {
-                float fv[9];
-#pragma unroll
-                for (int k = 0; k < 9; k++) fv[k] = f[k];
-                dc = depth_constants(fv, S);
-            }
-            const float *fz = (fix_batch_z ? faces + (size_t)b * F * 9 : zbase) + (size_t)fn * 9;
-            face_z[0] = fz[2]; face_z[1] = fz[5]; face_z[2] = fz[8];
-            img = (size_t)b * S * S;
-        }
-    }
-    walk_owned_pixels<(TS2 && DEPTH) ? 1 : 2>(cd, any_box ? cd.n : 0, fn, face_index_map + img, S, sub, L, s_queue, [&](int off) {
-        const size_t p = img + (size_t)off;
-        float wk[3] = {0.0f, 0.0f, 0.0f}, depth = 0.0f, gd = 0.0f;
-        if (weight_map) { wk[0] = weight_map[3 * p]; wk[1] = weight_map[3 * p + 1]; wk[2] = weight_map[3 * p + 2]; }
-        if (depth_map) depth = depth_map[p];
-        if (DEPTH) gd = g_depth[p];
-        const float g[3] = {g_rgb[3 * p], g_rgb[3 * p + 1], g_rgb[3 * p + 2]};
-        if (LIT) own = true;
-        Taps t;
-        if (sampling_weight_map) {
-#pragma unroll
-            for (int pn = 0; pn < 8; pn++) {
-                t.w[pn] = sampling_weight_map[8 * p + pn];
-                t.isc[pn] = sampling_index_map[8 * p + pn];
-            }
-        } else {
-            compute_taps(face_z, wk, depth, ts, eps, t, LIT && flip);
-        }
-        if (DEPTH) {
-            const float depth2 = depth * depth;
-#pragma unroll
-            for (int k = 0; k < 3; k++) dacc[3 * k + 2] += gd * wk[k] * depth2 / dc.zz[k];
-#pragma unroll
-            for (int k = 0; k < 3; k++)
-#pragma unroll
-                for (int l = 0; l < 2; l++) dacc[3 * k + l] += -gd * dc.tmp[l] * wk[k] * depth2 * (float)S / 2.0f;
-        }
-#pragma unroll
-        for (int pn = 0; pn < 8; pn++) {
-            if (TS2) {
-                acc[3 * pn + 0] += t.w[pn] * g[0];
-                acc[3 * pn + 1] += t.w[pn] * g[1];
-                acc[3 * pn + 2] += t.w[pn] * g[2];
-            } else {
-                if (t.isc[pn] * 3 >= n_tex) continue;
-                double *q = acc_l + t.isc[pn] * 3;
-                atomicAdd(q + 0, (double)(t.w[pn] * g[0]));
-                atomicAdd(q + 1, (double)(t.w[pn] * g[1]));
-                atomicAdd(q + 2, (double)(t.w[pn] * g[2]));
-            }
-        }
-    });
-
-    bool owned = false;
-    if (LIT) {
-        if (L <= 64) {
-            const unsigned long long bm = __ballot(own);
-            owned = L == 64 ? bm != 0ull : ((bm >> (tid & 48)) & 0xffffull) != 0ull;
-        } else {
-            if (own) s_own = 1;
-            __syncthreads();
-            owned = s_own != 0;
-        }
-    }
-    if (TS2) {
-#pragma unroll
-        for (int k = 0; k < 24; k++) acc[k] = row16_sum_last(acc[k]);
-        if (LIT) {
-            if (face_ok && sub == 15 && owned) {
-                const float *lc = lit.light + (size_t)gi * 3;
-                const float l3[3] = {lc[0], lc[1], lc[2]};
-                float tx[24];
-                if (lit.textures) {
-                    const float4 *src = reinterpret_cast<const float4 *>(lit.textures + cube * 24);
-#pragma unroll
-                    for (int k = 0; k < 6; k++) {
-                        const float4 v = src[k];
-                        tx[4 * k] = v.x; tx[4 * k + 1] = v.y; tx[4 * k + 2] = v.z; tx[4 * k + 3] = v.w;
-                    }
-                } else {
-#pragma unroll
-                    for (int k = 0; k < 24; k++) tx[k] = 0.0f;
-                }
-                float o[24], gl[3] = {0.0f, 0.0f, 0.0f};
-#pragma unroll
-                for (int u = 0; u < 8; u++) {
-                    const int r = (u & 1) * 4 + (u & 2) + (u >> 2);
-#pragma unroll
-                    for (int c = 0; c < 3; c++) {
-                        const float a = flip ? acc[3 * u + c] : acc[3 * r + c];
-                        o[3 * u + c] = a * l3[c];
-                        gl[c] += a * tx[3 * u + c];
-                    }
-                }
-                float4 *dst = reinterpret_cast<float4 *>(grad_textures + cube * 24);
-#pragma unroll
-                for (int k = 0; k < 6; k++) dst[k] = make_float4(o[4 * k], o[4 * k + 1], o[4 * k + 2], o[4 * k + 3]);
-                if (lit.grad_light) {
-                    float *gd = lit.grad_light + (size_t)gi * 3;
-                    gd[0] = gl[0]; gd[1] = gl[1]; gd[2] = gl[2];
-                }
-            }
-        } else if (face_ok && sub == 15) {
-            float o[24];
-#pragma unroll
-            for (int pn = 0; pn < 8; pn++) {
-                const int isc = (pn & 1) * 4 + ((pn >> 1) & 1) * 2 + ((pn >> 2) & 1);
-                o[3 * isc + 0] = acc[3 * pn + 0];
-                o[3 * isc + 1] = acc[3 * pn + 1];
-                o[3 * isc + 2] = acc[3 * pn + 2];
-            }
-            float4 *dst = reinterpret_cast<float4 *>(grad_textures + (size_t)gi * 24);
-#pragma unroll
-            for (int k = 0; k < 6; k++) dst[k] = make_float4(o[4 * k], o[4 * k + 1], o[4 * k + 2], o[4 * k + 3]);
-        }
-    } else if (LIT) {
-        __syncthreads();
-        float gl0 = 0.0f, gl1 = 0.0f, gl2 = 0.0f;
-        if (face_ok && owned) {
-            const float *lc = lit.light + (size_t)gi * 3;
-            const float l3[3] = {lc[0], lc[1], lc[2]};
-            const float *tex = lit.textures ? lit.textures + cube * n_tex : nullptr;
-            float *dst = grad_textures + cube * n_tex;
-            if (tex) {
-                for (int k = sub; k < n_tex; k += L) {
-                    const int c = k % 3;
-                    const float v = (float)acc_l[k] * tex[k];
-                    gl0 += c == 0 ? v : 0.0f;
-                    gl1 += c == 1 ? v : 0.0f;
-                    gl2 += c == 2 ? v : 0.0f;
-                }
-            }
-            for (int k = sub; k < n_tex; k += L) {
-                const int c = k % 3;
-                dst[k] = (float)acc_l[k] * (c == 0 ? l3[0] : (c == 1 ? l3[1] : l3[2]));
-            }
-        }
-        if (lit.grad_light) {
-            if (L <= 64) {
-                gl0 = group_sum(gl0, L); gl1 = group_sum(gl1, L); gl2 = group_sum(gl2, L);
-            } else {
-                if (gl0 != 0.0f) atomicAdd(&s_gl[0], gl0);
-                if (gl1 != 0.0f) atomicAdd(&s_gl[1], gl1);
-                if (gl2 != 0.0f) atomicAdd(&s_gl[2], gl2);
-                __syncthreads();
-                gl0 = s_gl[0]; gl1 = s_gl[1]; gl2 = s_gl[2];
-            }
-            if (face_ok && owned && sub == 0) {
-                float *gd = lit.grad_light + (size_t)gi * 3;
-                gd[0] = gl0; gd[1] = gl1; gd[2] = gl2;
-            }
-        }
-    } else {
-        __syncthreads();
-        if (face_ok) {
-            float *dst = grad_textures + (size_t)gi * n_tex;
-            for (int k = sub; k < n_tex; k += L) dst[k] = (float)acc_l[k];
-        }
-    }
-    if (DEPTH || k6_scratch) {
-        if (DEPTH && __ballot(any_box) != 0ull) {
-#pragma unroll
-            for (int k = 0; k < 9; k++) dacc[k] = (L == 16) ? row16_sum_last(dacc[k]) : group_sum(dacc[k], L);
-        }
-        if (face_ok && sub == ((L == 16) ? 15 : 0)) {
-            float *gf = grad_faces + (size_t)gi * 9;
-            if (k6_scratch) {
-                const double *sc = k6_scratch + ((size_t)by * F + slot) * 6;
-#pragma unroll
-                for (int v = 0; v < 3; v++) {
-                    gf[3 * v + 0] = (float)sc[2 * v + 0] + dacc[3 * v + 0];
-                    gf[3 * v + 1] = (float)sc[2 * v + 1] + dacc[3 * v + 1];
-                    gf[3 * v + 2] = 0.0f + dacc[3 * v + 2];
-                }
-            } else if (any_box) {
-#pragma unroll
-                for (int k = 0; k < 9; k++) gf[k] += dacc[k];
-            }
-        }
-    }
-}
 
 template <bool TS2, bool DEPTH, bool LIT>
 __global__ __launch_bounds__(256) void k_backward_textures_face(FaceGatherArgs a)
 {
     face_gather_body<TS2, DEPTH, LIT>(a, (int)blockIdx.x, (int)blockIdx.y);
-}
-
-struct ZeroArgs {
-    float *grad_textures;
-    const int *slot_of;
-    int F;
-    int epf;
-    int vec;
-    unsigned wgs;
-};
-
-__device__ __forceinline__ void zero_unlisted_body(const ZeroArgs &z, const int bx, const int by)
-{
-    const size_t per_image = (size_t)z.F * z.epf;
-    const size_t e0 = (size_t)bx * 2048, e1 = e0 + 2048 < per_image ? e0 + 2048 : per_image;
-    const int *__restrict__ slot = z.slot_of + (size_t)by * z.F;
-    for (size_t e = e0 + threadIdx.x; e < e1; e += 256) {
-        const int face = (int)(e / (unsigned)z.epf);
-        if (slot[face] >= 0) continue;
-        const size_t at = (size_t)by * per_image + e;
-        if (z.vec) reinterpret_cast<float4 *>(z.grad_textures)[at] = make_float4(0.0f, 0.0f, 0.0f, 0.0f);
-        else z.grad_textures[at] = 0.0f;
-    }
 }
 
 template <bool TS2, bool DEPTH, bool LIT>
@@ -430,7 +35,7 @@
     extern __shared__ __attribute__((aligned(16))) double s_tex[];
     __shared__ int s_list[256];
     __shared__ int s_wave_n[4];
-    __shared__ float s_red[36];
+    __shared__ float s_red[4][36];
     __shared__ int s_own;
     const int tid = threadIdx.x;
     if (vis_list && (int)blockIdx.x * 256 >= vis_count[blockIdx.y]) return;
@@ -442,13 +47,15 @@
             ok = gi < vis_count[blockIdx.y];
             gi = ok ? (int)blockIdx.y * F + vis_list[(size_t)blockIdx.y * F + gi] : 0;
         }
-        if (k6_scratch && ok && blockIdx.z == 0) {
+        const bool finish = k6_scratch && ok && blockIdx.z == 0;
+        float k6v[6], had[6];
+        float *gf = grad_faces + (size_t)gi * 9;
+        if (finish) {
             const double *sc = k6_scratch + ((size_t)blockIdx.y * F + blockIdx.x * 256 + tid) * 6;
-            float *gf = grad_faces + (size_t)gi * 9;
 #pragma unroll
             for (int v = 0; v < 3; v++) {
-                atomicAdd(gf + 3 * v + 0, (float)sc[2 * v + 0]);
-                atomicAdd(gf + 3 * v + 1, (float)sc[2 * v + 1]);
+                k6v[2 * v + 0] = (float)sc[2 * v + 0]; k6v[2 * v + 1] = (float)sc[2 * v + 1];
+                had[2 * v + 0] = gf[3 * v + 0]; had[2 * v + 1] = gf[3 * v + 1];
             }
         }
         bool big = false;
@@ -457,6 +64,18 @@
             const float *f = faces + (size_t)gi * 9;
             const Cand cd = face_candidates(f[0], f[1], f[3], f[4], f[6], f[7], S);
             big = cd.n > BIG_PX;
+        }
+        if (finish) {
+#pragma unroll
+            for (int v = 0; v < 3; v++) {
+                if (big) {
+                    atomicAdd(gf + 3 * v + 0, k6v[2 * v + 0]);
+                    atomicAdd(gf + 3 * v + 1, k6v[2 * v + 1]);
+                } else {
+                    gf[3 * v + 0] = k6v[2 * v + 0] + had[2 * v + 0];
+                    gf[3 * v + 1] = k6v[2 * v + 1] + had[2 * v + 1];
+                }
+            }
         }
         const unsigned long long m = __ballot(big);
         const int lane = tid & 63, wave = tid >> 6;
@@ -484,7 +103,7 @@
         const float face_z[3] = {fz[2], fz[5], fz[8]};
         const bool flip = TEX && LIT && fn >= lit.tex_faces;
         for (int k = tid; k < n_lds; k += 256) s_tex[k] = 0.0;
-        if (tid < 36) s_red[tid] = 0.0f;
+        if (tid < 4 * 36) (&s_red[0][0])[tid] = 0.0f;
         if (LIT && tid == 0) s_own = 0;
         __syncthreads();
         bool own = false;
@@ -553,18 +172,19 @@
 #pragma unroll
             for (int k = 0; k < 9; k++) {
                 const float v = group_sum(dacc[k], 64);
-                if ((tid & 63) == 0 && v != 0.0f) atomicAdd(&s_red[k], v);
+                if ((tid & 63) == 0) s_red[tid >> 6][k] = v;
             }
         }
         if (TEX == 2) {
 #pragma unroll
             for (int k = 0; k < 24; k++) {
                 const float v = group_sum(tacc[k], 64);
-                if ((tid & 63) == 0 && v != 0.0f) atomicAdd(&s_red[9 + k], v);
+                if ((tid & 63) == 0) s_red[tid >> 6][9 + k] = v;
             }
         }
         if (TEX && LIT && own) s_own = 1;
         __syncthreads();
+        auto red = [&](int k) { return ((s_red[0][k] + s_red[1][k]) + s_red[2][k]) + s_red[3][k]; };
         if (TEX && LIT) {
             if (s_own) {
                 const size_t cube = (size_t)b * lit.tex_faces + (flip ? fn - lit.tex_faces : fn);
@@ -577,16 +197,16 @@
                     float a;
                     if (TEX == 2) {
                         u = 3 * (flip ? q : (q & 1) * 4 + (q & 2) + (q >> 2)) + c;
-                        a = s_red[9 + k];
+                        a = red(9 + k);
                     } else {
                         a = (float)s_tex[k];
                     }
                     dst[u] = a * lc[c];
-                    if (tex && a != 0.0f) atomicAdd(&s_red[33 + c], a * tex[u]);
+                    if (tex && a != 0.0f) atomicAdd(&s_red[0][33 + c], a * tex[u]);
                 }
                 if (lit.grad_light) {
                     __syncthreads();
-                    if (tid < 3) lit.grad_light[(size_t)gi * 3 + tid] = s_red[33 + tid];
+                    if (tid < 3) lit.grad_light[(size_t)gi * 3 + tid] = s_red[0][33 + tid];
                 }
             }
         } else {
@@ -597,12 +217,12 @@
         if (TEX == 2 && tid < 24) {
             const int pn = tid / 3, c = tid - 3 * pn;
             const int isc = (pn & 1) * 4 + ((pn >> 1) & 1) * 2 + ((pn >> 2) & 1);
-            grad_textures[(size_t)gi * 24 + 3 * isc + c] = s_red[9 + tid];
+            grad_textures[(size_t)gi * 24 + 3 * isc + c] = red(9 + tid);
         }
         }
         if (DEPTH && tid < 9) {
-            if (k6_scratch) atomicAdd(grad_faces + (size_t)gi * 9 + tid, s_red[tid]);
-            else grad_faces[(size_t)gi * 9 + tid] += s_red[tid];
+            if (k6_scratch) atomicAdd(grad_faces + (size_t)gi * 9 + tid, red(tid));
+            else grad_faces[(size_t)gi * 9 + tid] += red(tid);
         }
         __syncthreads();
     }
@@ -784,14 +404,7 @@
     const int per = 256 / p.lanes;
     const int *vis_list = p.listed ? l.vis_list : nullptr;
     const dim3 grid = vis_list ? dim3((unsigned)((F + per - 1) / per), (unsigned)B) : dim3((unsigned)((n + per - 1) / per));
-    const bool fold = p.finish == FINISH_GATHER;
-    const FaceGatherArgs ga = {c.face_index_map, c.sampling_weight_map, c.sampling_index_map, c.faces,
-                               c.faces_z_ref ? c.faces_z_ref : c.faces,
-                               c.weight_map, c.depth_map, c.grad_rgb_map, c.grad_textures, n, F, c.S, ts, c.eps,
-                               (c.flags & NR_FLAG_FIX_TEXTURE_BATCH_Z) ? 1 : 0, p.lanes, vis_list, l.vis_count,
-                               p.depth_in_gather ? c.grad_depth_map : nullptr,
-                               (p.depth_in_gather || fold) ? c.grad_faces : nullptr, fold ? l.scratch : nullptr,
-                               fold ? l.slot_of : nullptr, c.lit};
+    const FaceGatherArgs ga = face_gather_args(c, p, l);
     auto go = [&](auto ts2, auto dep, auto lit) {
         constexpr bool T = decltype(ts2)::value, D = decltype(dep)::value, LIT = decltype(lit)::value;
         if (ls) {
diff --git a/neural_renderer_amd/csrc/nr_backward_pixel_map.hip b/neural_renderer_amd/csrc/nr_backward_pixel_map.hip
--- a/neural_renderer_amd/csrc/nr_backward_pixel_map.hip
+++ b/neural_renderer_amd/csrc/nr_backward_pixel_map.hip
@@ -1,5 +1,6 @@
 #include "nr_device.h"
 #include "nr_band_lines.h"
+#include "nr_face_gather.h"
 #include "nr_k6_tune.h"
 
 #include <atomic>
@@ -1159,13 +1160,13 @@
 #define NR_ROW_STAT(i, v) ((void)0)
 #endif
 
-template <bool RGB, bool ALPHA, int MODE, bool CHUNKED>
-__global__ __launch_bounds__(rowk::NT, MODE == K6_FAST ? 5 : 4) void k_bpm_row(
+template <bool RGB, bool ALPHA, int MODE, bool CHUNKED, bool UNLISTED>
+__device__ __forceinline__ void bpm_row_body(
     const int32_t *__restrict__ fi_map, const float *__restrict__ rgb_map, const float *__restrict__ alpha_map,
     const float *__restrict__ g_rgb, const float *__restrict__ g_alpha, double *__restrict__ scratch,
     const int *__restrict__ band_lines, const int *__restrict__ band_start, const int *__restrict__ lines_ok,
     const BandLine *__restrict__ line_buf, size_t cap, int F, int S, int W, int CH, float eps_f, double eps_d, int B,
-    uint4 *__restrict__ zero16, size_t n_zero16)
+    uint4 *__restrict__ zero16, size_t n_zero16, const int *__restrict__ zero_slot, unsigned zero_epf)
 {
     using namespace rowk;
     constexpr bool EXACT = MODE != K6_FAST;
@@ -1177,7 +1178,10 @@
     if (logical >= total_wg) return;
     if (n_zero16) {
         const size_t per = (n_zero16 + total_wg - 1) / total_wg, z_lo = (size_t)logical * per, z_hi = min(n_zero16, z_lo + per);
-        for (size_t k = z_lo + tid; k < z_hi; k += NT) zero16[k] = make_uint4(0u, 0u, 0u, 0u);
+        for (size_t k = z_lo + tid; k < z_hi; k += NT) {
+            if constexpr (UNLISTED) { if (zero_slot[k / zero_epf] >= 0) continue; }
+            zero16[k] = make_uint4(0u, 0u, 0u, 0u);
+        }
     }
     const unsigned bandidx = logical / n_ch;
     const int c0 = CHUNKED ? (int)(logical - bandidx * n_ch) * CH : 0, SL = CHUNKED ? min(CH, S - c0) : S;
@@ -1695,6 +1699,47 @@
     }
 }
 
+template <bool RGB, bool ALPHA, int MODE, bool CHUNKED>
+__global__ __launch_bounds__(rowk::NT, MODE == K6_FAST ? 5 : 4) void k_bpm_row(
+    const int32_t *__restrict__ fi_map, const float *__restrict__ rgb_map, const float *__restrict__ alpha_map,
+    const float *__restrict__ g_rgb, const float *__restrict__ g_alpha, double *__restrict__ scratch,
+    const int *__restrict__ band_lines, const int *__restrict__ band_start, const int *__restrict__ lines_ok,
+    const BandLine *__restrict__ line_buf, size_t cap, int F, int S, int W, int CH, float eps_f, double eps_d, int B,
+    uint4 *__restrict__ zero16, size_t n_zero16)
+{
+    bpm_row_body<RGB, ALPHA, MODE, CHUNKED, false>(fi_map, rgb_map, alpha_map, g_rgb, g_alpha, scratch, band_lines, band_start, lines_ok,
+                                                   line_buf, cap, F, S, W, CH, eps_f, eps_d, B, zero16, n_zero16, nullptr, 1u);
+}
+
+struct BandRowArgs {
+    const int32_t *fi_map;
+    const float *rgb_map, *alpha_map, *g_rgb, *g_alpha;
+    double *scratch;
+    const int *band_lines, *band_start, *lines_ok;
+    const BandLine *line_buf;
+    size_t cap;
+    int F, S, W, B;
+    float eps_f;
+    double eps_d;
+    uint4 *zero16;
+    size_t n_zero16;
+    const int *zero_slot;
+    unsigned zero_epf;
+};
+
+template <bool RGB, bool ALPHA, bool DEPTH>
+__global__ __launch_bounds__(rowk::NT, 5) void k_band_gather(BandRowArgs r, FaceGatherArgs g, unsigned band_grid, unsigned gather_x)
+{
+    if (blockIdx.x < band_grid) {
+        bpm_row_body<RGB, ALPHA, K6_FAST, false, true>(r.fi_map, r.rgb_map, r.alpha_map, r.g_rgb, r.g_alpha, r.scratch, r.band_lines,
+                                                       r.band_start, r.lines_ok, r.line_buf, r.cap, r.F, r.S, r.W, r.S, r.eps_f, r.eps_d,
+                                                       r.B, r.zero16, r.n_zero16, r.zero_slot, r.zero_epf);
+    } else {
+        const unsigned id = blockIdx.x - band_grid;
+        face_gather_body<true, DEPTH, false>(g, (int)(id % gather_x), (int)(id / gather_x));
+    }
+}
+
 __global__ __launch_bounds__(256) void k_bpm_finalize(const double *__restrict__ scratch, const int *__restrict__ slot_of,
                                                       float *__restrict__ grad_faces, int F, int n_faces_total, int add)
 {
@@ -1905,6 +1950,28 @@
     return n_ch > 1 ? go(std::true_type()) : go(std::false_type());
 }
 
+template <bool RGB, bool ALPHA>
+int launch_band_gather(const K6Plan &p, const BackwardCall &c, const BackwardPlan &bp, const K6Lists &l, const LineSetupArgs &ls,
+                       void *fill, size_t fill_bytes)
+{
+    const int B = c.B, F = c.F, S = c.S, W = p.W_row;
+    const unsigned total_wg = (unsigned)((S + W - 1) / W) * 2u * (unsigned)B, band_grid = xcd_grid(total_wg);
+    const unsigned gather_x = (unsigned)((F + 15) / 16);
+    const BandRowArgs ra = {c.face_index_map, c.rgb_map, c.alpha_map, c.grad_rgb_map, c.grad_alpha_map, l.scratch, ls.band_lines,
+                            ls.band_start, ls.lines_ok, ls.line_buf, ls.cap, F, S, W, B, (float)c.eps, c.eps, (uint4 *)fill,
+                            fill_bytes / 16, l.slot_of, 6u};
+    const FaceGatherArgs ga = face_gather_args(c, bp, l);
+    auto go = [&](auto depth) {
+        constexpr bool D = decltype(depth)::value;
+        static LdsLimit limit;
+        if (int rc = limit.ensure((const void *)k_band_gather<RGB, ALPHA, D>, p.row_lds)) return rc;
+        hipLaunchKernelGGL((k_band_gather<RGB, ALPHA, D>), dim3(band_grid + gather_x * (unsigned)B), dim3(rowk::NT), p.row_lds, c.st,
+                           ra, ga, band_grid, gather_x);
+        return 0;
+    };
+    return bp.depth_in_gather ? go(std::true_type()) : go(std::false_type());
+}
+
 int k6_row_band(int B, int F, int S, bool rgb, double eps, int flags, size_t *row_lds)
 {
     const bool exact = (flags & NR_FLAG_EXACT_GRADIENT) != 0;
@@ -1932,6 +1999,7 @@
     const bool row = p.W_row > 0;
     p.kernel = row ? K6_KERNEL_ROW : K6_KERNEL_FAST;
     p.overflow_pass = row;
+    p.row_chunked = row && row_chunk(S, F) < S;
     p.W = row ? 1 : p.W_fast;
     p.n_bands = (S + p.W - 1) / p.W;
     p.use_records = !(flags & NR_FLAG_K6_SCAN) && B <= 65535 && p.n_bands <= 3072;
@@ -2071,7 +2139,8 @@
     return launch_status();
 }
 
-int nr::k6_band(const BackwardCall &c, const K6Plan &plan, const K6Lists &l, const LineSetupArgs &ls, void *fill, size_t fill_bytes)
+int nr::k6_band(const BackwardCall &c, const K6Plan &plan, const K6Lists &l, const LineSetupArgs &ls, void *fill, size_t fill_bytes,
+                const BackwardPlan *tail)
 {
     if (plan.kernel == K6_KERNEL_GLOBAL) {
         auto global = [&](auto r, auto a) {
@@ -2095,8 +2164,16 @@
             return launch_row<decltype(r)::value, decltype(a)::value, decltype(m)::value>(plan, c, l, ls, fill, fill_bytes);
         });
     };
+    auto band_gather = [&]() {
+        auto go = [&](auto r, auto a) {
+            return launch_band_gather<decltype(r)::value, decltype(a)::value>(plan, c, *tail, l, ls, fill, fill_bytes);
+        };
+        using T = std::true_type;
+        using N = std::false_type;
+        return (c.rgb && c.alpha) ? go(T(), T()) : (c.rgb ? go(T(), N()) : go(N(), T()));
+    };
     NR_BAND_TIMER_START(c.st, plan.kernel);
-    int rc = plan.kernel == K6_KERNEL_ROW ? band_row() : band_fast(std::false_type(), fill, fill_bytes);
+    int rc = tail ? band_gather() : (plan.kernel == K6_KERNEL_ROW ? band_row() : band_fast(std::false_type(), fill, fill_bytes));
     NR_BAND_TIMER_STOP(c.st);
     if (rc == 0 && plan.overflow_pass) rc = band_fast(std::true_type(), nullptr, 0);
     return rc ? rc : launch_status();
diff --git a/neural_renderer_amd/csrc/nr_device.h b/neural_renderer_amd/csrc/nr_device.h
--- a/neural_renderer_amd/csrc/nr_device.h
+++ b/neural_renderer_amd/csrc/nr_device.h
@@ -365,12 +365,13 @@
     int W, n_bands;
     bool use_records;
     bool overflow_pass;
+    bool row_chunked;
     size_t fill_max;
 };
 K6Plan plan_k6(int B, int F, int S, bool rgb, double eps, int flags);
 
 enum FaceZeros { FACE_ZEROS_NONE, FACE_ZEROS_UNLISTED, FACE_ZEROS_ALL };
-enum TexZeros { TEX_ZEROS_NONE, TEX_ZEROS_BAND, TEX_ZEROS_SETUP, TEX_ZEROS_FILL };
+enum TexZeros { TEX_ZEROS_NONE, TEX_ZEROS_BAND, TEX_ZEROS_SETUP, TEX_ZEROS_FILL, TEX_ZEROS_BAND_UNLISTED };
 enum K6Finish { FINISH_NONE, FINISH_KERNEL, FINISH_GATHER, FINISH_BIG, FINISH_ADD };
 enum Gather { GATHER_NONE, GATHER_FACE, GATHER_ATOMIC };
 
@@ -380,6 +381,7 @@
     bool bands;
     int face_zeros;
     bool gather_first;
+    bool gather_in_tail;
     bool setup_alone;
     bool setup_in_gather;
     int tex_zeros;
@@ -409,8 +411,8 @@
 int k6_compact(const BackwardCall &c, const K6Plan &p, int face_zeros, K6Lists &out);
 LineSetupArgs k6_line_setup_args(const BackwardCall &c, const K6Plan &p);
 int run_line_setup(const LineSetupArgs &a, hipStream_t st);
-int k6_band(const BackwardCall &c, const K6Plan &p, const K6Lists &l, const LineSetupArgs &ls, void *fill,
-            size_t fill_bytes);
+int k6_band(const BackwardCall &c, const K6Plan &p, const K6Lists &l, const LineSetupArgs &ls, void *fill, size_t fill_bytes,
+            const BackwardPlan *tail);
 void k6_finalize(const BackwardCall &c, const K6Lists &l, bool add);
 bool k6_lists_fit(int B, int F, size_t workspace_bytes);
 K6Lists k6_list_visible(const BackwardCall &c);
diff --git a/neural_renderer_amd/csrc/nr_face_gather.h b/neural_renderer_amd/csrc/nr_face_gather.h
--- /dev/null
+++ b/neural_renderer_amd/csrc/nr_face_gather.h
@@ -0,0 +1,416 @@
+#pragma once
+#include "nr_device.h"
+
+namespace nr {
+namespace {
+
+constexpr int BIG_PX = 2048;
+
+__device__ __forceinline__ float group_sum(float v, int width)
+{
+    for (int o = width >> 1; o > 0; o >>= 1) v += __shfl_xor(v, o, WAVE);
+    return v;
+}
+
+__device__ __forceinline__ float row16_sum_last(float v)
+{
+    v += __int_as_float(__builtin_amdgcn_update_dpp(0, __float_as_int(v), 0x111, 0xf, 0xf, true));
+    v += __int_as_float(__builtin_amdgcn_update_dpp(0, __float_as_int(v), 0x112, 0xf, 0xf, true));
+    v += __int_as_float(__builtin_amdgcn_update_dpp(0, __float_as_int(v), 0x114, 0xf, 0xf, true));
+    v += __int_as_float(__builtin_amdgcn_update_dpp(0, __float_as_int(v), 0x118, 0xf, 0xf, true));
+    return v;
+}
+
+struct DepthConst {
+    float tmp[3], zz[3];
+};
+__device__ __forceinline__ DepthConst depth_constants(const float f[9], int S)
+{
+    const float fs = (float)S;
+    const float px[3] = {to_pixel(f[0], fs), to_pixel(f[3], fs), to_pixel(f[6], fs)};
+    const float py[3] = {to_pixel(f[1], fs), to_pixel(f[4], fs), to_pixel(f[7], fs)};
+    float inv[9];
+    compute_face_inv(px, py, inv);
+    DepthConst d;
+#pragma unroll
+    for (int k = 0; k < 3; k++) {
+        d.tmp[k] = 0.0f;
+#pragma unroll
+        for (int l = 0; l < 3; l++) d.tmp[k] += -inv[3 * l + k] / f[3 * l + 2];
+        d.zz[k] = f[3 * k + 2] * f[3 * k + 2];
+    }
+    return d;
+}
+
+template <int STEPS, class Eval>
+__device__ __forceinline__ void walk_owned_pixels(const Cand &cd, int n_mine, int fn, const int32_t *__restrict__ fi_img,
+                                                  int S, int sub, int L, int *__restrict__ queue_base, Eval eval)
+{
+    const int tid = threadIdx.x;
+    const int QL = L < 64 ? L : 64;
+    int *queue = queue_base + (tid / QL) * (2 * QL);
+    const int qsub = tid & (QL - 1);
+    const int qshift = (tid & 63) & ~(QL - 1);
+    const unsigned long long qmask = QL == 64 ? ~0ull : ((1ull << QL) - 1ull);
+    int waiting = 0;
+    for (int i = sub;; i += STEPS * L) {
+        bool more2[STEPS], owned2[STEPS];
+        int off2[STEPS];
+#pragma unroll
+        for (int h = 0; h < STEPS; ++h) {
+            const int ii = i + h * L;
+            more2[h] = ii < n_mine;
+            int x = 0, y = 0, f = 0;
+            off2[h] = 0;
+            bool in = false;
+            if (more2[h] && cand_pixel(cd, ii, S, x, y)) {
+                off2[h] = y * S + x;
+                f = fi_img[off2[h]];
+                in = true;
+            }
+            owned2[h] = in && f == fn;
+        }
+        bool done = false;
+#pragma unroll
+        for (int h = 0; h < STEPS; ++h) {
+            if (done) break;
+            const bool more = more2[h], owned = owned2[h];
+            const int off = off2[h];
+            const bool any_more = __ballot(more) != 0ull;
+            const unsigned long long m = (__ballot(owned) >> qshift) & qmask;
+            if (owned) queue[waiting + __popcll(m & ((1ull << qsub) - 1ull))] = off;
+            waiting += __popcll(m);
+            const bool ready = waiting >= QL || (!any_more && waiting > 0);
+            if (__ballot(ready) != 0ull) {
+                __builtin_amdgcn_fence(__ATOMIC_RELEASE, "wavefront");
+                __builtin_amdgcn_wave_barrier();
+                __builtin_amdgcn_fence(__ATOMIC_ACQUIRE, "wavefront");
+                const int take = ready ? (waiting < QL ? waiting : QL) : 0;
+                const int e = qsub < take ? queue[qsub] : 0;
+                const int rest = (ready && qsub + QL < waiting) ? queue[qsub + QL] : 0;
+                __builtin_amdgcn_fence(__ATOMIC_RELEASE, "wavefront");
+                __builtin_amdgcn_wave_barrier();
+                __builtin_amdgcn_fence(__ATOMIC_ACQUIRE, "wavefront");
+                waiting -= take;
+                if (ready && qsub < waiting) queue[qsub] = rest;
+                if (qsub < take) eval(e);
+            }
+            if (!any_more) done = true;
+        }
+        if (done) break;
+    }
+}
+
+struct FaceGatherArgs {
+    const int32_t *face_index_map;
+    const float *sampling_weight_map;
+    const int32_t *sampling_index_map;
+    const float *faces, *zbase, *weight_map, *depth_map, *g_rgb;
+    float *grad_textures;
+    int n_faces_total, F, S, ts;
+    double eps;
+    int fix_batch_z, L;
+    const int *vis_list, *vis_count;
+    const float *g_depth;
+    float *grad_faces;
+    const double *k6_scratch;
+    const int *slot_of;
+    FaceLight lit;
+};
+
+inline FaceGatherArgs face_gather_args(const BackwardCall &c, const BackwardPlan &p, const K6Lists &l)
+{
+    const bool fold = p.finish == FINISH_GATHER;
+    return {c.face_index_map, c.sampling_weight_map, c.sampling_index_map, c.faces,
+            c.faces_z_ref ? c.faces_z_ref : c.faces,
+            c.weight_map, c.depth_map, c.grad_rgb_map, c.grad_textures, c.B * c.F, c.F, c.S, c.ts, c.eps,
+            (c.flags & NR_FLAG_FIX_TEXTURE_BATCH_Z) ? 1 : 0, p.lanes, p.listed ? l.vis_list : nullptr, l.vis_count,
+            p.depth_in_gather ? c.grad_depth_map : nullptr,
+            (p.depth_in_gather || fold) ? c.grad_faces : nullptr, fold ? l.scratch : nullptr,
+            fold ? l.slot_of : nullptr, c.lit};
+}
+
+template <bool TS2, bool DEPTH, bool LIT>
+__device__ __forceinline__ void face_gather_body(const FaceGatherArgs &a, const int bx, const int by)
+{
+    const int32_t *__restrict__ face_index_map = a.face_index_map;
+    const float *__restrict__ sampling_weight_map = a.sampling_weight_map;
+    const int32_t *__restrict__ sampling_index_map = a.sampling_index_map;
+    const float *__restrict__ faces = a.faces, *__restrict__ zbase = a.zbase, *__restrict__ weight_map = a.weight_map,
+                *__restrict__ depth_map = a.depth_map, *__restrict__ g_rgb = a.g_rgb;
+    float *__restrict__ grad_textures = a.grad_textures;
+    const int n_faces_total = a.n_faces_total, F = a.F, S = a.S, ts = a.ts;
+    const double eps = a.eps;
+    const int fix_batch_z = a.fix_batch_z, L = a.L;
+    const int *__restrict__ vis_list = a.vis_list, *__restrict__ vis_count = a.vis_count;
+    const float *__restrict__ g_depth = a.g_depth;
+    float *__restrict__ grad_faces = a.grad_faces;
+    const double *__restrict__ k6_scratch = a.k6_scratch;
+    const FaceLight &lit = a.lit;
+    extern __shared__ __attribute__((aligned(16))) double s_acc[];
+    __shared__ int s_queue[512];
+    __shared__ int s_own;
+    __shared__ float s_gl[3];
+
+    const int tid = threadIdx.x;
+    const int grp = tid / L, sub = tid - grp * L;
+    const int n_tex = ts * ts * ts * 3;
+    int gi = bx * (256 / L) + grp;
+    bool face_ok = gi < n_faces_total;
+    int slot = 0;
+    if (vis_list) {
+        slot = gi;
+        const int n_vis = vis_count[by];
+        if (bx * (256 / L) >= n_vis) return;
+        face_ok = slot < n_vis;
+        gi = face_ok ? by * F + vis_list[(size_t)by * F + slot] : 0;
+    }
+    double *acc_l = s_acc + (size_t)grp * n_tex;
+
+    float acc[24];
+#pragma unroll
+    for (int k = 0; k < 24; k++) acc[k] = 0.0f;
+    float dacc[9];
+#pragma unroll
+    for (int k = 0; k < 9; k++) dacc[k] = 0.0f;
+    bool any_box = false;
+    bool own = false;
+    if (!TS2) {
+        for (int k = sub; k < n_tex; k += L) acc_l[k] = 0.0;
+        if (LIT) {
+            if (tid < 3) s_gl[tid] = 0.0f;
+            if (tid == 0) s_own = 0;
+        }
+        __syncthreads();
+    }
+
+    Cand cd;
+    cd.n = 0;
+    int fn = 0;
+    size_t img = 0;
+    DepthConst dc;
+#pragma unroll
+    for (int k = 0; k < 3; k++) dc.tmp[k] = dc.zz[k] = 0.0f;
+    float face_z[3] = {1.0f, 1.0f, 1.0f};
+    bool flip = false;
+    size_t cube = 0;
+    if (LIT) {
+        const int b = vis_list ? by : gi / F, f = gi - b * F;
+        flip = f >= lit.tex_faces;
+        cube = (size_t)b * lit.tex_faces + (flip ? f - lit.tex_faces : f);
+    }
+    if (face_ok) {
+        const int b = gi / F;
+        fn = gi - b * F;
+        const float *f = faces + (size_t)gi * 9;
+        cd = face_candidates(f[0], f[1], f[3], f[4], f[6], f[7], S);
+        if (cd.n > 0 && (L == 256 || (cd.n <= BIG_PX))) {
+            any_box = true;
+            if (DEPTH) {
+                float fv[9];
+#pragma unroll
+                for (int k = 0; k < 9; k++) fv[k] = f[k];
+                dc = depth_constants(fv, S);
+            }
+            const float *fz = (fix_batch_z ? faces + (size_t)b * F * 9 : zbase) + (size_t)fn * 9;
+            face_z[0] = fz[2]; face_z[1] = fz[5]; face_z[2] = fz[8];
+            img = (size_t)b * S * S;
+        }
+    }
+    walk_owned_pixels<(TS2 && DEPTH) ? 1 : 2>(cd, any_box ? cd.n : 0, fn, face_index_map + img, S, sub, L, s_queue, [&](int off) {
+        const size_t p = img + (size_t)off;
+        float wk[3] = {0.0f, 0.0f, 0.0f}, depth = 0.0f, gd = 0.0f;
+        if (weight_map) { wk[0] = weight_map[3 * p]; wk[1] = weight_map[3 * p + 1]; wk[2] = weight_map[3 * p + 2]; }
+        if (depth_map) depth = depth_map[p];
+        if (DEPTH) gd = g_depth[p];
+        const float g[3] = {g_rgb[3 * p], g_rgb[3 * p + 1], g_rgb[3 * p + 2]};
+        if (LIT) own = true;
+        Taps t;
+        if (sampling_weight_map) {
+#pragma unroll
+            for (int pn = 0; pn < 8; pn++) {
+                t.w[pn] = sampling_weight_map[8 * p + pn];
+                t.isc[pn] = sampling_index_map[8 * p + pn];
+            }
+        } else {
+            compute_taps(face_z, wk, depth, ts, eps, t, LIT && flip);
+        }
+        if (DEPTH) {
+            const float depth2 = depth * depth;
+#pragma unroll
+            for (int k = 0; k < 3; k++) dacc[3 * k + 2] += gd * wk[k] * depth2 / dc.zz[k];
+#pragma unroll
+            for (int k = 0; k < 3; k++)
+#pragma unroll
+                for (int l = 0; l < 2; l++) dacc[3 * k + l] += -gd * dc.tmp[l] * wk[k] * depth2 * (float)S / 2.0f;
+        }
+#pragma unroll
+        for (int pn = 0; pn < 8; pn++) {
+            if (TS2) {
+                acc[3 * pn + 0] += t.w[pn] * g[0];
+                acc[3 * pn + 1] += t.w[pn] * g[1];
+                acc[3 * pn + 2] += t.w[pn] * g[2];
+            } else {
+                if (t.isc[pn] * 3 >= n_tex) continue;
+                double *q = acc_l + t.isc[pn] * 3;
+                atomicAdd(q + 0, (double)(t.w[pn] * g[0]));
+                atomicAdd(q + 1, (double)(t.w[pn] * g[1]));
+                atomicAdd(q + 2, (double)(t.w[pn] * g[2]));
+            }
+        }
+    });
+
+    bool owned = false;
+    if (LIT) {
+        if (L <= 64) {
+            const unsigned long long bm = __ballot(own);
+            owned = L == 64 ? bm != 0ull : ((bm >> (tid & 48)) & 0xffffull) != 0ull;
+        } else {
+            if (own) s_own = 1;
+            __syncthreads();
+            owned = s_own != 0;
+        }
+    }
+    if (TS2) {
+#pragma unroll
+        for (int k = 0; k < 24; k++) acc[k] = row16_sum_last(acc[k]);
+        if (LIT) {
+            if (face_ok && sub == 15 && owned) {
+                const float *lc = lit.light + (size_t)gi * 3;
+                const float l3[3] = {lc[0], lc[1], lc[2]};
+                float tx[24];
+                if (lit.textures) {
+                    const float4 *src = reinterpret_cast<const float4 *>(lit.textures + cube * 24);
+#pragma unroll
+                    for (int k = 0; k < 6; k++) {
+                        const float4 v = src[k];
+                        tx[4 * k] = v.x; tx[4 * k + 1] = v.y; tx[4 * k + 2] = v.z; tx[4 * k + 3] = v.w;
+                    }
+                } else {
+#pragma unroll
+                    for (int k = 0; k < 24; k++) tx[k] = 0.0f;
+                }
+                float o[24], gl[3] = {0.0f, 0.0f, 0.0f};
+#pragma unroll
+                for (int u = 0; u < 8; u++) {
+                    const int r = (u & 1) * 4 + (u & 2) + (u >> 2);
+#pragma unroll
+                    for (int c = 0; c < 3; c++) {
+                        const float a = flip ? acc[3 * u + c] : acc[3 * r + c];
+                        o[3 * u + c] = a * l3[c];
+                        gl[c] += a * tx[3 * u + c];
+                    }
+                }
+                float4 *dst = reinterpret_cast<float4 *>(grad_textures + cube * 24);
+#pragma unroll
+                for (int k = 0; k < 6; k++) dst[k] = make_float4(o[4 * k], o[4 * k + 1], o[4 * k + 2], o[4 * k + 3]);
+                if (lit.grad_light) {
+                    float *gd = lit.grad_light + (size_t)gi * 3;
+                    gd[0] = gl[0]; gd[1] = gl[1]; gd[2] = gl[2];
+                }
+            }
+        } else if (face_ok && sub == 15) {
+            float o[24];
+#pragma unroll
+            for (int pn = 0; pn < 8; pn++) {
+                const int isc = (pn & 1) * 4 + ((pn >> 1) & 1) * 2 + ((pn >> 2) & 1);
+                o[3 * isc + 0] = acc[3 * pn + 0];
+                o[3 * isc + 1] = acc[3 * pn + 1];
+                o[3 * isc + 2] = acc[3 * pn + 2];
+            }
+            float4 *dst = reinterpret_cast<float4 *>(grad_textures + (size_t)gi * 24);
+#pragma unroll
+            for (int k = 0; k < 6; k++) dst[k] = make_float4(o[4 * k], o[4 * k + 1], o[4 * k + 2], o[4 * k + 3]);
+        }
+    } else if (LIT) {
+        __syncthreads();
+        float gl0 = 0.0f, gl1 = 0.0f, gl2 = 0.0f;
+        if (face_ok && owned) {
+            const float *lc = lit.light + (size_t)gi * 3;
+            const float l3[3] = {lc[0], lc[1], lc[2]};
+            const float *tex = lit.textures ? lit.textures + cube * n_tex : nullptr;
+            float *dst = grad_textures + cube * n_tex;
+            if (tex) {
+                for (int k = sub; k < n_tex; k += L) {
+                    const int c = k % 3;
+                    const float v = (float)acc_l[k] * tex[k];
+                    gl0 += c == 0 ? v : 0.0f;
+                    gl1 += c == 1 ? v : 0.0f;
+                    gl2 += c == 2 ? v : 0.0f;
+                }
+            }
+            for (int k = sub; k < n_tex; k += L) {
+                const int c = k % 3;
+                dst[k] = (float)acc_l[k] * (c == 0 ? l3[0] : (c == 1 ? l3[1] : l3[2]));
+            }
+        }
+        if (lit.grad_light) {
+            if (L <= 64) {
+                gl0 = group_sum(gl0, L); gl1 = group_sum(gl1, L); gl2 = group_sum(gl2, L);
+            } else {
+                if (gl0 != 0.0f) atomicAdd(&s_gl[0], gl0);
+                if (gl1 != 0.0f) atomicAdd(&s_gl[1], gl1);
+                if (gl2 != 0.0f) atomicAdd(&s_gl[2], gl2);
+                __syncthreads();
+                gl0 = s_gl[0]; gl1 = s_gl[1]; gl2 = s_gl[2];
+            }
+            if (face_ok && owned && sub == 0) {
+                float *gd = lit.grad_light + (size_t)gi * 3;
+                gd[0] = gl0; gd[1] = gl1; gd[2] = gl2;
+            }
+        }
+    } else {
+        __syncthreads();
+        if (face_ok) {
+            float *dst = grad_textures + (size_t)gi * n_tex;
+            for (int k = sub; k < n_tex; k += L) dst[k] = (float)acc_l[k];
+        }
+    }
+    if (DEPTH || k6_scratch) {
+        if (DEPTH && __ballot(any_box) != 0ull) {
+#pragma unroll
+            for (int k = 0; k < 9; k++) dacc[k] = (L == 16) ? row16_sum_last(dacc[k]) : group_sum(dacc[k], L);
+        }
+        if (face_ok && sub == ((L == 16) ? 15 : 0)) {
+            float *gf = grad_faces + (size_t)gi * 9;
+            if (k6_scratch) {
+                const double *sc = k6_scratch + ((size_t)by * F + slot) * 6;
+#pragma unroll
+                for (int v = 0; v < 3; v++) {
+                    gf[3 * v + 0] = (float)sc[2 * v + 0] + dacc[3 * v + 0];
+                    gf[3 * v + 1] = (float)sc[2 * v + 1] + dacc[3 * v + 1];
+                    gf[3 * v + 2] = 0.0f + dacc[3 * v + 2];
+                }
+            } else if (any_box) {
+#pragma unroll
+                for (int k = 0; k < 9; k++) gf[k] += dacc[k];
+            }
+        }
+    }
+}
+
+struct ZeroArgs {
+    float *grad_textures;
+    const int *slot_of;
+    int F;
+    int epf;
+    int vec;
+    unsigned wgs;
+};
+
+__device__ __forceinline__ void zero_unlisted_body(const ZeroArgs &z, const int bx, const int by)
+{
+    const size_t per_image = (size_t)z.F * z.epf;
+    const size_t e0 = (size_t)bx * 2048, e1 = e0 + 2048 < per_image ? e0 + 2048 : per_image;
+    const int *__restrict__ slot = z.slot_of + (size_t)by * z.F;
+    for (size_t e = e0 + threadIdx.x; e < e1; e += 256) {
+        const int face = (int)(e / (unsigned)z.epf);
+        if (slot[face] >= 0) continue;
+        const size_t at = (size_t)by * per_image + e;
+        if (z.vec) reinterpret_cast<float4 *>(z.grad_textures)[at] = make_float4(0.0f, 0.0f, 0.0f, 0.0f);
+        else z.grad_textures[at] = 0.0f;
+    }
+}
+
+}
+}
diff --git a/neural_renderer_amd/csrc/nr_k6_tune.h b/neural_renderer_amd/csrc/nr_k6_tune.h
--- a/neural_renderer_amd/csrc/nr_k6_tune.h
+++ b/neural_renderer_amd/csrc/nr_k6_tune.h
@@ -41,6 +41,9 @@
 #ifndef NR_SHARED_LAUNCH_MAX_FACES
 #define NR_SHARED_LAUNCH_MAX_FACES 98304
 #endif
+#ifndef NR_TAIL_GATHER_MAX_FACES
+#define NR_TAIL_GATHER_MAX_FACES 655360
+#endif
 
 namespace nr {
 namespace k6 {
@@ -56,5 +59,6 @@
 constexpr unsigned OVF_GRID = NR_K6_OVF_GRID;
 constexpr int WIDE_BUDGET_FROM = NR_K6_WIDE_BUDGET_FROM, WIDE_BUDGET_TO = NR_K6_WIDE_BUDGET_TO;
 constexpr unsigned long SHARED_LAUNCH_MAX_FACES = NR_SHARED_LAUNCH_MAX_FACES;
+constexpr unsigned long TAIL_GATHER_MAX_FACES = NR_TAIL_GATHER_MAX_FACES;
 }
 }
```

New measurement: 15060, median of 6. 1.06x the previous value.
